# antonilo/unsupervised_detection

Hardware: NVIDIA H100
Metric: frame-pairs/sec adversarial train step 256x448 (higher is better)
Workload: dtype bf16

## Files before the change

include/cis_b200.h:

```cpp
#ifndef CIS_B200_H_
#define CIS_B200_H_
#include <stdint.h>
#include <stddef.h>

#ifdef __cplusplus
extern "C" {
#endif

typedef void* cis_stream_t;

enum { CIS_OK = 0, CIS_ERR_BAD_ARG = 1, CIS_ERR_UNSUPPORTED = 2, CIS_ERR_CUDA = 3 };
enum { CIS_ACT_NONE = 0, CIS_ACT_ELU = 1, CIS_ACT_LEAKY = 2 };
enum { CIS_MAX_TAPS = 49, CIS_MAX_SRC = 4 };

typedef struct {
  const void* ptr;
  int32_t pitch;
  int32_t c_off;
  int32_t chunks;
  int32_t n_mod;
} CisSrc;

typedef struct {
  int32_t N, H, W;
  int32_t OH, OW;
  int32_t sh, sw;
  int32_t ntaps;
  int16_t dh[CIS_MAX_TAPS];
  int16_t dw[CIS_MAX_TAPS];
  int32_t nsrc;
  CisSrc src[CIS_MAX_SRC];
  const void* wpack;
  int32_t K_pad;
  int32_t BN;
  int32_t n_tiles;
  const float* bias;
  int32_t act;
  float alpha;
  int32_t DH, DW;
  int32_t osh, osw, oa, ob;
  void* out;
  int32_t out_pitch, out_coff, out_ch;
  float* outf;
  int32_t outf_pitch, outf_coff, outf_ch;
  const void* add_pre;
  int32_t add_pre_pitch, add_pre_coff;
  const float* addf_pre;
  int32_t addf_pitch, addf_coff;
  const void* add_post;
  int32_t add_post_pitch, add_post_coff;
  int32_t mode;
  int32_t halo;
  int32_t dil;
  int32_t MT;
  int32_t hoy, hox;
  int32_t ey, ex;
  int32_t splits;
  float* sk_scratch;
  int32_t* sk_counters;
  int32_t nph;
  int32_t ph_tap[5];
  int32_t sk_cluster;
  int32_t nsub;
  struct {
    int32_t tap0, ntaps;
    int32_t hoy, hox;
    int32_t OH, OW, oa, ob;
    const void* wpack;
  } sub[4];
  int32_t nwg;
} CisConv;

typedef struct {
  int32_t N, H, W, OH, OW, sh, sw, ntaps;
  int16_t dh[CIS_MAX_TAPS];
  int16_t dw[CIS_MAX_TAPS];
  int32_t nsrc;
  CisSrc src[CIS_MAX_SRC];
  const void* g;
  int32_t g_pitch, g_coff, g_chunks;
  float* dwp;
  int32_t Cout;
  int32_t K_pad;
  int32_t splits;
  int32_t tma;
  int32_t nh;
  int32_t nwg;
} CisWgrad;

const char* cis_last_error(void);
int cis_version(void);
uint32_t cis_crc32c(uint32_t crc, const void* data, size_t n);
int cis_host_resize_bilinear_legacy(const float* src, int32_t H, int32_t W, int32_t C, float* dst, int32_t OH, int32_t OW);
int cis_host_bgr8_to_rgb_resized(const unsigned char* bgr, int32_t H, int32_t W, float* dst, int32_t OH, int32_t OW);

int cis_conv_igemm(const CisConv* d, cis_stream_t stream);
int cis_set_persist_mode(int mode);
int cis_conv_wgrad(const CisWgrad* d, cis_stream_t stream);

int cis_pack_weights(const float* w, const int32_t* kmap, int32_t K_pad, int32_t rows, int32_t cout, int32_t sn, const int32_t* nmap,
                     void* wp, cis_stream_t stream);
int cis_pack_weights_tiled(const float* w, const int32_t* kmap, int32_t cin8, int32_t ntaps, int32_t n_tiles, int32_t BN, int32_t cout,
                           int32_t sn, const int32_t* nmap, void* out, cis_stream_t stream);
int cis_unpack_wgrad(const float* dwp, const int32_t* kmap, int32_t K_pad, int32_t cout, int32_t nsplit, float* dw, const float* colpart,
                     int32_t nblocks, int32_t nch, float* db, int32_t layout, cis_stream_t stream);
int cis_bn_fold(const float* w, const float* bias, const float* gamma, const float* beta, int64_t nw, int32_t cout, float* w_eff,
                float* b_eff, cis_stream_t stream);
int cis_bn_chain(const float* w, const float* bias, const float* gamma, float* dw_eff_to_dw, const float* db_eff, int64_t nw,
                 int32_t cout, float* dbias, float* dgamma, float* dbeta, cis_stream_t stream);

enum { CIS_JOB_PACK = 0, CIS_JOB_PACK_TILED = 1, CIS_JOB_UNPACK = 2, CIS_JOB_BN_FOLD = 3, CIS_JOB_BN_CHAIN = 4 };
typedef struct {
  int32_t kind;
  int32_t i[8];
  int64_t n;
  const void* p[8];
} CisParamJob;
int cis_param_multi(const CisParamJob* jobs_dev, int32_t njobs, int32_t total_blocks, cis_stream_t stream);

int cis_dact_mul(void* g, int32_t g_pitch, int32_t g_coff, const void* y, int32_t y_pitch, int32_t y_coff, const void* res,
                 int32_t res_pitch, int32_t res_coff, int64_t npix, int32_t chunks, int32_t act, float alpha, cis_stream_t stream);
int cis_add_slice(void* dst, int32_t dst_pitch, int32_t dst_coff, const void* src, int32_t src_pitch, int32_t src_coff,
                  int64_t npix_dst, int32_t chunks, int32_t reps, int32_t accumulate, cis_stream_t stream);
int cis_colsum(const void* g, int32_t g_pitch, int32_t g_coff, int64_t npix, int32_t nch, float* part, int32_t nblocks, cis_stream_t stream);

int cis_zero(void* ptr, int64_t nbytes, cis_stream_t stream);

int cis_dact_colsum(void* g, int32_t g_pitch, int32_t g_coff, const void* y, int32_t y_pitch, int32_t y_coff, const void* res,
                    int32_t res_pitch, int32_t res_coff, int64_t npix, int32_t nch, int32_t act, float alpha, float* part, int32_t nblocks,
                    cis_stream_t stream);

int cis_resize_bilinear_bf16(const void* src, int32_t s_pitch, int32_t s_coff, int32_t N, int32_t H, int32_t W, void* dst,
                             int32_t d_pitch, int32_t d_coff, int32_t OH, int32_t OW, int32_t chunks, cis_stream_t stream);
int cis_resize_concat_bf16(const CisSrc* srcs, int32_t nsrc, int32_t N, int32_t H, int32_t W, void* dst, int32_t d_pitch, int32_t d_coff,
                           int32_t OH, int32_t OW, cis_stream_t stream);
int cis_resize_concat_bf16_bwd(const void* ddst, int32_t d_pitch, int32_t d_coff, int32_t N, int32_t OH, int32_t OW, const CisSrc* grads,
                               const int32_t* want, const int32_t* accumulate, int32_t nsrc, int32_t H, int32_t W, cis_stream_t stream);
int cis_resize_bilinear_bf16_bwd(const void* ddst, int32_t d_pitch, int32_t d_coff, int32_t N, int32_t OH, int32_t OW, void* dsrc,
                                 int32_t s_pitch, int32_t s_coff, int32_t H, int32_t W, int32_t chunks, int32_t accumulate,
                                 cis_stream_t stream);
int cis_resize_bilinear_f32(const float* src, int32_t N, int32_t H, int32_t W, int32_t C, float* dst, int32_t OH, int32_t OW,
                            float scale, cis_stream_t stream);
int cis_upsample_nn2x(const void* src, int32_t N, int32_t H, int32_t W, int32_t pitch, void* dst, cis_stream_t stream);
int cis_upsample_nn2x_bwd(const void* ddst, int32_t N, int32_t H, int32_t W, int32_t pitch, void* dsrc, int32_t accumulate,
                          cis_stream_t stream);
int cis_crop_resize_bilinear_f32(const float* src, int32_t Hs, int32_t Ws, int32_t C, int32_t y0, int32_t x0, int32_t ch, int32_t cw, float* dst,
                                 int32_t OH, int32_t OW, cis_stream_t stream);
int cis_crop_resize_flow_f32(const float* src, int32_t Hs, int32_t Ws, int32_t y0, int32_t x0, int32_t ch, int32_t cw, float* dst, int32_t OH,
                             int32_t OW, float s0, float s1, cis_stream_t stream);
int cis_resize_nn_f32(const float* src, int32_t N, int32_t H, int32_t W, int32_t C, float* dst, int32_t OH, int32_t OW,
                      cis_stream_t stream);
enum { CIS_RESIZE_BILINEAR = 0, CIS_RESIZE_NEAREST = 1 };
int cis_resize_f32(const float* src, int32_t N, int32_t H, int32_t W, int32_t C, float* dst, int32_t OH, int32_t OW, int32_t method,
                   int32_t align_corners, cis_stream_t stream);
int cis_resize_f32_bwd(const float* ddst, int32_t N, int32_t OH, int32_t OW, int32_t C, int32_t H, int32_t W, float* dsrc, int32_t method,
                       int32_t align_corners, cis_stream_t stream);

int cis_warp_costvol(const void* c1, int32_t c1_pitch, int32_t c1_coff, const void* c2, int32_t c2_pitch, int32_t c2_coff,
                     const float* flow, float flow_scale, int32_t B, int32_t h, int32_t w, int32_t C, void* out, int32_t out_pitch,
                     int32_t out_coff, cis_stream_t stream);
int cis_warp_costvol_r(const void* c1, int32_t c1_pitch, int32_t c1_coff, const void* c2, int32_t c2_pitch, int32_t c2_coff,
                       const float* flow, float flow_scale, int32_t B, int32_t h, int32_t w, int32_t C, void* out, int32_t out_pitch,
                       int32_t out_coff, int32_t search_range, cis_stream_t stream);
int cis_dense_image_warp(const void* img, int32_t pitch, int32_t coff, const float* flow, float flow_scale, int32_t B, int32_t h,
                         int32_t w, int32_t C, void* out, int32_t out_pitch, cis_stream_t stream);

int cis_pack_f32_to_bf16(const float* src, int64_t npix, int32_t C, float offset, void* dst, int32_t d_pitch, int32_t d_coff,
                         cis_stream_t stream);
int cis_flow_stats(const float* flow, int32_t B, int64_t hw, double* stats, cis_stream_t stream);
int cis_pack_generator_input(const float* image, const float* flow, const double* stats, int32_t B, int64_t hw, void* dst,
                             cis_stream_t stream);
int cis_flow_standardize(const float* flow, const double* stats, int32_t B, int64_t hw, float* out, cis_stream_t stream);
int cis_flow_standardize_bwd(const float* y, const float* dy, const double* stats, int32_t B, int64_t hw, double* scratch, float* dx,
                             cis_stream_t stream);
int cis_masked_epe(const float* pred, const float* gt, const float* mask, int32_t B, int64_t hw, double* scratch, double* out,
                   cis_stream_t stream);

int cis_mask_apply(const float* flow, const float* mask, int32_t B, int64_t hw, void* dst, cis_stream_t stream);
int cis_box_masks(float* mask, int32_t B, int32_t H, int32_t W, int32_t lo_h, int32_t hi_h, int32_t lo_w, int32_t hi_w, int64_t sample_offset,
                  const long long* step, uint64_t seed, cis_stream_t stream);
int cis_charbonnier_sum(const float* gt, const float* pred, const float* mask, int32_t B, int64_t hw, int32_t C, int32_t mask_c, float cbn,
                        double* sums, cis_stream_t stream);
int cis_cis_loss_fwd(const float* flow, const float* mask, const float* flow1, int32_t B, int32_t H, int32_t W, int32_t h1,
                     int32_t w1, float cbn, double* sums, float* pred_out , cis_stream_t stream);
int cis_cis_loss_reduce(const double* sums, int32_t B, int32_t global_batch, int64_t hw, float epsilon, float* scalars, float* coef,
                        cis_stream_t stream);
// ... 49 lines not shown
```

unsupervised_detection_b200/_lib.py:

```python
import ctypes as C
import os

_HERE = os.path.dirname(os.path.abspath(__file__))
LIB_PATH = os.path.join(_HERE, os.environ.get('CIS_LIB_NAME', 'libcis_b200.so'))

MAX_TAPS, MAX_SRC = 49, 4
ACT_NONE, ACT_ELU, ACT_LEAKY = 0, 1, 2
RESIZE_BILINEAR, RESIZE_NEAREST = 0, 1


class CisSrc(C.Structure):
    _fields_ = [('ptr', C.c_void_p), ('pitch', C.c_int32), ('c_off', C.c_int32), ('chunks', C.c_int32), ('n_mod', C.c_int32)]


class CisParamJob(C.Structure):
    _fields_ = [('kind', C.c_int32), ('i', C.c_int32 * 8), ('n', C.c_int64), ('p', C.c_void_p * 8)]


JOB_PACK, JOB_PACK_TILED, JOB_UNPACK, JOB_BN_FOLD, JOB_BN_CHAIN = range(5)


class CisSub(C.Structure):
    _fields_ = [('tap0', C.c_int32), ('ntaps', C.c_int32), ('hoy', C.c_int32), ('hox', C.c_int32), ('OH', C.c_int32), ('OW', C.c_int32),
                ('oa', C.c_int32), ('ob', C.c_int32), ('wpack', C.c_void_p)]


class CisConv(C.Structure):
    _fields_ = [('N', C.c_int32), ('H', C.c_int32), ('W', C.c_int32), ('OH', C.c_int32), ('OW', C.c_int32),
                ('sh', C.c_int32), ('sw', C.c_int32), ('ntaps', C.c_int32),
                ('dh', C.c_int16 * MAX_TAPS), ('dw', C.c_int16 * MAX_TAPS),
                ('nsrc', C.c_int32), ('src', CisSrc * MAX_SRC),
                ('wpack', C.c_void_p), ('K_pad', C.c_int32), ('BN', C.c_int32), ('n_tiles', C.c_int32),
                ('bias', C.c_void_p), ('act', C.c_int32), ('alpha', C.c_float),
                ('DH', C.c_int32), ('DW', C.c_int32), ('osh', C.c_int32), ('osw', C.c_int32), ('oa', C.c_int32), ('ob', C.c_int32),
                ('out', C.c_void_p), ('out_pitch', C.c_int32), ('out_coff', C.c_int32), ('out_ch', C.c_int32),
                ('outf', C.c_void_p), ('outf_pitch', C.c_int32), ('outf_coff', C.c_int32), ('outf_ch', C.c_int32),
                ('add_pre', C.c_void_p), ('add_pre_pitch', C.c_int32), ('add_pre_coff', C.c_int32),
                ('addf_pre', C.c_void_p), ('addf_pitch', C.c_int32), ('addf_coff', C.c_int32),
                ('add_post', C.c_void_p), ('add_post_pitch', C.c_int32), ('add_post_coff', C.c_int32),
                ('mode', C.c_int32),
                ('halo', C.c_int32), ('dil', C.c_int32), ('MT', C.c_int32), ('hoy', C.c_int32), ('hox', C.c_int32),
                ('ey', C.c_int32), ('ex', C.c_int32),
                ('splits', C.c_int32), ('sk_scratch', C.c_void_p), ('sk_counters', C.c_void_p),
                ('nph', C.c_int32), ('ph_tap', C.c_int32 * 5), ('sk_cluster', C.c_int32),
                ('nsub', C.c_int32), ('sub', CisSub * 4), ('nwg', C.c_int32)]


class CisWgrad(C.Structure):
    _fields_ = [('N', C.c_int32), ('H', C.c_int32), ('W', C.c_int32), ('OH', C.c_int32), ('OW', C.c_int32),
                ('sh', C.c_int32), ('sw', C.c_int32), ('ntaps', C.c_int32),
                ('dh', C.c_int16 * MAX_TAPS), ('dw', C.c_int16 * MAX_TAPS),
                ('nsrc', C.c_int32), ('src', CisSrc * MAX_SRC),
                ('g', C.c_void_p), ('g_pitch', C.c_int32), ('g_coff', C.c_int32), ('g_chunks', C.c_int32),
                ('dwp', C.c_void_p), ('Cout', C.c_int32), ('K_pad', C.c_int32), ('splits', C.c_int32), ('tma', C.c_int32),
                ('nh', C.c_int32), ('nwg', C.c_int32)]


_i32, _i64, _f32, _p, _u64 = C.c_int32, C.c_int64, C.c_float, C.c_void_p, C.c_uint64

_PROTOS = {
    'cis_conv_igemm': [C.POINTER(CisConv)],
    'cis_conv_wgrad': [C.POINTER(CisWgrad)],
    'cis_pack_weights': [_p, _p, _i32, _i32, _i32, _i32, _p, _p],
    'cis_pack_weights_tiled': [_p, _p, _i32, _i32, _i32, _i32, _i32, _i32, _p, _p],
    'cis_unpack_wgrad': [_p, _p, _i32, _i32, _i32, _p, _p, _i32, _i32, _p, _i32],
    'cis_bn_fold': [_p, _p, _p, _p, _i64, _i32, _p, _p],
    'cis_param_multi': [_p, _i32, _i32],
    'cis_bn_chain': [_p, _p, _p, _p, _p, _i64, _i32, _p, _p, _p],
    'cis_dact_mul': [_p, _i32, _i32, _p, _i32, _i32, _p, _i32, _i32, _i64, _i32, _i32, _f32],
    'cis_add_slice': [_p, _i32, _i32, _p, _i32, _i32, _i64, _i32, _i32, _i32],
    'cis_colsum': [_p, _i32, _i32, _i64, _i32, _p, _i32],
    'cis_zero': [_p, _i64],
    'cis_dact_colsum': [_p, _i32, _i32, _p, _i32, _i32, _p, _i32, _i32, _i64, _i32, _i32, _f32, _p, _i32],
    'cis_resize_bilinear_bf16': [_p, _i32, _i32, _i32, _i32, _i32, _p, _i32, _i32, _i32, _i32, _i32],
    'cis_resize_concat_bf16': [C.POINTER(CisSrc), _i32, _i32, _i32, _i32, _p, _i32, _i32, _i32, _i32],
    'cis_resize_concat_bf16_bwd': [_p, _i32, _i32, _i32, _i32, _i32, C.POINTER(CisSrc), C.POINTER(C.c_int32), C.POINTER(C.c_int32), _i32, _i32, _i32],
    'cis_resize_bilinear_bf16_bwd': [_p, _i32, _i32, _i32, _i32, _i32, _p, _i32, _i32, _i32, _i32, _i32, _i32],
    'cis_resize_bilinear_f32': [_p, _i32, _i32, _i32, _i32, _p, _i32, _i32, _f32],
    'cis_upsample_nn2x': [_p, _i32, _i32, _i32, _i32, _p],
    'cis_upsample_nn2x_bwd': [_p, _i32, _i32, _i32, _i32, _p, _i32],
    'cis_crop_resize_bilinear_f32': [_p, _i32, _i32, _i32, _i32, _i32, _i32, _i32, _p, _i32, _i32],
    'cis_crop_resize_flow_f32': [_p, _i32, _i32, _i32, _i32, _i32, _i32, _p, _i32, _i32, _f32, _f32],
    'cis_resize_nn_f32': [_p, _i32, _i32, _i32, _i32, _p, _i32, _i32],
    'cis_resize_f32': [_p, _i32, _i32, _i32, _i32, _p, _i32, _i32, _i32, _i32],
    'cis_resize_f32_bwd': [_p, _i32, _i32, _i32, _i32, _i32, _i32, _p, _i32, _i32],
    'cis_flow_standardize': [_p, _p, _i32, _i64, _p],
    'cis_flow_standardize_bwd': [_p, _p, _p, _i32, _i64, _p, _p],
    'cis_masked_epe': [_p, _p, _p, _i32, _i64, _p, _p],
    'cis_warp_costvol': [_p, _i32, _i32, _p, _i32, _i32, _p, _f32, _i32, _i32, _i32, _i32, _p, _i32, _i32],
    'cis_dense_image_warp': [_p, _i32, _i32, _p, _f32, _i32, _i32, _i32, _i32, _p, _i32],
    'cis_pack_f32_to_bf16': [_p, _i64, _i32, _f32, _p, _i32, _i32],
    'cis_flow_stats': [_p, _i32, _i64, _p],
    'cis_pack_generator_input': [_p, _p, _p, _i32, _i64, _p],
    'cis_mask_apply': [_p, _p, _i32, _i64, _p],
    'cis_box_masks': [_p, _i32, _i32, _i32, _i32, _i32, _i32, _i32, _i64, _p, _u64],
    'cis_charbonnier_sum': [_p, _p, _p, _i32, _i64, _i32, _i32, _f32, _p],
    'cis_cis_loss_fwd': [_p, _p, _p, _i32, _i32, _i32, _i32, _i32, _f32, _p, _p],
    'cis_cis_loss_reduce': [_p, _i32, _i32, _i64, _f32, _p, _p],
    'cis_cis_loss_bwd': [_p, _p, _p, _p, _p, _i32, _i32, _i32, _i32, _i32, _f32, _i32, _p, _p],
    'cis_resize_f32_bwd_to_bf16': [_p, _i32, _i32, _i32, _i32, _i32, _i32, _p, _i32],
    'cis_mask_bwd': [_p, _p, _p, _p, _i32, _i64, _p],
    'cis_abs_sum': [_p, _i64, _p],
    'cis_grad_avg_abs': [_p, _p, _i32, _p],
    'cis_clip_adam': [_p, _p, _p, _p, _i64, _f32, _f32, _f32, _f32, _f32, _f32, _p, _p, _i32, _u64],
    'cis_cast_f32_to_bf16': [_p, _i64, _p],
    'cis_cast_bf16_to_f32': [_p, _i64, _i32, _i32, _i32, _p],
    'cis_cast_bf16_to_f32_scaled': [_p, _i64, _i32, _i32, _i32, _f32, _p],
    'cis_charbonnier_bwd': [_p, _p, _p, _i32, _i64, _i32, _i32, _f32, _p, _p, _p, _p],
    'cis_dense_image_warp_bwd': [_p, _i32, _i32, _p, _f32, _i32, _i32, _i32, _i32, _p, _p, _p, _p],
    'cis_cost_volume_bwd': [_p, _i32, _i32, _p, _i32, _i32, _p, _i32, _i32, _i32, _i32, _p, _p, _p],
    'cis_resize_f32_bwd_to_bf16_scaled': [_p, _i32, _i32, _i32, _i32, _i32, _i32, _p, _i32, _f32],
    'cis_warp_costvol_bwd': [_p, _i32, _i32, _p, _i32, _i32, _p, _f32, _i32, _i32, _i32, _i32, _p, _i32, _i32, _p, _i32, _i32, _p, _i32, _i32,
                             _p, _i32, _i32, _i32, _p, _p, _p],
    'cis_parity_split_bf16': [_p, _i32, _i32, _i32, _i32, _i32, _i32, _p, _i32],
    'cis_warp_costvol_r': [_p, _i32, _i32, _p, _i32, _i32, _p, _f32, _i32, _i32, _i32, _i32, _p, _i32, _i32, _i32],
    'cis_cost_volume_bwd_r': [_p, _i32, _i32, _p, _i32, _i32, _p, _i32, _i32, _i32, _i32, _p, _p, _p, _i32],
    'cis_warp_costvol_bwd_r': [_p, _i32, _i32, _p, _i32, _i32, _p, _f32, _i32, _i32, _i32, _i32, _p, _i32, _i32, _p, _i32, _i32, _p, _i32, _i32,
                               _p, _i32, _i32, _i32, _p, _p, _p, _i32],
}
EXPORTS = sorted(list(_PROTOS) + ['cis_last_error', 'cis_version', 'cis_set_persist_mode', 'cis_crc32c', 'cis_host_resize_bilinear_legacy',
                                  'cis_host_bgr8_to_rgb_resized'])

_lib = None


def load():
    global _lib
    if _lib is None:
        if not os.path.exists(LIB_PATH):
            raise RuntimeError('libcis_b200.so not built: run `python -c "import __graft_entry__ as g; g.build()"` '
                               '(no CPU fallback exists for the product path)')
        lib = C.CDLL(LIB_PATH)
        lib.cis_last_error.restype = C.c_char_p
        lib.cis_version.restype = C.c_int
        lib.cis_set_persist_mode.argtypes = [C.c_int]
        lib.cis_set_persist_mode.restype = C.c_int
        lib.cis_crc32c.argtypes = [C.c_uint32, C.c_void_p, C.c_size_t]
        lib.cis_crc32c.restype = C.c_uint32
        lib.cis_host_resize_bilinear_legacy.argtypes = [C.c_void_p, C.c_int32, C.c_int32, C.c_int32, C.c_void_p, C.c_int32, C.c_int32]
        lib.cis_host_resize_bilinear_legacy.restype = C.c_int
        lib.cis_host_bgr8_to_rgb_resized.argtypes = [C.c_void_p, C.c_int32, C.c_int32, C.c_void_p, C.c_int32, C.c_int32]
        lib.cis_host_bgr8_to_rgb_resized.restype = C.c_int
        for name, args in _PROTOS.items():
            fn = getattr(lib, name)
            fn.argtypes = list(args) + [C.c_void_p]
            fn.restype = C.c_int
        _lib = lib
# ... 11 lines not shown
```

unsupervised_detection_b200/csrc/conv_igemm.cu:

```cuda
#include "ptx.cuh"
#include "../../include/cis_b200.h"
#include "common.cuh"
#include <cuda.h>
#include <stdlib.h>
#include <string.h>


namespace cis {

#ifdef CIS_TRACE
__device__ unsigned long long* g_trace = nullptr;
__device__ int g_trace_cap = 0;
#define CIS_TRACE_AT(slot)                                                                                         \
  do {                                                                                                             \
    if (g_trace && blockIdx.x == 0 && blockIdx.y == 0 && blockIdx.z == 0 && (slot) < g_trace_cap) g_trace[(slot)] = clock64(); \
  } while (0)
#else
#define CIS_TRACE_AT(slot) ((void)0)
#endif

static constexpr int kBM = 128;
static constexpr int kBK = 64;
static constexpr int kAStage = kBM * 128;
static constexpr int kThreads = 256;
// ... 408 lines not shown
      else if (i == 1) cp_async_wait<1>();
      else cp_async_wait<0>();
      fence_proxy_async();
      mbar_arrive(bar_full + 8 * ((nkb - 1 - i) % S));
    }

    mbar_wait(bar_accum, 0);
    if (tid == 0) CIS_TRACE_AT(2);
    const int qtr = warp & 3, half = warp >> 2;
    const int row = qtr * 32 + lane;
    const int g = blockIdx.x * kBM + row;
    const bool valid = g < M;
    size_t dpix = 0;
    if (valid) {
      const int ow = g % p.OW;
      const int t = g / p.OW;
      const int oh = t % p.OH;
      const int n = t / p.OH;
      dpix = (size_t)(n * p.DH + oh * p.osh + p.oa) * p.DW + ow * p.osw + p.ob;
    }
    const uint32_t t_row = tile_base + (uint32_t)row * 16;
    const int cbase = ny * BN;
    constexpr int kHalf = BN >= 32 ? BN / 2 : BN;
    const int c_lo = half * kHalf, c_hi = (BN >= 32 || half == 0) ? c_lo + kHalf : c_lo;
    if (nsplit > 1 && p.sk_cluster) {
    } else if (nsplit > 1) {
      const int tile_id = blockIdx.x * gridDim.y + ny;
      float* tile0 = p.sk_scratch + (size_t)tile_id * nsplit * kBM * BN;
      splitk_store_partial<BN>(tile0 + (size_t)blockIdx.z * kBM * BN, t_row, row, c_lo, c_hi);
    } else {
      epi_cols<BN>(p, t_row, cbase, dpix, valid, s_bias, c_lo, c_hi);
    }
  } else {
    const int wtid = tid - kMmaWarp * 32;
    float acc[BN];
    const uint32_t dhi = desc_hi(1024);
    constexpr uint32_t a_half = (8 * 1024) >> 4;
    for (int kb = 0; kb < nkb; ++kb) {
      const int s = kb % S;
      mbar_wait(bar_full + 8 * s, (uint32_t)((kb / S) & 1));
      if (wtid == 0) CIS_TRACE_AT(8 + 2 * kb);
      const uint32_t alo = desc_lo(a_base + s * kAStage, 16), blo = desc_lo(b_base + s * Cfg::kBStage, 16);
      wg_fence();
#pragma unroll
      for (int k = 0; k < kBK / 16; ++k) mma128<BN, 0, 0>(acc, alo + 2 * k, dhi, blo + 2 * k, dhi, a_half, (uint32_t)((kb | k) != 0));
      wg_commit();
      wg_wait<1>();
      if (wtid == 0 && kb > 0) mbar_arrive(bar_empty + 8 * ((kb - 1) % S));
      if (wtid == 0) CIS_TRACE_AT(9 + 2 * kb);
    }
    wg_wait<0>();
    acc_store<BN>(acc, tile_base, wtid);
    mbar_arrive(bar_accum);
  }
  if (nsplit > 1 && p.sk_cluster) {
    cluster_sync_all();
    if (warp < kMmaWarp) {
      const int cbase = ny * BN;
      cluster_reduce_rows<BN>(p, tile_base, nsplit, (int)cluster_ctarank(), tid, kGProducers, cbase, [&](int row, bool& valid) -> size_t {
        const int g = blockIdx.x * kBM + row;
        valid = g < M;
        if (!valid) return 0;
        const int ow = g % p.OW;
        const int t = g / p.OW;
        const int oh = t % p.OH;
        const int n = t / p.OH;
        return (size_t)(n * p.DH + oh * p.osh + p.oa) * p.DW + ow * p.osw + p.ob;
      });
    }
    cluster_sync_all();
  }
  if (tid == 0) CIS_TRACE_AT(3);
}


static constexpr int kHaloMaxBStages = 8;
struct HaloMaps {
  CUtensorMap m[CIS_MAX_SRC * 4];
};

template <int NK, int MT, int BN, int MTM>
__device__ __forceinline__ void halo_issue_stage(float (&acc)[MTM][BN], const uint32_t hlo, uint32_t blo, const uint32_t* s_aoff, const int gt,
                                                 const uint32_t ahi, const uint32_t bhi, const uint32_t a_mstep, const uint32_t a_half,
                                                 const bool first) {
  const uint32_t bstep = (uint32_t)(BN * 128) >> 4;
  uint32_t off0 = s_aoff[0], off1 = gt > 1 ? s_aoff[1] : 0u;
  int tt = 0;
#pragma unroll 1
  do {
    const uint32_t off2 = tt + 2 < gt ? s_aoff[tt + 2] : 0u;
    const uint32_t alo = hlo + off0;
    const uint32_t acc0 = (uint32_t)(!(first && tt == 0));
    wg_fence();
#pragma unroll
    for (int m = 0; m < MT; ++m) {
#pragma unroll
      for (int k = 0; k < NK; ++k) mma128<BN, 0, 0>(acc[m], alo + m * a_mstep + 2 * k, ahi, blo + 2 * k, bhi, a_half, k ? 1u : acc0);
    }
    wg_commit();
    off0 = off1;
    off1 = off2;
    blo += bstep;
  } while (++tt < gt);
}
template <int MT, int BN, int MTM>
__device__ __forceinline__ void halo_issue_nk(const int nk16, float (&acc)[MTM][BN], const uint32_t hlo, const uint32_t blo, const uint32_t* s_aoff,
                                              const int gt, const uint32_t ahi, const uint32_t bhi, const uint32_t a_mstep, const uint32_t a_half,
                                              const bool first) {
  if (nk16 == 4) halo_issue_stage<4, MT>(acc, hlo, blo, s_aoff, gt, ahi, bhi, a_mstep, a_half, first);
  else if (nk16 == 1) halo_issue_stage<1, MT>(acc, hlo, blo, s_aoff, gt, ahi, bhi, a_mstep, a_half, first);
  else if (nk16 == 2) halo_issue_stage<2, MT>(acc, hlo, blo, s_aoff, gt, ahi, bhi, a_mstep, a_half, first);
  else halo_issue_stage<3, MT>(acc, hlo, blo, s_aoff, gt, ahi, bhi, a_mstep, a_half, first);
}
template <int BN, int MTM>
__device__ __forceinline__ void halo_issue_any(const int nk16, float (&acc)[MTM][BN], const uint32_t hlo, const uint32_t blo, const uint32_t* s_aoff,
                                               const int gt, const int MT, const uint32_t ahi, const uint32_t bhi, const uint32_t a_mstep,
                                               const uint32_t a_half, const bool first) {
  static_assert(MTM >= 1 && MTM <= 4, "1..4 stacked tiles");
  if (MT == 1) halo_issue_nk<1>(nk16, acc, hlo, blo, s_aoff, gt, ahi, bhi, a_mstep, a_half, first);
  else if constexpr (MTM >= 2) {
    if (MT == 2) halo_issue_nk<2>(nk16, acc, hlo, blo, s_aoff, gt, ahi, bhi, a_mstep, a_half, first);
    else if constexpr (MTM >= 3) {
      if (MT == 3) halo_issue_nk<3>(nk16, acc, hlo, blo, s_aoff, gt, ahi, bhi, a_mstep, a_half, first);
      else if constexpr (MTM >= 4) halo_issue_nk<4>(nk16, acc, hlo, blo, s_aoff, gt, ahi, bhi, a_mstep, a_half, first);
    }
  }
  wg_wait<0>();
}

template <int BN, int NWG>
__global__ void __launch_bounds__(HaloCfg<BN, NWG>::kThreads, 1) conv_halo_kernel(const __grid_constant__ CisConv p, const int halo_stage_bytes, const int BS, const int NHS,
                                                        const __grid_constant__ HaloMaps maps, const int use_tma, const int G) {
  using Cfg = HaloCfg<BN, NWG>;
  constexpr int kBStage = BN * 128;
  constexpr int kHMmaWarp_ = Cfg::kMmaWarp, kHThreads_ = Cfg::kThreads;
  extern __shared__ uint8_t smem_raw[];
  __shared__ uint64_t bars[2 * 2 + 2 * kHaloMaxBStages + 1];
  __shared__ uint32_t s_aoff[CIS_MAX_TAPS];
  __shared__ SrcS s_src[CIS_MAX_SRC];

  const int tid = threadIdx.x, warp = tid >> 5, lane = tid & 31;
  const int MT = p.MT, MTC = NWG * MT, d = p.dil;
  const int nph = p.nph > 1 ? p.nph : 1;
  const int Wh = 8 + p.ex, Hh = 16 * MTC + p.ey, HP = Wh * Hh;
  const uint32_t stage_bytes = (uint32_t)G * kBStage;
  const uint32_t tile_base = (smem_u32(smem_raw) + 1023u) & ~1023u;
  const uint32_t h_base = tile_base;
  const uint32_t b_base = tile_base + NHS * halo_stage_bytes;
  int* pixtab = reinterpret_cast<int*>(smem_raw + (b_base + BS * stage_bytes - smem_u32(smem_raw)));
  const uint32_t bar_hfull = smem_u32(&bars[0]), bar_hempty = smem_u32(&bars[2]);
  const uint32_t bar_bfull = smem_u32(&bars[4]), bar_bempty = smem_u32(&bars[4 + kHaloMaxBStages]);
  const uint32_t bar_accum = smem_u32(&bars[4 + 2 * kHaloMaxBStages]);

  const bool grouped = p.nsub > 1;
  const int tap0 = grouped ? p.sub[blockIdx.z].tap0 : 0, ntaps = grouped ? p.sub[blockIdx.z].ntaps : p.ntaps;
  const int hoy = grouped ? p.sub[blockIdx.z].hoy : p.hoy, hox = grouped ? p.sub[blockIdx.z].hox : p.hox;
  const int OHs = grouped ? p.sub[blockIdx.z].OH : p.OH, OWs = grouped ? p.sub[blockIdx.z].OW : p.OW;
  const int oa = grouped ? p.sub[blockIdx.z].oa : p.oa, ob = grouped ? p.sub[blockIdx.z].ob : p.ob;
  const void* const wpack = grouped ? p.sub[blockIdx.z].wpack : p.wpack;
  const int Hp0 = (OHs + d - 1) / d, Wp0 = (OWs + d - 1) / d;
  const int tiles_x = (Wp0 + 7) / 8, tiles_y = (Hp0 + 16 * MTC - 1) / (16 * MTC);
  if (grouped && (int)blockIdx.x >= tiles_x * tiles_y * p.N) return;
  int bid = blockIdx.x;
  const int tx = bid % tiles_x; bid /= tiles_x;
  const int ty = bid % tiles_y; bid /= tiles_y;
  const int ph = bid % (d * d);
  const int n = bid / (d * d);
  const int pa = ph / d, pb = ph % d;
  const int ny = blockIdx.y;
  int m_chunks = 0;
  for (int i = 0; i < p.nsrc; ++i) m_chunks += p.src[i].chunks;
  const int nchunks_all = (m_chunks + 7) / 8;
  const int nsplit = (!grouped && p.splits > 1) ? p.splits : 1;
  const int cper = (nchunks_all + nsplit - 1) / nsplit;
  const int cc_lo = grouped ? 0 : blockIdx.z * cper;
  const int nchunks = min(cper, nchunks_all - cc_lo);
  __shared__ __align__(16) float s_bias[BN];
  pdl_launch_dependents();

  if (tid < ntaps) s_aoff[tid] = (uint32_t)((p.dh[tap0 + tid] * Wh + p.dw[tap0 + tid]) * 8);
  if (tid < p.nsrc) {
    s_src[tid].ptr = reinterpret_cast<const __nv_bfloat16*>(p.src[tid].ptr);
    s_src[tid].pitch = p.src[tid].pitch;
    s_src[tid].c_off = p.src[tid].c_off;
    s_src[tid].chunks = p.src[tid].chunks;
    s_src[tid].n_mod = p.src[tid].n_mod;
  }
  for (int q = tid; q < (use_tma ? 0 : HP); q += kHThreads_) {
    const int hy = q / Wh, hx = q - hy * Wh;
    const int gy = ty * 16 * MTC + hy + hoy, gx = tx * 8 + hx + hox;
    const int y = pa + d * gy, x = pb + d * gx;
    pixtab[q] = (gy >= 0 && gx >= 0 && y < p.H && x < p.W) ? (y * p.W + x) : -1;
  }
  if (tid == kHMmaWarp_ * 32) {
    for (int s = 0; s < 2; ++s) {
      mbar_init(bar_hfull + 8 * s, use_tma ? 1 : 96);
      mbar_init(bar_hempty + 8 * s, NWG);
    }
    for (int s = 0; s < BS; ++s) {
      mbar_init(bar_bfull + 8 * s, 1);
      mbar_init(bar_bempty + 8 * s, NWG);
    }
    mbar_init(bar_accum, 128 * NWG);
    fence_mbar_init();
  }
  if (use_tma && tid < p.nsrc) tma_prefetch_desc(&maps.m[tid]);
  pdl_wait();
  if (tid < BN) s_bias[tid] = p.bias ? p.bias[ny * BN + tid] : 0.f;
  __syncthreads();
  if (tid == 0) CIS_TRACE_AT(0);

  if (warp < kHMmaWarp_) {
   if (warp < 4) {
    if (use_tma) {
      if (tid == 0) {
        int hcount = 0;
        for (int vc = 0; vc < nchunks * nph; ++vc) {
          const int cc = vc / nph, ph = vc - cc * nph;
          if (nph > 1 && p.ph_tap[ph + 1] == p.ph_tap[ph]) continue;
          const int hs = hcount % NHS;
          mbar_wait(bar_hempty + 8 * hs, (uint32_t)(((hcount / NHS) & 1) ^ 1));
          ++hcount;
          int c = (cc_lo + cc) * 8, si = 0;
          while (si < p.nsrc - 1 && c >= s_src[si].chunks) {
            c -= s_src[si].chunks;
            ++si;
          }
          const int nmod = s_src[si].n_mod;
          mbar_expect_tx(bar_hfull + 8 * hs, (uint32_t)(HP * 128));
          tma_load_4d(h_base + hs * halo_stage_bytes, &maps.m[si * nph + ph], bar_hfull + 8 * hs, c * 8, pb + d * (tx * 8 + hox),
                      pa + d * (ty * 16 * MTC + hoy), nmod ? (n % nmod) : n);
        }
      }
      __syncwarp();
    } else if (warp != 2) {
      const int hid = warp == 3 ? tid - 32 : tid;
      const int j = hid & 7, pl = hid >> 3;
      for (int cc = 0; cc < nchunks; ++cc) {
        const int hs = cc % NHS;
        mbar_wait(bar_hempty + 8 * hs, (uint32_t)(((cc / NHS) & 1) ^ 1));
        const int rem = m_chunks - (cc_lo + cc) * 8;
        const int nk16 = rem >= 8 ? 4 : (rem + 1) / 2;
        const bool need = j < 2 * nk16;
        const bool cvalid = j < rem;
        int c = (cc_lo + cc) * 8 + j, si = 0;
        if (cvalid) {
          while (si < p.nsrc - 1 && c >= s_src[si].chunks) {
            c -= s_src[si].chunks;
            ++si;
          }
        } else {
          c = 0;
        }
        const int nmod = s_src[si].n_mod, pitch = s_src[si].pitch;
        const int ne = nmod ? (n % nmod) : n;
        const __nv_bfloat16* sp = s_src[si].ptr;
        const __nv_bfloat16* sb = sp + (size_t)ne * p.H * p.W * pitch + s_src[si].c_off + c * 8;
        if (need) {
          const uint32_t hdst = h_base + hs * halo_stage_bytes + (uint32_t)(j << 4);
          for (int q = pl; q < HP; q += 12) {
            const int off = pixtab[q];
            const bool ok = cvalid && off >= 0;
            cp_async16((hdst + q * 128) ^ (uint32_t)((q & 7) << 4), ok ? (const void*)(sb + (size_t)off * pitch) : (const void*)sp,
                       ok ? 16u : 0u);
          }
        }
        cp_async_commit();
        if (NHS == 1) {
          cp_async_wait<0>();
          fence_proxy_async();
          mbar_arrive(bar_hfull);
        } else if (cc >= 1) {
          cp_async_wait<1>();
          fence_proxy_async();
          mbar_arrive(bar_hfull + 8 * ((cc - 1) % NHS));
        }
      }
      if (NHS > 1) {
        cp_async_wait<0>();
        fence_proxy_async();
        mbar_arrive(bar_hfull + 8 * ((nchunks - 1) % NHS));
      }
    }
    if (tid == 64) {
      const uint8_t* wt = reinterpret_cast<const uint8_t*>(wpack) + ((size_t)ny * nchunks_all + cc_lo) * ntaps * kBStage;
      int bs = 0;
      uint32_t bph = 1;
      for (int vc = 0; vc < nchunks * nph; ++vc) {
        const int cc = vc / nph, ph = vc - cc * nph;
        const int tlo = nph > 1 ? p.ph_tap[ph] : 0, thi = nph > 1 ? p.ph_tap[ph + 1] : ntaps;
        for (int t0 = tlo; t0 < thi; t0 += G) {
          const uint32_t bytes = (uint32_t)min(G, thi - t0) * kBStage;
          mbar_wait(bar_bempty + 8 * bs, bph);
          mbar_expect_tx(bar_bfull + 8 * bs, bytes);
          bulk_g2s(b_base + bs * stage_bytes, wt + (size_t)(cc * ntaps + t0) * kBStage, bytes, bar_bfull + 8 * bs);
          if (++bs == BS) {
            bs = 0;
            bph ^= 1u;
          }
        }
      }
    }
    __syncwarp();
   }

  } else {
    const int wg = NWG > 1 ? (warp - kHMmaWarp_) >> 2 : 0;
    const int wtid = tid - (kHMmaWarp_ + 4 * wg) * 32;
    constexpr int MTM = Cfg::kMaxMT;
    float acc[MTM][BN];
    const uint32_t ahi = desc_hi((uint32_t)(Wh * 128)), bhi = desc_hi(1024);
    const uint32_t a_mstep = (uint32_t)(16 * Wh * 128) >> 4;
    const uint32_t a_half = (uint32_t)(8 * Wh * 128) >> 4;
    const uint32_t a_wg = (uint32_t)(wg * MT) * a_mstep;
    int bs = 0, hs = 0, it = 0;
    uint32_t bph = 0, hph = 0;
    bool any = false;
    for (int vc = 0; vc < nchunks * nph; ++vc) {
      const int cc = vc / nph, ph = vc - cc * nph;
      const int tlo = nph > 1 ? p.ph_tap[ph] : 0, thi = nph > 1 ? p.ph_tap[ph + 1] : ntaps;
      if (thi == tlo) continue;
      const int rem = m_chunks - (cc_lo + cc) * 8;
      const int nk16 = rem >= 8 ? 4 : (rem + 1) / 2;
      mbar_wait(bar_hfull + 8 * hs, hph);
      if (vc == 0 && wtid == 0 && wg == 0) CIS_TRACE_AT(1);
      const uint32_t hlo = desc_lo(h_base + hs * halo_stage_bytes, 16) + a_wg;
      for (int t0 = tlo; t0 < thi; t0 += G, ++it) {
        const int gt = min(G, thi - t0);
        mbar_wait(bar_bfull + 8 * bs, bph);
        if (wtid == 0 && wg == 0) CIS_TRACE_AT(8 + 2 * it);
        const uint32_t blo = desc_lo(b_base + bs * stage_bytes, 16);
        halo_issue_any<BN, MTM>(nk16, acc, hlo, blo, s_aoff + t0, gt, MT, ahi, bhi, a_mstep, a_half, !any);
        if (wtid == 0) {
          mbar_arrive(bar_bempty + 8 * bs);
          if (t0 + G >= thi) mbar_arrive(bar_hempty + 8 * hs);
          if (wg == 0) CIS_TRACE_AT(9 + 2 * it);
        }
        any = true;
        if (++bs == BS) {
          bs = 0;
          bph ^= 1u;
        }
      }
      if (++hs == NHS) {
        hs = 0;
        hph ^= 1u;
      }
    }
    if constexpr (NWG > 1) asm volatile("bar.sync 1, %0;" ::"n"(128 * NWG) : "memory");
#pragma unroll
    for (int m = 0; m < MTM; ++m)
      if (m < MT) acc_store<BN>(acc[m], tile_base + (uint32_t)((wg * MT + m) * BN) * kAccColBytes, wtid);
    mbar_arrive(bar_accum);
  }

  if (warp < Cfg::kEpiWarps) {
    mbar_wait(bar_accum, 0);
    if (tid == 0) CIS_TRACE_AT(2);
    constexpr int kParts = Cfg::kEpiParts, kCols = BN / kParts, kUnits = 4 * kParts;
    const int cbase = ny * BN;
    const int tile_id = blockIdx.x * gridDim.y + ny;
    if (!(nsplit > 1 && p.sk_cluster)) {
#pragma unroll 1
      for (int u = warp; u < MTC * kUnits; u += Cfg::kEpiWarps) {
        const int m = u / kUnits, r = (u & 3) * 32 + lane, c_lo = ((u >> 2) % kParts) * kCols, c_hi = c_lo + kCols;
        const uint32_t t_row = tile_base + (uint32_t)(m * BN) * kAccColBytes + (uint32_t)r * 16;
        if (nsplit > 1) {
          splitk_store_partial<BN>(p.sk_scratch + (((size_t)tile_id * MTC + m) * nsplit + blockIdx.z) * kBM * BN, t_row, r, c_lo, c_hi);
        } else {
          const int gy = ty * 16 * MTC + 16 * m + (r >> 3), gx = tx * 8 + (r & 7);
          const int oy = pa + d * gy, ox = pb + d * gx;
          const bool valid = oy < OHs && ox < OWs;
          const size_t dpix = valid ? ((size_t)(n * p.DH + oy * p.osh + oa) * p.DW + ox * p.osw + ob) : 0;
          epi_cols<BN>(p, t_row, cbase, dpix, valid, s_bias, c_lo, c_hi);
        }
      }
    }
  }
  if (nsplit > 1 && p.sk_cluster) {
    cluster_sync_all();
    if (warp < 4) {
      const int cbase = ny * BN;
      for (int m = 0; m < MTC; ++m)
        cluster_reduce_rows<BN>(p, tile_base + (uint32_t)m * (kBM * BN * 4), nsplit, (int)cluster_ctarank(), tid, 128, cbase,
                                [&](int row, bool& valid) -> size_t {
                                  const int gy = ty * 16 * MTC + 16 * m + (row >> 3), gx = tx * 8 + (row & 7);
                                  const int oy = pa + d * gy, ox = pb + d * gx;
                                  valid = oy < OHs && ox < OWs;
                                  return valid ? ((size_t)(n * p.DH + oy * p.osh + oa) * p.DW + ox * p.osw + ob) : 0;
                                });
    }
    cluster_sync_all();
  }
  if (tid == 0) CIS_TRACE_AT(3);
}

template <int BN>
__global__ void __launch_bounds__(256) splitk_finish_kernel(const __grid_constant__ CisConv p) {
  constexpr int G = BN / 16;
  constexpr int kBlock = (128 * G < 256) ? 128 * G : 256;
  constexpr int kSub = 128 * G / kBlock;
  pdl_launch_dependents();
  pdl_wait();
  const int tid = threadIdx.x;
  if (tid >= kBlock) return;
  const int m = blockIdx.z / kSub;
  const int item = (blockIdx.z % kSub) * kBlock + tid;
  const int r = item % 128, c0 = (item / 128) * 16;
  const int ny = blockIdx.y;
  const int nsplit = p.splits;
  const int tile_id = blockIdx.x * gridDim.y + ny;
  bool valid;
  size_t dpix = 0;
  const float* tile0;
  if (p.halo) {
    const int MT = p.MT * (p.nwg > 1 ? p.nwg : 1), d = p.dil;
    const int Hp0 = (p.OH + d - 1) / d, Wp0 = (p.OW + d - 1) / d;
    const int tiles_x = (Wp0 + 7) / 8, tiles_y = (Hp0 + 16 * MT - 1) / (16 * MT);
    int bid = blockIdx.x;
    const int tx = bid % tiles_x; bid /= tiles_x;
    const int ty = bid % tiles_y; bid /= tiles_y;
    const int ph = bid % (d * d);
    const int n = bid / (d * d);
    const int pa = ph / d, pb = ph % d;
    const int gy = ty * 16 * MT + 16 * m + (r >> 3), gx = tx * 8 + (r & 7);
    const int oy = pa + d * gy, ox = pb + d * gx;
    valid = oy < p.OH && ox < p.OW;
    if (valid) dpix = (size_t)(n * p.DH + oy * p.osh + p.oa) * p.DW + ox * p.osw + p.ob;
    tile0 = p.sk_scratch + ((size_t)tile_id * MT + m) * nsplit * kBM * BN;
  } else {
    const int M = p.N * p.OH * p.OW;
    const int g = blockIdx.x * kBM + r;
    valid = g < M;
    if (valid) {
      const int ow = g % p.OW;
      const int t = g / p.OW;
      const int oh = t % p.OH;
      const int n = t / p.OH;
      dpix = (size_t)(n * p.DH + oh * p.osh + p.oa) * p.DW + ow * p.osw + p.ob;
    }
    tile0 = p.sk_scratch + (size_t)tile_id * nsplit * kBM * BN;
  }
  if (!valid) return;
  float v[16];
  splitk_reduce16<BN>(tile0, nsplit, r, c0, v);
  epi_chunk(p, v, ny * BN + c0, dpix);
}
static constexpr int kPThreads = 448;
static constexpr int kPMaxAccCols = 64;

template <int BN>
__global__ void __launch_bounds__(kPThreads, 1) conv_halo_persist_kernel(const __grid_constant__ CisConv p, const int halo_stage_bytes,
                                                                       const int BS, const int NHS, const int AS, const int G,
                                                                       const __grid_constant__ HaloMaps maps, const int ws) {
  constexpr int kBStage = BN * 128;
  constexpr int kMaxHS = 4;
  extern __shared__ uint8_t smem_raw[];
  __shared__ uint64_t bars[2 * kMaxHS + 2 * kHaloMaxBStages + 4];
  __shared__ uint32_t s_aoff[CIS_MAX_TAPS];
  __shared__ __align__(16) float s_bias[BN];

  const int tid = threadIdx.x, warp = tid >> 5, lane = tid & 31;
  const int MT = p.MT;
  const int Wh = 8 + p.ex, Hh = 16 * MT + p.ey, HP = Wh * Hh;
  const uint32_t stage_bytes = (uint32_t)G * kBStage;
  const uint32_t tile_base = (smem_u32(smem_raw) + 1023u) & ~1023u;
  const uint32_t acc_bytes = (uint32_t)(MT * BN) * kAccColBytes;
  const uint32_t acc_base = tile_base, h_base = tile_base + AS * acc_bytes, b_base = h_base + NHS * halo_stage_bytes;
  const uint32_t bar_hfull = smem_u32(&bars[0]), bar_hempty = smem_u32(&bars[kMaxHS]);
  const uint32_t bar_bfull = smem_u32(&bars[2 * kMaxHS]), bar_bempty = smem_u32(&bars[2 * kMaxHS + kHaloMaxBStages]);
  const uint32_t bar_tfull = smem_u32(&bars[2 * kMaxHS + 2 * kHaloMaxBStages]), bar_tempty = smem_u32(&bars[2 * kMaxHS + 2 * kHaloMaxBStages + 2]);

  const int tiles_x = (p.OW + 7) / 8, tiles_y = (p.OH + 16 * MT - 1) / (16 * MT);
  const int total = tiles_x * tiles_y * p.N;
  int m_chunks = 0;
  for (int i = 0; i < p.nsrc; ++i) m_chunks += p.src[i].chunks;
  const int nchunks = (m_chunks + 7) / 8;

  pdl_launch_dependents();
  if (tid < p.ntaps) s_aoff[tid] = (uint32_t)((p.dh[tid] * Wh + p.dw[tid]) * 8);
  if (tid == 0) {
    for (int s = 0; s < NHS; ++s) {
      mbar_init(bar_hfull + 8 * s, 1);
      mbar_init(bar_hempty + 8 * s, 1);
    }
    for (int s = 0; s < BS; ++s) {
      mbar_init(bar_bfull + 8 * s, 1);
      mbar_init(bar_bempty + 8 * s, 1);
    }
    for (int s = 0; s < AS; ++s) {
      mbar_init(bar_tfull + 8 * s, 128);
      mbar_init(bar_tempty + 8 * s, 4);
    }
    fence_mbar_init();
  }
  if (tid < p.nsrc) tma_prefetch_desc(&maps.m[tid]);
  pdl_wait();
  if (tid < BN) s_bias[tid] = p.bias ? p.bias[tid] : 0.f;
  __syncthreads();
  if (tid == 0) {
    CIS_TRACE_AT(0);
    CIS_TRACE_AT(4);
  }

  if (warp == 12) {
    if (lane == 0) {
      int hs = 0;
      uint32_t hph = 1;
      for (int w = blockIdx.x; w < total; w += gridDim.x) {
        const int tx = w % tiles_x, r1 = w / tiles_x, ty = r1 % tiles_y, n = r1 / tiles_y;
        for (int cc = 0; cc < nchunks; ++cc) {
          mbar_wait(bar_hempty + 8 * hs, hph);
          int c = cc * 8, si = 0;
          while (si < p.nsrc - 1 && c >= p.src[si].chunks) {
            c -= p.src[si].chunks;
            ++si;
          }
          int nmod = p.src[0].n_mod;
          if (si == 1) nmod = p.src[1].n_mod;
          if (si == 2) nmod = p.src[2].n_mod;
          if (si == 3) nmod = p.src[3].n_mod;
          mbar_expect_tx(bar_hfull + 8 * hs, (uint32_t)(HP * 128));
          tma_load_4d(h_base + hs * halo_stage_bytes, &maps.m[si], bar_hfull + 8 * hs, c * 8, tx * 8 + p.hox, ty * 16 * MT + p.hoy,
                      nmod ? (n % nmod) : n);
          if (++hs == NHS) {
            hs = 0;
            hph ^= 1u;
          }
        }
      }
    }
  } else if (warp == 13) {
    if (lane == 0) {
      const uint8_t* wt = reinterpret_cast<const uint8_t*>(p.wpack);
      const int per_tile = nchunks * p.ntaps;
      if (ws) {
        if ((int)blockIdx.x < total) {
          mbar_expect_tx(bar_bfull, (uint32_t)(per_tile * kBStage));
          for (int it = 0; it < per_tile; it += 8) {
            const int nt = min(8, per_tile - it);
            bulk_g2s(b_base + it * kBStage, wt + (size_t)it * kBStage, (uint32_t)(nt * kBStage), bar_bfull);
          }
        }
      } else {
        int bs = 0;
        uint32_t bph = 1;
        for (int w = blockIdx.x; w < total; w += gridDim.x) {
          for (int cc = 0; cc < nchunks; ++cc) {
            for (int t0 = 0; t0 < p.ntaps; t0 += G) {
              const uint32_t bytes = (uint32_t)min(G, p.ntaps - t0) * kBStage;
              mbar_wait(bar_bempty + 8 * bs, bph);
              mbar_expect_tx(bar_bfull + 8 * bs, bytes);
              bulk_g2s(b_base + bs * stage_bytes, wt + (size_t)(cc * p.ntaps + t0) * kBStage, bytes, bar_bfull + 8 * bs);
              if (++bs == BS) {
                bs = 0;
                bph ^= 1u;
              }
            }
          }
        }
      }
    }
  } else if (warp < 4) {
    const int wtid = tid;
    constexpr int MTM = (kPMaxAccCols / BN) < 4 ? kPMaxAccCols / BN : 4;
    float acc[MTM][BN];
    const uint32_t ahi = desc_hi((uint32_t)(Wh * 128)), bhi = desc_hi(1024);
    const uint32_t a_mstep = (uint32_t)(16 * Wh * 128) >> 4;
    const uint32_t a_half = (uint32_t)(8 * Wh * 128) >> 4;
    int hs = 0, bs = 0, as = 0;
    uint32_t hph = 0, bph = 0, tph = 1;
    if (ws && (int)blockIdx.x < total) mbar_wait(bar_bfull, 0u);
    int wi = 0;
    for (int w = blockIdx.x; w < total; w += gridDim.x, ++wi) {
      if (wtid == 0) CIS_TRACE_AT(8 + 5 * wi);
      for (int cc = 0; cc < nchunks; ++cc) {
        const int rem = m_chunks - cc * 8;
        const int nk16 = rem >= 8 ? 4 : (rem + 1) / 2;
        mbar_wait(bar_hfull + 8 * hs, hph);
        if (cc == 0 && wtid == 0) CIS_TRACE_AT(10 + 5 * wi);
        const uint32_t hlo = desc_lo(h_base + hs * halo_stage_bytes, 16);
        const int gstep = ws ? p.ntaps : G;
        for (int t0 = 0; t0 < p.ntaps; t0 += gstep) {
          const int gt = min(gstep, p.ntaps - t0);
          if (!ws) mbar_wait(bar_bfull + 8 * bs, bph);
          const uint32_t blo = desc_lo(ws ? b_base + (uint32_t)(cc * p.ntaps) * kBStage : b_base + bs * stage_bytes, 16);
          halo_issue_any<BN, MTM>(nk16, acc, hlo, blo, s_aoff + t0, gt, MT, ahi, bhi, a_mstep, a_half, (cc | t0) == 0);
          if (wtid == 0) {
            if (!ws) mbar_arrive(bar_bempty + 8 * bs);
            if (t0 + gstep >= p.ntaps) mbar_arrive(bar_hempty + 8 * hs);
          }
          if (!ws && ++bs == BS) {
            bs = 0;
            bph ^= 1u;
          }
        }
        if (++hs == NHS) {
          hs = 0;
          hph ^= 1u;
        }
      }
      mbar_wait(bar_tempty + 8 * as, tph);
      if (wtid == 0) CIS_TRACE_AT(9 + 5 * wi);
#pragma unroll
      for (int m = 0; m < MTM; ++m)
        if (m < MT) acc_store<BN>(acc[m], acc_base + as * acc_bytes + (uint32_t)(m * BN) * kAccColBytes, wtid);
      mbar_arrive(bar_tfull + 8 * as);
      if (wtid == 0) CIS_TRACE_AT(11 + 5 * wi);
      if (++as == AS) {
        as = 0;
        tph ^= 1u;
      }
    }
  } else if (warp >= 4) {
    const int grp = (warp - 4) >> 2, q = warp & 3;
    const int r = q * 32 + lane;
    if (grp < AS) {
      uint32_t tph = 0;
      int wi = 0;
      for (int w = blockIdx.x; w < total; w += gridDim.x, ++wi) {
        if (wi % AS != grp) continue;
        const int tx = w % tiles_x, r1 = w / tiles_x, ty = r1 % tiles_y, n = r1 / tiles_y;
        mbar_wait(bar_tfull + 8 * grp, tph);
        tph ^= 1u;
        for (int m = 0; m < MT; ++m) {
          const int oy = ty * 16 * MT + 16 * m + (r >> 3), ox = tx * 8 + (r & 7);
          const bool valid = oy < p.OH && ox < p.OW;
          const size_t dpix = valid ? ((size_t)(n * p.DH + oy * p.osh + p.oa) * p.DW + ox * p.osw + p.ob) : 0;
          epi_row<BN>(p, acc_base + grp * acc_bytes + (uint32_t)r * 16 + (uint32_t)(m * BN) * kAccColBytes, 0, dpix, valid, s_bias);
        }
        __syncwarp();
        if (lane == 0) mbar_arrive(bar_tempty + 8 * grp);
        if (q == 0 && lane == 0) CIS_TRACE_AT(12 + 5 * wi);
      }
    }
  }
}

static constexpr int kWStages = 3;
static constexpr int kWTile = 64 * 128;
static constexpr int kWStage = 4 * kWTile;
static constexpr int kWSmem = kWStages * kWStage + 1024;

struct WgradMaps {
  CUtensorMap g;
  CUtensorMap x[CIS_MAX_SRC];
};

__global__ void __launch_bounds__(kGThreads) conv_wgrad_kernel(const __grid_constant__ CisWgrad p, const __grid_constant__ WgradMaps maps) {
  constexpr int S = kWStages;
  extern __shared__ uint8_t smem_raw[];
  __shared__ uint64_t bars[2 * S + 1];
  __shared__ int s_dh[CIS_MAX_TAPS], s_dw[CIS_MAX_TAPS];
  const uint32_t tile_base = (smem_u32(smem_raw) + 1023u) & ~1023u;
  const uint32_t bar_full = smem_u32(&bars[0]);
  const uint32_t bar_empty = smem_u32(&bars[S]);
  const uint32_t bar_accum = smem_u32(&bars[2 * S]);
  const int tid = threadIdx.x, warp = tid >> 5, lane = tid & 31;
  const int nprod = (int)blockDim.x - 128, mma_warp = nprod >> 5;
  pdl_launch_dependents();
  if (tid < p.ntaps) {
    s_dh[tid] = p.dh[tid];
    s_dw[tid] = p.dw[tid];
  }
  const int M = p.N * p.OH * p.OW;
  int m_chunks = 0;
  for (int i = 0; i < p.nsrc; ++i) m_chunks += p.src[i].chunks;
  const int k_chunks = p.ntaps * m_chunks;
  const int tiles_x = (p.OW + 7) / 8, tiles_y = (p.OH + 7) / 8;
  const int nkb_total = p.tma ? p.N * tiles_x * tiles_y : (M + 63) / 64;
  const int per = (nkb_total + p.splits - 1) / p.splits;
  const int kb0 = blockIdx.y * per;
  const int kb1 = min(kb0 + per, nkb_total);
  const int nkb = kb1 - kb0;
  if (nkb <= 0) return;

  if (tid == mma_warp * 32) {
    for (int s = 0; s < S; ++s) {
      mbar_init(bar_full + 8 * s, p.tma ? 1 : nprod);
      mbar_init(bar_empty + 8 * s, 1);
    }
    mbar_init(bar_accum, 128);
    fence_mbar_init();
  }
  pdl_wait();
  __syncthreads();

  if (warp < mma_warp) {
    if (p.tma) {
      if (tid == 0) {
        const int nch64 = (m_chunks + 7) / 8;
        int gsrc[2], gc0[2], gdh[2], gdw[2], gnm[2];
        bool gok[2];
#pragma unroll
        for (int u = 0; u < 2; ++u) {
          const int grp = blockIdx.x * 2 + u;
          gok[u] = grp < p.ntaps * nch64;
          const int t = gok[u] ? grp / nch64 : 0;
          int c = gok[u] ? (grp - t * nch64) * 8 : 0, si = 0;
          while (si < p.nsrc - 1 && c >= p.src[si].chunks) {
            c -= p.src[si].chunks;
            ++si;
          }
          gsrc[u] = si;
          gc0[u] = c * 8;
          gdh[u] = s_dh[t];
          gdw[u] = s_dw[t];
          int nm = p.src[0].n_mod;
          if (si == 1) nm = p.src[1].n_mod;
          if (si == 2) nm = p.src[2].n_mod;
          if (si == 3) nm = p.src[3].n_mod;
// ... 349 lines not shown
  constexpr int kBlock = (128 * G < 256) ? 128 * G : 256;
  constexpr int kSub = 128 * G / kBlock;
  const int mt = d->halo ? d->MT * (d->nwg > 1 ? d->nwg : 1) : 1;
  return launch_pdl(splitk_finish_kernel<BN>, dim3(main_grid.x, main_grid.y, mt * kSub), dim3(kBlock), 0, st, *d);
}

template <int BN>
static int launch_fwd(const CisConv* d, cudaStream_t st) {
  using Cfg = FwdCfg<BN>;
  static bool attr_set = false;
  if (!attr_set) {
    cudaError_t e = cudaFuncSetAttribute(conv_igemm_kernel<BN>, cudaFuncAttributeMaxDynamicSharedMemorySize, Cfg::kSmem);
    if (e != cudaSuccess) return cis_set_cuda_error(e, "cudaFuncSetAttribute(conv_igemm)");
    attr_set = true;
  }
  const int M = d->N * d->OH * d->OW;
  int splits = d->splits > 1 ? d->splits : 1;
  if (splits > 1) {
    const int nkb = d->K_pad / kBK, per = (nkb + splits - 1) / splits;
    if ((!d->sk_scratch && !d->sk_cluster) || d->sk_counters || (splits - 1) * per >= nkb || (d->sk_cluster && splits > 8))
      return cis_set_error(CIS_ERR_BAD_ARG, "cis_conv_igemm: bad split-K setup");
  }
  dim3 grid((M + kBM - 1) / kBM, d->n_tiles, splits);
  cudaError_t le = (splits > 1 && d->sk_cluster)
                       ? launch_pdl_zcluster(conv_igemm_kernel<BN>, grid, dim3(kGThreads), Cfg::kSmem, st, splits, *d)
                       : launch_pdl(conv_igemm_kernel<BN>, grid, dim3(kGThreads), Cfg::kSmem, st, *d);
  if (le != cudaSuccess) return cis_set_cuda_error(le, "launch(conv_igemm)");
  if (splits > 1 && !d->sk_cluster) {
    le = launch_splitk_finish<BN>(d, grid, st);
    if (le != cudaSuccess) return cis_set_cuda_error(le, "launch(splitk_finish)");
  }
  return cis_check_launch("conv_igemm");
}


typedef CUresult (*EncodeTiledFn)(CUtensorMap*, CUtensorMapDataType, cuuint32_t, void*, const cuuint64_t*, const cuuint64_t*, const cuuint32_t*,
                                  const cuuint32_t*, CUtensorMapInterleave, CUtensorMapSwizzle, CUtensorMapL2promotion, CUtensorMapFloatOOBfill);
static EncodeTiledFn get_encode_tiled() {
  static EncodeTiledFn fn = nullptr;
  static bool tried = false;
  if (!tried) {
    tried = true;
    void* p = nullptr;
    cudaDriverEntryPointQueryResult q;
    if (cudaGetDriverEntryPoint("cuTensorMapEncodeTiled", &p, cudaEnableDefault, &q) == cudaSuccess && q == cudaDriverEntryPointSuccess)
      fn = (EncodeTiledFn)p;
  }
  return fn;
}
static bool encode_src_map(CUtensorMap* m, const CisSrc& s, int N, int H, int W, int bw, int bh, int step = 1, int py = 0, int px = 0,
                           int estride = 1, int bc = 64, CUtensorMapSwizzle swz = CU_TENSOR_MAP_SWIZZLE_128B) {
  EncodeTiledFn enc = get_encode_tiled();
  if (!enc) return false;
  const int nb = s.n_mod > 0 ? s.n_mod : N;
  const int Hq = (H - py + step - 1) / step, Wq = (W - px + step - 1) / step;
  if (Hq < 1 || Wq < 1) return false;
  cuuint64_t dims[4] = {(cuuint64_t)s.chunks * 8, (cuuint64_t)Wq, (cuuint64_t)Hq, (cuuint64_t)nb};
  cuuint64_t strides[3] = {(cuuint64_t)step * s.pitch * 2, (cuuint64_t)step * W * s.pitch * 2, (cuuint64_t)H * W * s.pitch * 2};
  cuuint32_t box[4] = {(cuuint32_t)bc, (cuuint32_t)(bw * estride), (cuuint32_t)(bh * estride), 1};
  cuuint32_t es[4] = {1, (cuuint32_t)estride, (cuuint32_t)estride, 1};
  void* base = (void*)((const char*)s.ptr + ((size_t)(py * W + px) * s.pitch + (size_t)s.c_off) * 2);
  return enc(m, CU_TENSOR_MAP_DATA_TYPE_BFLOAT16, 4, base, dims, strides, box, es, CU_TENSOR_MAP_INTERLEAVE_NONE, swz,
             CU_TENSOR_MAP_L2_PROMOTION_L2_128B, CU_TENSOR_MAP_FLOAT_OOB_FILL_NONE) == CUDA_SUCCESS;
}

#ifdef CIS_TRACE
extern "C" int cis_trace_set(unsigned long long* buf, int cap) {
  cudaError_t e = cudaMemcpyToSymbol(cis::g_trace, &buf, sizeof(buf));
  if (e == cudaSuccess) e = cudaMemcpyToSymbol(cis::g_trace_cap, &cap, sizeof(cap));
  return e == cudaSuccess ? CIS_OK : cis_set_cuda_error(e, "cis_trace_set");
}
#endif

static int g_persist_mode = -1;
extern "C" int cis_set_persist_mode(int mode) {
  g_persist_mode = mode;
  return CIS_OK;
}

template <int BN, int NWG>
static int launch_halo(const CisConv* d, cudaStream_t st) {
  const int MTC = d->MT * NWG;
  const int Wh = 8 + d->ex, Hh = 16 * MTC + d->ey, HP = Wh * Hh;
  const int halo_stage = (HP * 128 + 1023) & ~1023;
  int chunks = 0;
  for (int i = 0; i < d->nsrc; ++i) chunks += d->src[i].chunks;
  const int nchunks = (chunks + 7) / 8;
  const int nsub = d->nsub > 1 ? d->nsub : 1;
  const int nsp = (nsub == 1 && d->splits > 1) ? d->splits : 1;
  const int cper = (nchunks + nsp - 1) / nsp;
  const int nhs = cper > 1 ? 2 : 1;
  const int dd = d->dil;
  int tiles = 0, ntaps_max = d->ntaps;
  if (nsub > 1) {
    if (nsub > 4 || dd != 1 || d->splits > 1 || d->nph > 1) return cis_set_error(CIS_ERR_BAD_ARG, "cis_conv_igemm(halo): bad grouped launch");
    ntaps_max = 0;
    int tsum = 0;
    for (int i = 0; i < nsub; ++i) {
      const int t = ((d->sub[i].OW + 7) / 8) * ((d->sub[i].OH + 16 * MTC - 1) / (16 * MTC));
      if (t > tiles) tiles = t;
      if (d->sub[i].ntaps > ntaps_max) ntaps_max = d->sub[i].ntaps;
      if (d->sub[i].ntaps < 1 || d->sub[i].tap0 != tsum || !d->sub[i].wpack) return cis_set_error(CIS_ERR_BAD_ARG, "cis_conv_igemm(halo): bad sub-problem");
      tsum += d->sub[i].ntaps;
    }
    if (tsum != d->ntaps) return cis_set_error(CIS_ERR_BAD_ARG, "cis_conv_igemm(halo): sub-problem taps must add up to ntaps");
  } else {
    const int Hp0 = (d->OH + dd - 1) / dd, Wp0 = (d->OW + dd - 1) / dd;
    tiles = ((Wp0 + 7) / 8) * ((Hp0 + 16 * MTC - 1) / (16 * MTC));
  }
  const long ncta_all = (long)tiles * dd * dd * d->N * d->n_tiles * nsp * nsub;
  static const int g_env = getenv("CIS_HALO_G") ? atoi(getenv("CIS_HALO_G")) : 0;
  static const int stage_kb = getenv("CIS_HALO_STAGE_KB") ? atoi(getenv("CIS_HALO_STAGE_KB")) : 48;
  const int kB = BN * 128;
  int G = g_env > 0 ? g_env : (stage_kb * 1024) / kB;
  if (G < 1) G = 1;
  if (G > ntaps_max) G = ntaps_max;
  const int fixed = nhs * halo_stage + HP * 4 + 1024;
  static const int lim_small_kb = getenv("CIS_HALO_SMALL_KB") ? atoi(getenv("CIS_HALO_SMALL_KB")) : 226;
  static const int lim_kb_wide = getenv("CIS_HALO_LIMIT_KB") ? atoi(getenv("CIS_HALO_LIMIT_KB")) : 113;
  static const int lim_kb_thin = getenv("CIS_HALO_LIMIT_THIN_KB") ? atoi(getenv("CIS_HALO_LIMIT_THIN_KB")) : 113;
  const int lim_kb = BN <= 32 ? lim_kb_thin : lim_kb_wide;
  const int nsm = cis_num_sms();
  int limit = (ncta_all > nsm && fixed + 2 * kB <= lim_kb * 1024) ? lim_kb * 1024 : 226 * 1024;
  if (ncta_all <= nsm && fixed + 2 * kB <= lim_small_kb * 1024) limit = lim_small_kb * 1024;
  while (G > 1 && fixed + 2 * G * kB > limit) --G;
  const int groups = cper * ((nsub > 1 ? 1 : (ntaps_max + G - 1) / G));
  int BS = (limit - fixed) / (G * kB);
  if (BS > (ncta_all > nsm ? 4 : kHaloMaxBStages)) BS = ncta_all > nsm ? 4 : kHaloMaxBStages;
  if (BS > groups) BS = groups;
  if (BS < 1) return cis_set_error(CIS_ERR_UNSUPPORTED, "cis_conv_igemm(halo): tile does not fit shared memory");
  int smem = fixed + BS * G * kB;
  if (smem < MTC * kBM * BN * 4 + 1024) smem = MTC * kBM * BN * 4 + 1024;
  if (smem > 226 * 1024) return cis_set_error(CIS_ERR_UNSUPPORTED, "cis_conv_igemm(halo): accumulator tiles do not fit shared memory");
  static int attr_smem = 0;
  if (smem > attr_smem) {
    cudaError_t e = cudaFuncSetAttribute(conv_halo_kernel<BN, NWG>, cudaFuncAttributeMaxDynamicSharedMemorySize, smem);
    if (e != cudaSuccess) return cis_set_cuda_error(e, "cudaFuncSetAttribute(conv_halo)");
    attr_smem = smem;
  }

  int splits = d->splits > 1 ? d->splits : 1;
  if (splits > 1) {
    const int per = (nchunks + splits - 1) / splits;
    if ((!d->sk_scratch && !d->sk_cluster) || d->sk_counters || (splits - 1) * per >= nchunks || (d->sk_cluster && splits > 8))
      return cis_set_error(CIS_ERR_BAD_ARG, "cis_conv_igemm(halo): bad split-K setup");
  }
  dim3 grid(tiles * dd * dd * d->N, d->n_tiles, nsub > 1 ? nsub : splits);
  HaloMaps maps;
  const int nph = d->nph > 1 ? d->nph : 1;
  static const int dil_tma = getenv("CIS_DIL_TMA") ? atoi(getenv("CIS_DIL_TMA")) : 1;
  int use_tma = ((d->dil == 1 || dil_tma) && Wh * d->dil <= 256 && Hh * d->dil <= 256) ? 1 : 0;
  for (int i = 0; use_tma && i < d->nsrc - 1; ++i)
    if (d->src[i].chunks % 8) use_tma = 0;
  for (int i = 0; use_tma && i < d->nsrc; ++i) {
    if (((uintptr_t)d->src[i].ptr + (size_t)d->src[i].c_off * 2) % 16) use_tma = 0;
    for (int ph = 0; use_tma && ph < nph; ++ph)
      if (!encode_src_map(&maps.m[i * nph + ph], d->src[i], d->N, d->H, d->W, Wh, Hh, nph > 1 ? 2 : 1, ph >> 1, ph & 1, d->dil)) use_tma = 0;
  }
  if (!use_tma) memset(&maps, 0, sizeof(maps));
  if (nph > 1 && !use_tma) return cis_set_error(CIS_ERR_UNSUPPORTED, "cis_conv_igemm(halo): stride-2 phases need the TMA halo path");
  const int persist_mode = g_persist_mode >= 0 ? g_persist_mode : (getenv("CIS_PERSIST_MODE") ? atoi(getenv("CIS_PERSIST_MODE")) : 1);
  static const int p_min_tiles = getenv("CIS_PERSIST_MIN_TILES") ? atoi(getenv("CIS_PERSIST_MIN_TILES")) : 296;
  static const int p_ws_kb = getenv("CIS_PERSIST_WS_KB") ? atoi(getenv("CIS_PERSIST_WS_KB")) : 112;
  if constexpr (BN <= kPMaxAccCols && NWG == 1) {
   if (persist_mode > 0 && use_tma && d->n_tiles == 1 && splits == 1 && nph == 1 && nsub == 1 && dd == 1 && d->MT * BN <= kPMaxAccCols) {
    const int total = tiles * d->N;
    const int per_tile = nchunks * d->ntaps;
    const int acc_stage = d->MT * BN * (int)kAccColBytes;
    const int AS = 2;
    const int fixed_p = AS * acc_stage + 1024;
    const int ws_bytes = per_tile * kB;
    int p_nhs = nchunks >= 3 ? 4 : 3;
    while (p_nhs > 2 && p_nhs * halo_stage + fixed_p + (ws_bytes <= p_ws_kb * 1024 ? ws_bytes : 2 * G * kB) > 226 * 1024) --p_nhs;
    const bool ws_fits = ws_bytes <= p_ws_kb * 1024 && p_nhs * halo_stage + fixed_p + ws_bytes <= 226 * 1024;
    const bool take = persist_mode == 2 || (persist_mode == 3 && ws_fits) || (persist_mode == 1 && ws_fits && total >= p_min_tiles);
    int p_bs = 0, p_smem = 0;
    if (ws_fits) {
      p_bs = 1;
      p_smem = p_nhs * halo_stage + fixed_p + ws_bytes;
    } else {
      p_bs = (226 * 1024 - p_nhs * halo_stage - fixed_p) / (G * kB);
      if (p_bs > 4) p_bs = 4;
      p_smem = p_nhs * halo_stage + fixed_p + p_bs * G * kB;
    }
    if (take && p_bs >= (ws_fits ? 1 : 2)) {
      static int attr_p = 0;
      if (p_smem > attr_p) {
        cudaError_t e = cudaFuncSetAttribute(conv_halo_persist_kernel<BN>, cudaFuncAttributeMaxDynamicSharedMemorySize, p_smem);
        if (e != cudaSuccess) return cis_set_cuda_error(e, "cudaFuncSetAttribute(conv_halo_persist)");
        attr_p = p_smem;
      }
      int cps = 0;
      cudaError_t e = cudaOccupancyMaxActiveBlocksPerMultiprocessor(&cps, conv_halo_persist_kernel<BN>, kPThreads, p_smem);
      if (e != cudaSuccess) return cis_set_cuda_error(e, "cudaOccupancyMaxActiveBlocksPerMultiprocessor(conv_halo_persist)");
      if (cps < 1) cps = 1;
      int g = total < nsm * cps ? total : nsm * cps;
      cudaError_t le = launch_pdl(conv_halo_persist_kernel<BN>, dim3(g), dim3(kPThreads), p_smem, st, *d, halo_stage, p_bs, p_nhs, AS, G, maps,
                                  ws_fits ? 1 : 0);
      if (le != cudaSuccess) return cis_set_cuda_error(le, "launch(conv_halo_persist)");
      return cis_check_launch("conv_halo_persist");
    }
   }
  }
  cudaError_t le = (splits > 1 && d->sk_cluster)
                       ? launch_pdl_zcluster(conv_halo_kernel<BN, NWG>, grid, dim3(HaloCfg<BN, NWG>::kThreads), smem, st, splits, *d, halo_stage, BS, nhs, maps,
                                             use_tma, G)
                       : launch_pdl(conv_halo_kernel<BN, NWG>, grid, dim3(HaloCfg<BN, NWG>::kThreads), smem, st, *d, halo_stage, BS, nhs, maps, use_tma, G);
  if (le != cudaSuccess) return cis_set_cuda_error(le, "launch(conv_halo)");
  if (splits > 1 && !d->sk_cluster) {
    le = launch_splitk_finish<BN>(d, grid, st);
    if (le != cudaSuccess) return cis_set_cuda_error(le, "launch(splitk_finish)");
  }
  return cis_check_launch("conv_halo");
}

extern "C" int cis_conv_igemm(const CisConv* d, cis_stream_t stream) {
  if (!d || d->ntaps < 1 || d->ntaps > CIS_MAX_TAPS || d->nsrc < 1 || d->nsrc > CIS_MAX_SRC || d->K_pad % 64 != 0 || d->K_pad <= 0 ||
      d->n_tiles < 1 || !d->wpack)
    return cis_set_error(CIS_ERR_BAD_ARG, "cis_conv_igemm: bad descriptor");
  int chunks = 0;
  for (int i = 0; i < d->nsrc; ++i) {
    if ((d->src[i].pitch | d->src[i].c_off) & 7) return cis_set_error(CIS_ERR_BAD_ARG, "cis_conv_igemm: source pitch/c_off must be multiples of 8");
    chunks += d->src[i].chunks;
  }
  if (d->ntaps * chunks * 8 > d->K_pad) return cis_set_error(CIS_ERR_BAD_ARG, "cis_conv_igemm: K_pad smaller than taps*channels");
  if (d->mode == 1 && !d->outf) return cis_set_error(CIS_ERR_BAD_ARG, "cis_conv_igemm: mode 1 needs outf");
  if ((d->add_pre || d->add_post) && (((d->add_pre_pitch | d->add_pre_coff | d->add_post_pitch | d->add_post_coff | d->out_ch) & 7) != 0))
    return cis_set_error(CIS_ERR_BAD_ARG, "cis_conv_igemm: residual slices must be 8-channel aligned");
  cudaStream_t st = (cudaStream_t)stream;
  if (d->halo) {
    if (d->MT < 1 || d->MT > 4 || d->MT * d->BN > kMaxAccCols || d->nwg < 0 || d->nwg > 2 || (d->nwg == 2 && d->BN < 64) || d->dil < 1 ||
        d->sh != 1 || d->sw != 1 || d->ey < 0 || d->ex < 0 ||
        (d->dil > 1 && (d->OH != d->H || d->OW != d->W)) || (d->nph > 1 && (d->nph != 4 || d->dil != 1 || d->ph_tap[0] != 0 || d->ph_tap[4] != d->ntaps)))
      return cis_set_error(CIS_ERR_BAD_ARG, "cis_conv_igemm(halo): bad tile parameters");
    switch (d->BN) {
      case 16: return launch_halo<16, 1>(d, st);
      case 32: return launch_halo<32, 1>(d, st);
      case 64: return d->nwg == 2 ? launch_halo<64, 2>(d, st) : launch_halo<64, 1>(d, st);
      case 128: return d->nwg == 2 ? launch_halo<128, 2>(d, st) : launch_halo<128, 1>(d, st);
      default: return cis_set_error(CIS_ERR_UNSUPPORTED, "cis_conv_igemm: BN must be 16/32/64/128");
    }
  }
  switch (d->BN) {
    case 16: return launch_fwd<16>(d, st);
    case 32: return launch_fwd<32>(d, st);
    case 64: return launch_fwd<64>(d, st);
    case 128: return launch_fwd<128>(d, st);
    default: return cis_set_error(CIS_ERR_UNSUPPORTED, "cis_conv_igemm: BN must be 16/32/64/128");
  }
}

template <int NH, int NWG>
static int launch_wgrad_halo_t(const CisWgrad* d, cudaStream_t st, int nch64, int Wh, int Hh, int hoy, int hox, int halo_bytes) {
  using Cfg = WgradHaloCfg<NH>;
  const bool wg_halves = NWG == 2 && d->Cout > 64;
  const int stage = halo_bytes + (wg_halves ? 2 : 1) * (int)Cfg::kGTile;
  const int npairs = (d->ntaps + 1) / 2, nhalf = d->Cout > 64 ? 2 : 1;
  const int gz = wg_halves ? (npairs + Cfg::kPairs - 1) / Cfg::kPairs : nhalf * ((npairs + NWG * Cfg::kPairs - 1) / (NWG * Cfg::kPairs));
  int S = (200 * 1024) / stage;
  if (S > kWHMaxStages) S = kWHMaxStages;
  if (S < 2) return cis_set_error(CIS_ERR_UNSUPPORTED, "cis_conv_wgrad(halo): halo does not fit shared memory");
  int smem = S * stage + 1024;
  const int acc_smem = NWG * kMaxAccCols * (int)kAccColBytes + 1024;
  if (smem < acc_smem) smem = acc_smem;
  static int attr_smem = 0;
  if (smem > attr_smem) {
    cudaError_t e = cudaFuncSetAttribute(conv_wgrad_halo_kernel<NH, NWG>, cudaFuncAttributeMaxDynamicSharedMemorySize, smem);
    if (e != cudaSuccess) return cis_set_cuda_error(e, "cudaFuncSetAttribute(conv_wgrad_halo)");
// ... 85 lines not shown
```

unsupervised_detection_b200/csrc/misc_kernels.cu:

```cuda
#include "ptx.cuh"
#include "../../include/cis_b200.h"
#include "common.cuh"
#include <math.h>

namespace cis {

typedef __nv_bfloat16 bf16;

__device__ __forceinline__ void unpack8(const uint4& u, float* f) {
  f[0] = bf16lo(u.x); f[1] = bf16hi(u.x); f[2] = bf16lo(u.y); f[3] = bf16hi(u.y);
  f[4] = bf16lo(u.z); f[5] = bf16hi(u.z); f[6] = bf16lo(u.w); f[7] = bf16hi(u.w);
}
__device__ __forceinline__ uint4 pack8(const float* f) {
  return make_uint4(pack_bf16(f[0], f[1]), pack_bf16(f[2], f[3]), pack_bf16(f[4], f[5]), pack_bf16(f[6], f[7]));
}
__device__ __forceinline__ float warp_sum(float v) {
#pragma unroll
  for (int o = 16; o > 0; o >>= 1) v += __shfl_xor_sync(0xffffffffu, v, o);
  return v;
}
__device__ __forceinline__ double warp_sum_d(double v) {
#pragma unroll
  for (int o = 16; o > 0; o >>= 1) v += __shfl_xor_sync(0xffffffffu, v, o);
  return v;
}

__device__ __forceinline__ void pack_weights_body(size_t i, const float* __restrict__ w, const int* __restrict__ kmap, int K_pad, int rows, int cout,
                                                  int sn, const int* __restrict__ nmap, bf16* __restrict__ wp) {
  if (i >= (size_t)rows * K_pad) return;
  const int n = (int)(i / K_pad), k = (int)(i % K_pad);
  const int km = kmap[k];
  const int ne = nmap ? nmap[n] : (n < cout ? n : -1);
  const float v = (km >= 0 && ne >= 0) ? w[(size_t)km + (size_t)ne * sn] : 0.f;
  wp[i] = __float2bfloat16(v);
}
__device__ __forceinline__ void pack_weights_tiled_body(size_t i, const float* __restrict__ w, const int* __restrict__ kmap, int cin8, int ntaps,
                                                        int n_tiles, int BN, int cout, int sn, const int* __restrict__ nmap,
                                                        bf16* __restrict__ out) {
  const int nchunks = (cin8 + 63) / 64;
  const size_t total = (size_t)n_tiles * nchunks * ntaps * BN * 64;
  if (i >= total) return;
  const int pos = (int)(i % 64);
  size_t r = i / 64;
  const int n = (int)(r % BN); r /= BN;
  const int t = (int)(r % ntaps); r /= ntaps;
  const int cc = (int)(r % nchunks);
  const int ny = (int)(r / nchunks);
  const int kk = (((pos >> 3) ^ (n & 7)) << 3) | (pos & 7);
  const int c = cc * 64 + kk;
  float v = 0.f;
  if (c < cin8) {
    const int km = kmap[t * cin8 + c];
    const int ng = ny * BN + n;
    const int ne = nmap ? nmap[ng] : (ng < cout ? ng : -1);
    if (km >= 0 && ne >= 0) v = w[(size_t)km + (size_t)ne * sn];
  }
  out[i] = __float2bfloat16(v);
}
__device__ __forceinline__ void pack_weights_tiled_tile(int blk, const float* __restrict__ w, const int* __restrict__ kmap, int cin8, int ntaps,
                                                        int n_tiles, int BN, int cout, const int* __restrict__ nmap, bf16* __restrict__ out,
                                                        float* tile) {
  const int nchunks = (cin8 + 63) / 64;
  const int t = blk % ntaps;
  const int r = blk / ntaps;
  const int cc = r % nchunks, ny = r / nchunks;
  const int ld = BN + 1;
  for (int idx = threadIdx.x; idx < BN * 64; idx += blockDim.x) {
    const int n = idx % BN, kk = idx / BN;
    const int c = cc * 64 + kk;
    float v = 0.f;
    if (c < cin8) {
      const int km = kmap[t * cin8 + c];
      const int ng = ny * BN + n;
      const int ne = nmap ? nmap[ng] : (ng < cout ? ng : -1);
      if (km >= 0 && ne >= 0) v = w[(size_t)km + ne];
    }
    tile[kk * ld + n] = v;
  }
  __syncthreads();
  bf16* o = out + (size_t)blk * BN * 64;
  for (int idx = threadIdx.x; idx < BN * 64; idx += blockDim.x) {
    const int pos = idx & 63, n = idx >> 6;
    const int kk = (((pos >> 3) ^ (n & 7)) << 3) | (pos & 7);
    o[idx] = __float2bfloat16(tile[kk * ld + n]);
  }
}
__device__ __forceinline__ void unpack_wgrad_body(size_t i, const float* __restrict__ dwp, const int* __restrict__ kmap, int K_pad, int cout,
                                                  int nsplit, float* __restrict__ dw, const float* __restrict__ colpart, int nblocks, int nch,
                                                  float* __restrict__ db, int layout) {
  const size_t nw = (size_t)cout * K_pad;
  if (i < nw) {
    const size_t sn = (layout >> 8) ? (size_t)(layout >> 8) : 1;
    int n, k;
    if ((layout & 0xff) == 0) {
      n = (int)(i / K_pad);
      k = (int)(i % K_pad);
    } else {
      const size_t g4 = i / ((size_t)cout * 4);
      const int rem = (int)(i - g4 * cout * 4);
      n = rem >> 2;
      k = (int)g4 * 4 + (rem & 3);
    }
    const int km = kmap[k];
    if (km < 0) return;
    float a[8] = {0.f, 0.f, 0.f, 0.f, 0.f, 0.f, 0.f, 0.f};
    const float* q = dwp + i;
    int s = 0;
    for (; s + 8 <= nsplit; s += 8) {
      float t[8];
#pragma unroll
      for (int u = 0; u < 8; ++u) t[u] = __ldcg(q + (size_t)(s + u) * nw);
#pragma unroll
      for (int u = 0; u < 8; ++u) a[u] += t[u];
    }
    for (; s < nsplit; ++s) a[0] += __ldcg(q + (size_t)s * nw);
    dw[(size_t)km + n * sn] = ((a[0] + a[1]) + (a[2] + a[3])) + ((a[4] + a[5]) + (a[6] + a[7]));
  } else if (colpart != nullptr && i - nw < (size_t)nch) {
    const int c = (int)(i - nw);
    float a = 0.f;
    for (int b = 0; b < nblocks; ++b) a += __ldcg(colpart + (size_t)b * nch + c);
    db[c] = a;
  }
}
#define BN_RSQRT 0.99950037468777323f
__device__ __forceinline__ void bn_fold_body(size_t i, const float* __restrict__ w, const float* __restrict__ bias, const float* __restrict__ gamma,
                                             const float* __restrict__ beta, size_t nw, int cout, float* __restrict__ w_eff,
                                             float* __restrict__ b_eff) {
  if (i < nw) w_eff[i] = w[i] * gamma[i % cout] * BN_RSQRT;
  if (i < (size_t)cout) b_eff[i] = bias[i] * gamma[i] * BN_RSQRT + beta[i];
}
static constexpr int kBnChainCo = 8;
__device__ __forceinline__ void bn_chain_body(int blk, const float* __restrict__ w, const float* __restrict__ bias, const float* __restrict__ gamma,
                                              float* __restrict__ dwe, const float* __restrict__ dbe, size_t nw, int cout,
                                              float* __restrict__ dbias, float* __restrict__ dgamma, float* __restrict__ dbeta, float* red) {
  const int rows = (int)(nw / cout);
  const int cl = threadIdx.x & 7, rl = threadIdx.x >> 3;
  const int co = blk * kBnChainCo + cl;
  const bool ok = co < cout;
  float acc = 0.f;
  if (ok)
    for (int r = rl; r < rows; r += 32) acc += dwe[(size_t)r * cout + co] * w[(size_t)r * cout + co];
  red[rl * 8 + cl] = acc;
  __syncthreads();
  float g = 0.f;
  if (ok) {
    g = gamma[co] * BN_RSQRT;
    if (rl == 0) {
      float v = 0.f;
      for (int q = 0; q < 32; ++q) v += red[q * 8 + cl];
      dgamma[co] = BN_RSQRT * (v + dbe[co] * bias[co]);
      dbias[co] = dbe[co] * g;
      dbeta[co] = dbe[co];
    }
    for (int r = rl; r < rows; r += 32) dwe[(size_t)r * cout + co] *= g;
  }
}
__global__ void pack_weights_kernel(const float* __restrict__ w, const int* __restrict__ kmap, int K_pad, int rows, int cout, int sn,
                                    const int* __restrict__ nmap, bf16* __restrict__ wp) {
  pdl_launch_dependents();
  pdl_wait();
  pack_weights_body((size_t)blockIdx.x * blockDim.x + threadIdx.x, w, kmap, K_pad, rows, cout, sn, nmap, wp);
}
__global__ void pack_weights_tiled_kernel(const float* __restrict__ w, const int* __restrict__ kmap, int cin8, int ntaps, int n_tiles, int BN,
                                          int cout, int sn, const int* __restrict__ nmap, bf16* __restrict__ out) {
  pdl_launch_dependents();
  pdl_wait();
  __shared__ float tile[64 * 129];
  if (sn == 1) pack_weights_tiled_tile(blockIdx.x, w, kmap, cin8, ntaps, n_tiles, BN, cout, nmap, out, tile);
  else pack_weights_tiled_body((size_t)blockIdx.x * blockDim.x + threadIdx.x, w, kmap, cin8, ntaps, n_tiles, BN, cout, sn, nmap, out);
}
__global__ void unpack_wgrad_kernel(const float* __restrict__ dwp, const int* __restrict__ kmap, int K_pad, int cout, int nsplit,
                                    float* __restrict__ dw, const float* __restrict__ colpart, int nblocks, int nch, float* __restrict__ db,
                                    int layout) {
  pdl_launch_dependents();
  pdl_wait();
  unpack_wgrad_body((size_t)blockIdx.x * blockDim.x + threadIdx.x, dwp, kmap, K_pad, cout, nsplit, dw, colpart, nblocks, nch, db, layout);
}
__global__ void bn_fold_kernel(const float* __restrict__ w, const float* __restrict__ bias, const float* __restrict__ gamma,
                               const float* __restrict__ beta, size_t nw, int cout, float* __restrict__ w_eff, float* __restrict__ b_eff) {
  pdl_launch_dependents();
  pdl_wait();
  bn_fold_body((size_t)blockIdx.x * blockDim.x + threadIdx.x, w, bias, gamma, beta, nw, cout, w_eff, b_eff);
}
__global__ void bn_chain_kernel(const float* __restrict__ w, const float* __restrict__ bias, const float* __restrict__ gamma,
                                float* __restrict__ dwe, const float* __restrict__ dbe, size_t nw, int cout, float* __restrict__ dbias,
                                float* __restrict__ dgamma, float* __restrict__ dbeta) {
  pdl_launch_dependents();
  pdl_wait();
  __shared__ float red[256];
  bn_chain_body(blockIdx.x, w, bias, gamma, dwe, dbe, nw, cout, dbias, dgamma, dbeta, red);
}
__global__ void param_multi_kernel(const CisParamJob* __restrict__ jobs, int njobs) {
  pdl_launch_dependents();
  pdl_wait();
  int lo = 0, hi = njobs - 1;
  while (lo < hi) {
    const int mid = (lo + hi + 1) >> 1;
    if (jobs[mid].i[7] <= (int)blockIdx.x) lo = mid; else hi = mid - 1;
  }
  const CisParamJob j = jobs[lo];
  const int blk = (int)blockIdx.x - j.i[7];
  const size_t i = (size_t)blk * blockDim.x + threadIdx.x;
  __shared__ float red[256];
  __shared__ float tile[64 * 129];
  switch (j.kind) {
    case CIS_JOB_PACK:
      pack_weights_body(i, (const float*)j.p[0], (const int*)j.p[1], j.i[0], j.i[1], j.i[2], j.i[3], (const int*)j.p[2], (bf16*)j.p[3]);
      break;
    case CIS_JOB_PACK_TILED:
      if (j.i[5] == 1)
        pack_weights_tiled_tile(blk, (const float*)j.p[0], (const int*)j.p[1], j.i[0], j.i[1], j.i[2], j.i[3], j.i[4], (const int*)j.p[2],
                                (bf16*)j.p[3], tile);
      else
        pack_weights_tiled_body(i, (const float*)j.p[0], (const int*)j.p[1], j.i[0], j.i[1], j.i[2], j.i[3], j.i[4], j.i[5], (const int*)j.p[2],
                                (bf16*)j.p[3]);
      break;
    case CIS_JOB_UNPACK:
      unpack_wgrad_body(i, (const float*)j.p[0], (const int*)j.p[1], j.i[0], j.i[1], j.i[2], (float*)j.p[2], (const float*)j.p[3], j.i[3], j.i[4],
                        (float*)j.p[4], j.i[5]);
      break;
    case CIS_JOB_BN_FOLD:
      bn_fold_body(i, (const float*)j.p[0], (const float*)j.p[1], (const float*)j.p[2], (const float*)j.p[3], (size_t)j.n, j.i[0], (float*)j.p[4],
                   (float*)j.p[5]);
      break;
    case CIS_JOB_BN_CHAIN:
      bn_chain_body(blk, (const float*)j.p[0], (const float*)j.p[1], (const float*)j.p[2], (float*)j.p[3], (const float*)j.p[4], (size_t)j.n,
                    j.i[0], (float*)j.p[5], (float*)j.p[6], (float*)j.p[7], red);
      break;
  }
}

__global__ void dact_mul_kernel(bf16* g, int gp, int gc, const bf16* __restrict__ y, int yp, int yc, const bf16* __restrict__ res, int rp,
                                int rc, size_t npix, int chunks, int act, float alpha) {
  pdl_launch_dependents();
  pdl_wait();
  const size_t i = (size_t)blockIdx.x * blockDim.x + threadIdx.x;
  if (i >= npix * chunks) return;
  const size_t pix = i / chunks;
  const int c = (int)(i % chunks) * 8;
  uint4* gpp = reinterpret_cast<uint4*>(g + pix * gp + gc + c);
  float gv[8], yv[8], rv[8];
  unpack8(*gpp, gv);
  unpack8(*reinterpret_cast<const uint4*>(y + pix * yp + yc + c), yv);
  if (res) {
    unpack8(*reinterpret_cast<const uint4*>(res + pix * rp + rc + c), rv);
#pragma unroll
    for (int e = 0; e < 8; ++e) yv[e] -= rv[e];
  }
#pragma unroll
  for (int e = 0; e < 8; ++e) {
    const float u = yv[e];
    const float d = (act == CIS_ACT_ELU) ? (u > 0.f ? 1.f : u + 1.f) : (u > 0.f ? 1.f : alpha);
    gv[e] *= d;
  }
  *gpp = pack8(gv);
}
__global__ void add_slice_kernel(bf16* dst, int dp, int dc, const bf16* __restrict__ src, int sp, int sc, size_t npix, int chunks, int reps,
                                 int accumulate) {
  pdl_launch_dependents();
  pdl_wait();
  const size_t i = (size_t)blockIdx.x * blockDim.x + threadIdx.x;
  if (i >= npix * chunks) return;
  const size_t pix = i / chunks;
  const int c = (int)(i % chunks) * 8;
  float a[8] = {0, 0, 0, 0, 0, 0, 0, 0}, t[8];
  uint4* d = reinterpret_cast<uint4*>(dst + pix * dp + dc + c);
  if (accumulate) unpack8(*d, a);
  for (int j = 0; j < reps; ++j) {
    unpack8(*reinterpret_cast<const uint4*>(src + (pix + (size_t)j * npix) * sp + sc + c), t);
#pragma unroll
    for (int e = 0; e < 8; ++e) a[e] += t[e];
  }
  *d = pack8(a);
}
__global__ void colsum_kernel(const bf16* __restrict__ g, int gp, int gc, size_t npix, int nch, int chunks, float* __restrict__ part) {
  pdl_launch_dependents();
  pdl_wait();
  extern __shared__ float sm[];
  const int P = blockDim.x / chunks;
  const int ck = threadIdx.x % chunks, pl = threadIdx.x / chunks;
  float a[8] = {0, 0, 0, 0, 0, 0, 0, 0}, t[8];
  if (pl < P) {
    for (size_t p = (size_t)blockIdx.x * P + pl; p < npix; p += (size_t)gridDim.x * P) {
      unpack8(*reinterpret_cast<const uint4*>(g + p * gp + gc + ck * 8), t);
#pragma unroll
      for (int e = 0; e < 8; ++e) a[e] += t[e];
    }
#pragma unroll
    for (int e = 0; e < 8; ++e) sm[pl * chunks * 8 + ck * 8 + e] = a[e];
  }
  __syncthreads();
  for (int c = threadIdx.x; c < nch; c += blockDim.x) {
    float s = 0.f;
// ... 1334 lines not shown
  if (!attr) {
    cudaError_t e = cudaFuncSetAttribute(warp_costvol_kernel<R>, cudaFuncAttributeMaxDynamicSharedMemorySize, cv_smem(R));
    if (e != cudaSuccess) return cis_set_cuda_error(e, "cudaFuncSetAttribute(warp_costvol)");
    attr = true;
  }
  dim3 grid((w + kCvTW - 1) / kCvTW, (h + kCvTH - 1) / kCvTH, B);
  CIS_LAUNCH(warp_costvol_kernel<R>, grid, 256, cv_smem(R), ST, (cbf)c1, c1p, c1o, (cbf)c2, c2p, c2o, flow, fs, B, h, w, C, (mbf)out, op, oo);
  return cis_check_launch("warp_costvol");
}
template <int R>
static int cost_volume_bwd(const void* c1, int32_t c1p, int32_t c1o, const void* warp, int32_t wp, int32_t wo, const float* dout, int32_t B,
                           int32_t h, int32_t w, int32_t C, float* gscratch, float* dc1, float* dwarp, cis_stream_t stream) {
  if (h < 2 || w < 2) return cis_set_error(CIS_ERR_BAD_ARG, "cis_cost_volume_bwd: needs h,w >= 2 (core_warp.py:188)");
  if (!gscratch || !dc1 || !dwarp) return cis_set_error(CIS_ERR_BAD_ARG, "cis_cost_volume_bwd: NULL output or scratch");
  static bool attr = false;
  if (!attr) {
    cudaError_t e = cudaFuncSetAttribute(costvol_bwd_gate_kernel<R, float>, cudaFuncAttributeMaxDynamicSharedMemorySize, cv_smem(R));
    if (e == cudaSuccess) e = cudaFuncSetAttribute(costvol_bwd_kernel<R, F32Out, F32Out>, cudaFuncAttributeMaxDynamicSharedMemorySize, cv_bwd_smem(R));
    if (e != cudaSuccess) return cis_set_cuda_error(e, "cudaFuncSetAttribute(costvol_bwd)");
    attr = true;
  }
  dim3 grid((w + kCvTW - 1) / kCvTW, (h + kCvTH - 1) / kCvTH, B);
  CIS_LAUNCH((costvol_bwd_gate_kernel<R, float>), grid, 256, cv_smem(R), ST, (cbf)c1, c1p, c1o, (cbf)warp, wp, wo, (const float*)nullptr, 1.f, dout,
             cv_ndisp(R), 0, B, h, w, C, gscratch);
  CIS_LAUNCH((costvol_bwd_kernel<R, F32Out, F32Out>), grid, 256, cv_bwd_smem(R), ST, (cbf)c1, c1p, c1o, (cbf)warp, wp, wo, (const float*)nullptr,
             1.f, (const float*)gscratch, B, h, w, C, F32Out{dc1, C, 0}, F32Out{dwarp, C, 0});
  return cis_check_launch("cost_volume_bwd");
}
template <int R>
static int warp_costvol_bwd(const void* c1, int32_t c1p, int32_t c1o, const void* c2, int32_t c2p, int32_t c2o, const float* flow, float fs,
                            int32_t B, int32_t h, int32_t w, int32_t C, const void* dcorr, int32_t dcp, int32_t dco, void* dc1, int32_t dc1p,
                            int32_t dc1o, void* dc2, int32_t dc2p, int32_t dc2o, void* dflow, int32_t dfp, int32_t dfo, int32_t accumulate,
                            float* gscratch, float* wscratch, double* dscratch, cis_stream_t stream) {
  if (h < 2 || w < 2) return cis_set_error(CIS_ERR_BAD_ARG, "cis_warp_costvol_bwd: needs h,w >= 2 (core_warp.py:188)");
  if (!dcorr || !dc1 || !dc2 || !gscratch) return cis_set_error(CIS_ERR_BAD_ARG, "cis_warp_costvol_bwd: NULL gradient or scratch");
  if (flow && (!dflow || !wscratch || !dscratch)) return cis_set_error(CIS_ERR_BAD_ARG, "cis_warp_costvol_bwd: the warp needs dflow and scratch");
  if ((c1p | c1o | c2p | c2o) & 7) return cis_set_error(CIS_ERR_BAD_ARG, "cis_warp_costvol_bwd: feature slices must be 8-channel aligned");
  static bool attr = false;
  if (!attr) {
    cudaError_t e = cudaFuncSetAttribute(costvol_bwd_gate_kernel<R, bf16>, cudaFuncAttributeMaxDynamicSharedMemorySize, cv_smem(R));
    if (e == cudaSuccess)
      e = cudaFuncSetAttribute(costvol_bwd_kernel<R, Bf16Out, F32Out>, cudaFuncAttributeMaxDynamicSharedMemorySize, cv_bwd_smem(R));
    if (e == cudaSuccess)
      e = cudaFuncSetAttribute(costvol_bwd_kernel<R, Bf16Out, Bf16Out>, cudaFuncAttributeMaxDynamicSharedMemorySize, cv_bwd_smem(R));
    if (e != cudaSuccess) return cis_set_cuda_error(e, "cudaFuncSetAttribute(warp_costvol_bwd)");
    attr = true;
  }
  const Bf16Out o1{(mbf)dc1, dc1p, dc1o, accumulate & 1}, o2{(mbf)dc2, dc2p, dc2o, (accumulate >> 1) & 1};
  dim3 grid((w + kCvTW - 1) / kCvTW, (h + kCvTH - 1) / kCvTH, B);
  CIS_LAUNCH((costvol_bwd_gate_kernel<R, bf16>), grid, 256, cv_smem(R), ST, (cbf)c1, c1p, c1o, (cbf)c2, c2p, c2o, flow, fs, (cbf)dcorr, dcp, dco, B,
             h, w, C, gscratch);
  if (!flow) {
    CIS_LAUNCH((costvol_bwd_kernel<R, Bf16Out, Bf16Out>), grid, 256, cv_bwd_smem(R), ST, (cbf)c1, c1p, c1o, (cbf)c2, c2p, c2o, flow, fs,
               (const float*)gscratch, B, h, w, C, o1, o2);
    return cis_check_launch("warp_costvol_bwd");
  }
  CIS_LAUNCH((costvol_bwd_kernel<R, Bf16Out, F32Out>), grid, 256, cv_bwd_smem(R), ST, (cbf)c1, c1p, c1o, (cbf)c2, c2p, c2o, flow, fs,
             (const float*)gscratch, B, h, w, C, o1, F32Out{wscratch, C, 0});
  const size_t npix = (size_t)B * h * w;
  cudaError_t e = cudaMemsetAsync(dscratch, 0, npix * C * sizeof(double), ST);
  if (e != cudaSuccess) return cis_set_cuda_error(e, "cudaMemsetAsync");
  CIS_LAUNCH(dense_image_warp_bwd_kernel<Bf16Out>, nblk(npix), 256, 0, ST, (cbf)c2, c2p, c2o, flow, fs, B, h, w, C, (const float*)wscratch, dscratch,
             Bf16Out{(mbf)dflow, dfp, dfo, (accumulate >> 2) & 1});
  CIS_LAUNCH(round_f64_kernel<Bf16Out>, nblk(npix * C), 256, 0, ST, (const double*)dscratch, npix, C, o2);
  return cis_check_launch("warp_costvol_bwd");
}
#define CIS_CV_DISPATCH(fn, what, ...)                                                                                  \
  switch (search_range) {                                                                                              \
    case 1: return fn<1>(__VA_ARGS__);                                                                                 \
    case 2: return fn<2>(__VA_ARGS__);                                                                                 \
    case 3: return fn<3>(__VA_ARGS__);                                                                                 \
    case 4: return fn<4>(__VA_ARGS__);                                                                                 \
    default: return cis_set_error(CIS_ERR_BAD_ARG, what ": search_range must be 1, 2, 3 or 4");                       \
  }

extern "C" {

int cis_pack_weights(const float* w, const int32_t* kmap, int32_t K_pad, int32_t rows, int32_t cout, int32_t sn, const int32_t* nmap, void* wp,
                     cis_stream_t stream) {
  CIS_LAUNCH(pack_weights_kernel, nblk((size_t)rows * K_pad), 256, 0, ST, w, kmap, K_pad, rows, cout, sn, nmap, (mbf)wp);
  return cis_check_launch("pack_weights");
}
int cis_pack_weights_tiled(const float* w, const int32_t* kmap, int32_t cin8, int32_t ntaps, int32_t n_tiles, int32_t BN, int32_t cout, int32_t sn,
                           const int32_t* nmap, void* out, cis_stream_t stream) {
  const size_t total = (size_t)n_tiles * ((cin8 + 63) / 64) * ntaps * BN * 64;
  const unsigned blocks = sn == 1 ? (unsigned)(n_tiles * ((cin8 + 63) / 64) * ntaps) : nblk(total);
  if (BN > 128) return cis_set_error(CIS_ERR_UNSUPPORTED, "cis_pack_weights_tiled: BN > 128");
  CIS_LAUNCH(pack_weights_tiled_kernel, blocks, 256, 0, ST, w, kmap, cin8, ntaps, n_tiles, BN, cout, sn, nmap, (mbf)out);
  return cis_check_launch("pack_weights_tiled");
}
int cis_unpack_wgrad(const float* dwp, const int32_t* kmap, int32_t K_pad, int32_t cout, int32_t nsplit, float* dw, const float* colpart,
                     int32_t nblocks, int32_t nch, float* db, int32_t layout, cis_stream_t stream) {
  if (nsplit < 1 || (colpart && (nblocks < 1 || !db)) || ((layout & 0xff) != 0 && (layout & 0xff) != 1) || layout < 0 || K_pad % 4)
    return cis_set_error(CIS_ERR_BAD_ARG, "cis_unpack_wgrad: bad split / column-sum / layout arguments");
  CIS_LAUNCH(unpack_wgrad_kernel, nblk((size_t)cout * K_pad + (colpart ? nch : 0)), 256, 0, ST, dwp, kmap, K_pad, cout, nsplit, dw, colpart, nblocks,
             nch, db, layout);
  return cis_check_launch("unpack_wgrad");
}
int cis_param_multi(const CisParamJob* jobs_dev, int32_t njobs, int32_t total_blocks, cis_stream_t stream) {
  if (!jobs_dev || njobs < 1 || total_blocks < 1) return cis_set_error(CIS_ERR_BAD_ARG, "cis_param_multi: bad job table");
  CIS_LAUNCH(param_multi_kernel, (unsigned)total_blocks, 256, 0, ST, jobs_dev, njobs);
  return cis_check_launch("param_multi");
}
int cis_bn_fold(const float* w, const float* bias, const float* gamma, const float* beta, int64_t nw, int32_t cout, float* w_eff, float* b_eff,
                cis_stream_t stream) {
  CIS_LAUNCH(bn_fold_kernel, nblk((size_t)nw), 256, 0, ST, w, bias, gamma, beta, (size_t)nw, cout, w_eff, b_eff);
  return cis_check_launch("bn_fold");
}
int cis_bn_chain(const float* w, const float* bias, const float* gamma, float* dwe, const float* dbe, int64_t nw, int32_t cout, float* dbias,
                 float* dgamma, float* dbeta, cis_stream_t stream) {
  CIS_LAUNCH(bn_chain_kernel, (unsigned)((cout + kBnChainCo - 1) / kBnChainCo), 256, 0, ST, w, bias, gamma, dwe, dbe, (size_t)nw, cout, dbias, dgamma, dbeta);
  return cis_check_launch("bn_chain");
}
int cis_dact_mul(void* g, int32_t gp, int32_t gc, const void* y, int32_t yp, int32_t yc, const void* res, int32_t rp, int32_t rc, int64_t npix,
                 int32_t chunks, int32_t act, float alpha, cis_stream_t stream) {
  if (act == CIS_ACT_NONE) return CIS_OK;
  CIS_LAUNCH(dact_mul_kernel, nblk((size_t)npix * chunks), 256, 0, ST, (mbf)g, gp, gc, (cbf)y, yp, yc, (cbf)res, rp, rc, (size_t)npix, chunks, act, alpha);
  return cis_check_launch("dact_mul");
}
int cis_add_slice(void* dst, int32_t dp, int32_t dc, const void* src, int32_t sp, int32_t sc, int64_t npix, int32_t chunks, int32_t reps,
                  int32_t accumulate, cis_stream_t stream) {
  CIS_LAUNCH(add_slice_kernel, nblk((size_t)npix * chunks), 256, 0, ST, (mbf)dst, dp, dc, (cbf)src, sp, sc, (size_t)npix, chunks, reps, accumulate);
  return cis_check_launch("add_slice");
}
int cis_colsum(const void* g, int32_t gp, int32_t gc, int64_t npix, int32_t nch, float* part, int32_t nblocks, cis_stream_t stream) {
  const int chunks = (nch + 7) / 8;
  if (chunks > 32) return cis_set_error(CIS_ERR_UNSUPPORTED, "cis_colsum: more than 256 channels");
  if (nblocks < 1 || nblocks > 592) return cis_set_error(CIS_ERR_BAD_ARG, "cis_colsum: nblocks must be in [1, 592]");
  const int P = 256 / chunks;
  CIS_LAUNCH(colsum_kernel, (unsigned)nblocks, 256, P * chunks * 8 * sizeof(float), ST, (cbf)g, gp, gc, (size_t)npix, nch, chunks, part);
  return cis_check_launch("colsum");
}
int cis_zero(void* ptr, int64_t nbytes, cis_stream_t stream) {
  if (!ptr || nbytes < 0) return cis_set_error(CIS_ERR_BAD_ARG, "cis_zero: bad buffer");
  cudaError_t e = cudaMemsetAsync(ptr, 0, (size_t)nbytes, ST);
  if (e != cudaSuccess) return cis_set_cuda_error(e, "cudaMemsetAsync");
  return CIS_OK;
}
int cis_dact_colsum(void* g, int32_t gp, int32_t gc, const void* y, int32_t yp, int32_t yc, const void* res, int32_t rp, int32_t rc, int64_t npix,
                    int32_t nch, int32_t act, float alpha, float* part, int32_t nblocks, cis_stream_t stream) {
  const int chunks = (nch + 7) / 8;
  if (act == CIS_ACT_NONE) return cis_colsum(g, gp, gc, npix, nch, part, nblocks, stream);
  if (chunks > 32) return cis_set_error(CIS_ERR_UNSUPPORTED, "cis_dact_colsum: more than 256 channels");
  if (nblocks < 1 || nblocks > 592) return cis_set_error(CIS_ERR_BAD_ARG, "cis_dact_colsum: nblocks must be in [1, 592]");
  const int P = 256 / chunks;
  CIS_LAUNCH(dact_colsum_kernel, (unsigned)nblocks, 256, P * chunks * 8 * sizeof(float), ST, (mbf)g, gp, gc, (cbf)y, yp, yc, (cbf)res, rp, rc,
             (size_t)npix, nch, chunks, act, alpha, part);
  return cis_check_launch("dact_colsum");
}
int cis_resize_bilinear_bf16(const void* src, int32_t sp, int32_t sc, int32_t N, int32_t H, int32_t W, void* dst, int32_t dp, int32_t dc, int32_t OH,
                             int32_t OW, int32_t chunks, cis_stream_t stream) {
  CIS_LAUNCH(resize_bilinear_bf16_kernel, nblk((size_t)N * OH * OW * chunks), 256, 0, ST, (cbf)src, sp, sc, N, H, W, (mbf)dst, dp, dc, OH, OW, chunks);
  return cis_check_launch("resize_bilinear_bf16");
}
int cis_resize_bilinear_bf16_bwd(const void* dd, int32_t dp, int32_t dc, int32_t N, int32_t OH, int32_t OW, void* ds, int32_t sp, int32_t sc, int32_t H,
                                 int32_t W, int32_t chunks, int32_t accumulate, cis_stream_t stream) {
  CIS_LAUNCH(resize_bilinear_bf16_bwd_kernel, nblk((size_t)N * H * W * chunks), 256, 0, ST, (cbf)dd, dp, dc, N, OH, OW, (mbf)ds, sp, sc, H, W, chunks,
                                                                                     accumulate);
  return cis_check_launch("resize_bilinear_bf16_bwd");
}
int cis_resize_concat_bf16(const CisSrc* srcs, int32_t nsrc, int32_t N, int32_t H, int32_t W, void* dst, int32_t dp, int32_t dc, int32_t OH, int32_t OW,
                           cis_stream_t stream) {
  if (!srcs || nsrc < 1 || nsrc > CIS_MAX_SRC) return cis_set_error(CIS_ERR_BAD_ARG, "cis_resize_concat_bf16: 1..4 sources");
  RcArgs a;
  a.nsrc = nsrc;
  int total = 0;
  for (int i = 0; i < nsrc; ++i) {
    a.s[i] = srcs[i];
    if ((srcs[i].pitch | srcs[i].c_off) & 7) return cis_set_error(CIS_ERR_BAD_ARG, "cis_resize_concat_bf16: slices must be 8-channel aligned");
    total += srcs[i].chunks;
  }
// ... 292 lines not shown
```

unsupervised_detection_b200/csrc/ptx.cuh:

```cuda
#pragma once
#include <cuda_runtime.h>
#include <cuda_bf16.h>
#include <stdint.h>

namespace cis {

__device__ __forceinline__ uint32_t smem_u32(const void* p) {
  return static_cast<uint32_t>(__cvta_generic_to_shared(p));
}

__device__ __forceinline__ void mbar_init(uint32_t bar, uint32_t count) {
  asm volatile("mbarrier.init.shared::cta.b64 [%0], %1;" ::"r"(bar), "r"(count) : "memory");
}
__device__ __forceinline__ void fence_mbar_init() {
  asm volatile("fence.mbarrier_init.release.cluster;" ::: "memory");
}
__device__ __forceinline__ void mbar_arrive(uint32_t bar) {
  asm volatile("{\n\t.reg .b64 st;\n\tmbarrier.arrive.shared::cta.b64 st, [%0];\n\t}" ::"r"(bar) : "memory");
}
__device__ __forceinline__ void mbar_expect_tx(uint32_t bar, uint32_t bytes) {
  asm volatile("{\n\t.reg .b64 st;\n\tmbarrier.arrive.expect_tx.shared::cta.b64 st, [%0], %1;\n\t}" ::"r"(bar), "r"(bytes)
               : "memory");
}
__device__ __forceinline__ bool mbar_try_wait(uint32_t bar, uint32_t parity) {
// ... 33 lines not shown
}
__device__ __forceinline__ void tma_load_4d(uint32_t dst, const void* tmap, uint32_t bar, int c0, int c1, int c2, int c3) {
  asm volatile(
      "cp.async.bulk.tensor.4d.shared::cluster.global.mbarrier::complete_tx::bytes [%0], [%1, {%3, %4, %5, %6}], [%2];" ::"r"(dst),
      "l"(tmap), "r"(bar), "r"(c0), "r"(c1), "r"(c2), "r"(c3)
      : "memory");
}
__device__ __forceinline__ void bulk_g2s(uint32_t dst, const void* src, uint32_t bytes, uint32_t bar) {
  asm volatile("cp.async.bulk.shared::cluster.global.mbarrier::complete_tx::bytes [%0], [%1], %2, [%3];" ::"r"(dst), "l"(src), "r"(bytes),
               "r"(bar)
               : "memory");
}
__device__ __forceinline__ uint32_t cluster_ctarank() {
  uint32_t r;
  asm volatile("mov.u32 %0, %%cluster_ctarank;" : "=r"(r));
  return r;
}
__device__ __forceinline__ void cluster_sync_all() {
  asm volatile("barrier.cluster.arrive.release.aligned;\n\tbarrier.cluster.wait.acquire.aligned;" ::: "memory");
}
__device__ __forceinline__ uint32_t dsmem_addr(uint32_t saddr, uint32_t rank) {
  uint32_t r;
  asm volatile("mapa.shared::cluster.u32 %0, %1, %2;" : "=r"(r) : "r"(saddr), "r"(rank));
  return r;
}
__device__ __forceinline__ float4 dsmem_ld4(uint32_t caddr) {
  float4 v;
  asm volatile("ld.shared::cluster.v4.f32 {%0, %1, %2, %3}, [%4];" : "=f"(v.x), "=f"(v.y), "=f"(v.z), "=f"(v.w) : "r"(caddr) : "memory");
  return v;
}
__device__ __forceinline__ void tma_prefetch_desc(const void* tmap) {
  asm volatile("prefetch.tensormap [%0];" ::"l"(tmap) : "memory");
}

__device__ __forceinline__ void pdl_launch_dependents() { asm volatile("griddepcontrol.launch_dependents;" ::: "memory"); }
__device__ __forceinline__ void pdl_wait() { asm volatile("griddepcontrol.wait;" ::: "memory"); }

__device__ __forceinline__ void wg_fence() { asm volatile("wgmma.fence.sync.aligned;" ::: "memory"); }
__device__ __forceinline__ void wg_commit() { asm volatile("wgmma.commit_group.sync.aligned;" ::: "memory"); }
template <int N>
__device__ __forceinline__ void wg_wait() {
  asm volatile("wgmma.wait_group.sync.aligned %0;" ::"n"(N) : "memory");
}

template <int N, int TA, int TB> struct Wgmma;
template <int TA, int TB> struct Wgmma<16, TA, TB> {
  static __device__ __forceinline__ void mma(float (&d)[8], uint64_t da, uint64_t db, uint32_t scale_d) {
    asm volatile(
        "{\n\t.reg .pred p;\n\tsetp.ne.b32 p, %10, 0;\n\t"
        "wgmma.mma_async.sync.aligned.m64n16k16.f32.bf16.bf16 {%0,%1,%2,%3,%4,%5,%6,%7}, %8, %9, p, 1, 1, %11, %12;\n\t}"
        : "+f"(d[0]), "+f"(d[1]), "+f"(d[2]), "+f"(d[3]), "+f"(d[4]), "+f"(d[5]), "+f"(d[6]), "+f"(d[7])
        : "l"(da), "l"(db), "r"(scale_d), "n"(TA), "n"(TB));
  }
};
template <int TA, int TB> struct Wgmma<32, TA, TB> {
  static __device__ __forceinline__ void mma(float (&d)[16], uint64_t da, uint64_t db, uint32_t scale_d) {
    asm volatile(
        "{\n\t.reg .pred p;\n\tsetp.ne.b32 p, %18, 0;\n\t"
        "wgmma.mma_async.sync.aligned.m64n32k16.f32.bf16.bf16 {%0,%1,%2,%3,%4,%5,%6,%7,%8,%9,%10,%11,%12,%13,%14,%15}, %16, %17, p, 1, 1, %19, %20;\n\t}"
        : "+f"(d[0]), "+f"(d[1]), "+f"(d[2]), "+f"(d[3]), "+f"(d[4]), "+f"(d[5]), "+f"(d[6]), "+f"(d[7]), "+f"(d[8]), "+f"(d[9]), "+f"(d[10]), "+f"(d[11]), "+f"(d[12]), "+f"(d[13]), "+f"(d[14]), "+f"(d[15])
        : "l"(da), "l"(db), "r"(scale_d), "n"(TA), "n"(TB));
  }
};
template <int TA, int TB> struct Wgmma<64, TA, TB> {
  static __device__ __forceinline__ void mma(float (&d)[32], uint64_t da, uint64_t db, uint32_t scale_d) {
    asm volatile(
        "{\n\t.reg .pred p;\n\tsetp.ne.b32 p, %34, 0;\n\t"
        "wgmma.mma_async.sync.aligned.m64n64k16.f32.bf16.bf16 {%0,%1,%2,%3,%4,%5,%6,%7,%8,%9,%10,%11,%12,%13,%14,%15,%16,%17,%18,%19,%20,%21,%22,%23,%24,%25,%26,%27,%28,%29,%30,%31}, %32, %33, p, 1, 1, %35, %36;\n\t}"
        : "+f"(d[0]), "+f"(d[1]), "+f"(d[2]), "+f"(d[3]), "+f"(d[4]), "+f"(d[5]), "+f"(d[6]), "+f"(d[7]), "+f"(d[8]), "+f"(d[9]), "+f"(d[10]), "+f"(d[11]), "+f"(d[12]), "+f"(d[13]), "+f"(d[14]), "+f"(d[15]), "+f"(d[16]), "+f"(d[17]), "+f"(d[18]), "+f"(d[19]), "+f"(d[20]), "+f"(d[21]), "+f"(d[22]), "+f"(d[23]), "+f"(d[24]), "+f"(d[25]), "+f"(d[26]), "+f"(d[27]), "+f"(d[28]), "+f"(d[29]), "+f"(d[30]), "+f"(d[31])
        : "l"(da), "l"(db), "r"(scale_d), "n"(TA), "n"(TB));
  }
};
template <int TA, int TB> struct Wgmma<128, TA, TB> {
  static __device__ __forceinline__ void mma(float (&d)[64], uint64_t da, uint64_t db, uint32_t scale_d) {
    asm volatile(
        "{\n\t.reg .pred p;\n\tsetp.ne.b32 p, %66, 0;\n\t"
        "wgmma.mma_async.sync.aligned.m64n128k16.f32.bf16.bf16 {%0,%1,%2,%3,%4,%5,%6,%7,%8,%9,%10,%11,%12,%13,%14,%15,%16,%17,%18,%19,%20,%21,%22,%23,%24,%25,%26,%27,%28,%29,%30,%31,%32,%33,%34,%35,%36,%37,%38,%39,%40,%41,%42,%43,%44,%45,%46,%47,%48,%49,%50,%51,%52,%53,%54,%55,%56,%57,%58,%59,%60,%61,%62,%63}, %64, %65, p, 1, 1, %67, %68;\n\t}"
        : "+f"(d[0]), "+f"(d[1]), "+f"(d[2]), "+f"(d[3]), "+f"(d[4]), "+f"(d[5]), "+f"(d[6]), "+f"(d[7]), "+f"(d[8]), "+f"(d[9]), "+f"(d[10]), "+f"(d[11]), "+f"(d[12]), "+f"(d[13]), "+f"(d[14]), "+f"(d[15]), "+f"(d[16]), "+f"(d[17]), "+f"(d[18]), "+f"(d[19]), "+f"(d[20]), "+f"(d[21]), "+f"(d[22]), "+f"(d[23]), "+f"(d[24]), "+f"(d[25]), "+f"(d[26]), "+f"(d[27]), "+f"(d[28]), "+f"(d[29]), "+f"(d[30]), "+f"(d[31]), "+f"(d[32]), "+f"(d[33]), "+f"(d[34]), "+f"(d[35]), "+f"(d[36]), "+f"(d[37]), "+f"(d[38]), "+f"(d[39]), "+f"(d[40]), "+f"(d[41]), "+f"(d[42]), "+f"(d[43]), "+f"(d[44]), "+f"(d[45]), "+f"(d[46]), "+f"(d[47]), "+f"(d[48]), "+f"(d[49]), "+f"(d[50]), "+f"(d[51]), "+f"(d[52]), "+f"(d[53]), "+f"(d[54]), "+f"(d[55]), "+f"(d[56]), "+f"(d[57]), "+f"(d[58]), "+f"(d[59]), "+f"(d[60]), "+f"(d[61]), "+f"(d[62]), "+f"(d[63])
        : "l"(da), "l"(db), "r"(scale_d), "n"(TA), "n"(TB));
  }
};

__device__ __forceinline__ uint32_t desc_hi(uint32_t sbo_bytes) { return ((sbo_bytes >> 4) & 0x3FFF) | (1u << 30); }
__device__ __forceinline__ uint32_t desc_lo(uint32_t saddr, uint32_t lbo_bytes) {
  return ((saddr & 0x3FFFF) >> 4) | (((lbo_bytes >> 4) & 0x3FFF) << 16);
}

template <int N, int TA, int TB>
__device__ __forceinline__ void mma128(float (&acc)[N], uint32_t alo, uint32_t ahi, uint32_t blo, uint32_t bhi, uint32_t a_half,
                                       uint32_t scale_d) {
  const uint64_t db = ((uint64_t)bhi << 32) | blo;
  Wgmma<N, TA, TB>::mma(*reinterpret_cast<float(*)[N / 2]>(&acc[0]), ((uint64_t)ahi << 32) | alo, db, scale_d);
  Wgmma<N, TA, TB>::mma(*reinterpret_cast<float(*)[N / 2]>(&acc[N / 2]), ((uint64_t)ahi << 32) | (alo + a_half), db, scale_d);
}

static constexpr uint32_t kAccColBytes = 512;
template <int N>
__device__ __forceinline__ void acc_store(const float (&acc)[N], uint32_t base, int wtid) {
  const int w = wtid >> 5, lane = wtid & 31;
  const int c2 = 2 * (lane & 3);
#pragma unroll
  for (int h = 0; h < 2; ++h) {
    const int row = 64 * h + 16 * w + (lane >> 2);
#pragma unroll
    for (int i = 0; i < N / 8; ++i) {
      const int col = 8 * i + c2;
      const uint32_t a = base + (uint32_t)((col >> 2) * 2048 + row * 16 + (col & 3) * 4);
      asm volatile("st.shared.v2.f32 [%0], {%1, %2};" ::"r"(a), "f"(acc[h * (N / 2) + 4 * i]), "f"(acc[h * (N / 2) + 4 * i + 1]) : "memory");
      asm volatile("st.shared.v2.f32 [%0], {%1, %2};" ::"r"(a + 8 * 16), "f"(acc[h * (N / 2) + 4 * i + 2]), "f"(acc[h * (N / 2) + 4 * i + 3])
                   : "memory");
    }
  }
}
__device__ __forceinline__ void acc_ld16(uint32_t addr, float* v) {
#pragma unroll
  for (int h = 0; h < 4; ++h)
    asm volatile("ld.shared.v4.f32 {%0, %1, %2, %3}, [%4];"
                 : "=f"(v[4 * h]), "=f"(v[4 * h + 1]), "=f"(v[4 * h + 2]), "=f"(v[4 * h + 3])
                 : "r"(addr + (uint32_t)h * 2048)
                 : "memory");
}

__device__ __forceinline__ float bf16lo(uint32_t u) { return __uint_as_float(u << 16); }
__device__ __forceinline__ float bf16hi(uint32_t u) { return __uint_as_float(u & 0xFFFF0000u); }
__device__ __forceinline__ uint32_t pack_bf16(float a, float b) {
  __nv_bfloat162 t = __floats2bfloat162_rn(a, b);
  return *reinterpret_cast<uint32_t*>(&t);
}

}
```

unsupervised_detection_b200/engine.py:

```python
import ctypes as C
import dataclasses
import os

import numpy as np
import torch

from . import _lib
from ._lib import CisConv, CisWgrad, CisSrc, ACT_NONE, ACT_ELU, ACT_LEAKY


def ru(x, m):
    return (x + m - 1) // m * m


def same_pad(n_in, k, s=1, d=1):
    out = -(-n_in // s)
    total = max((out - 1) * s + (k - 1) * d + 1 - n_in, 0)
    return total // 2, total - total // 2


SIDE_STREAM = True
_SIDE = {}
MULTI_PARAM_OPS = os.environ.get('CIS_MULTI_PARAM', '1') == '1'
DACT_COLSUM = os.environ.get('CIS_DACT_COLSUM', '1') == '1'
# ... 7 lines not shown
        _SIDE[k] = torch.cuda.Stream(device=device)
    return _SIDE[k]


class Plan(object):

    def __init__(self, name=''):
        self.name = name
        self.ops = []
        self.keep = []

    def add(self, fname, *args, flops=0.0, lane=0):
        fn = getattr(_lib.load(), fname)
        self.ops.append((fn, args, fname, flops, lane))

    def add_py(self, fn, label='py'):
        self.ops.append((None, fn, label, 0.0, 0))

    def zero(self, t):
        self.keep.append(t)
        self.add('cis_zero', t.data_ptr(), t.numel() * t.element_size())

    def join(self):
        self.ops.append((None, None, 'join', 0.0, 0))

    def run(self, stream=None, lane_key=0):
        if stream is not None or not SIDE_STREAM or not any(op[4] for op in self.ops):
            st = stream if stream is not None else torch.cuda.current_stream().cuda_stream
            for fn, args, name, _, _ in self.ops:
                if fn is None:
                    if args is not None:
                        args()
                else:
                    rc = fn(*args, st)
                    if rc != 0:
                        _lib.check(rc, name)
            return
        main = torch.cuda.current_stream()
        side = _side_stream(main.device, lane_key)
        st0, st1 = main.cuda_stream, side.cuda_stream
        main_ahead, side_used = True, False
        for fn, args, name, _, lane in self.ops:
            if fn is None:
                if name == 'join':
                    if side_used:
                        ev = torch.cuda.Event()
                        ev.record(side)
                        main.wait_event(ev)
                        side_used = False
                elif args is not None:
                    args()
                    main_ahead = True
                continue
            if lane == 1:
                if main_ahead:
                    ev = torch.cuda.Event()
                    ev.record(main)
                    side.wait_event(ev)
                    main_ahead = False
                rc = fn(*args, st1)
                side_used = True
            else:
                rc = fn(*args, st0)
                main_ahead = True
            if rc != 0:
                _lib.check(rc, name)
        if side_used:
            ev = torch.cuda.Event()
            ev.record(side)
            main.wait_event(ev)

    def batch_param_ops(self, device):
        from ._lib import CisParamJob, JOB_PACK, JOB_PACK_TILED, JOB_UNPACK, JOB_BN_FOLD, JOB_BN_CHAIN
        if not MULTI_PARAM_OPS or not self.ops:
            return self
        jobs = {k: [] for k in range(5)}
        for fn, a, name, _, _ in self.ops:
            j = CisParamJob()
            if name == 'cis_pack_weights':
                w, kmap, K_pad, rows, cout, sn, nmap, wp = a
                j.kind, blocks = JOB_PACK, -(-(rows * K_pad) // 256)
                ptrs, ints = [w, kmap, nmap, wp], [K_pad, rows, cout, sn]
            elif name == 'cis_pack_weights_tiled':
                w, kmap, cin8, ntaps, n_tiles, BN, cout, sn, nmap, out = a
                j.kind, blocks = JOB_PACK_TILED, -(-(n_tiles * (-(-cin8 // 64)) * ntaps * BN * 64) // 256)
                if sn == 1:
                    blocks = n_tiles * (-(-cin8 // 64)) * ntaps
                ptrs, ints = [w, kmap, nmap, out], [cin8, ntaps, n_tiles, BN, cout, sn]
            elif name == 'cis_unpack_wgrad':
                dwp, kmap, K_pad, cout, nsplit, dw, colpart, nblocks, nch, db, layout = a
                j.kind, blocks = JOB_UNPACK, -(-(cout * K_pad + nch) // 256)
                ptrs, ints = [dwp, kmap, dw, colpart, db], [K_pad, cout, nsplit, nblocks, nch, layout]
            elif name == 'cis_bn_fold':
                w, bias, gamma, beta, nw, cout, w_eff, b_eff = a
                j.kind, blocks, j.n = JOB_BN_FOLD, -(-max(nw, cout) // 256), nw
                ptrs, ints = [w, bias, gamma, beta, w_eff, b_eff], [cout]
            elif name == 'cis_bn_chain':
                w, bias, gamma, dwe, dbe, nw, cout, dbias, dgamma, dbeta = a
                j.kind, blocks, j.n = JOB_BN_CHAIN, -(-cout // 8), nw
                ptrs, ints = [w, bias, gamma, dwe, dbe, dbias, dgamma, dbeta], [cout]
            else:
                return self
            for q, v in enumerate(ptrs):
                j.p[q] = v
            for q, v in enumerate(ints):
                j.i[q] = v
            jobs[j.kind].append((j, blocks))
        out = Plan(self.name + '.multi')
        out.keep = self.keep
        for kind in (JOB_BN_FOLD, JOB_PACK_TILED, JOB_PACK, JOB_UNPACK, JOB_BN_CHAIN):
            if not jobs[kind]:
                continue
            arr = (CisParamJob * len(jobs[kind]))()
            first = 0
            for q, (j, blocks) in enumerate(jobs[kind]):
                j.i[7] = first
                arr[q] = j
                first += blocks
            tab = torch.frombuffer(bytearray(bytes(arr)), dtype=torch.uint8).to(device)
            out.keep.append(tab)
            out.add('cis_param_multi', tab.data_ptr(), len(jobs[kind]), first)
        return out

    def count(self):
        n = 0
        for fn, args, name, _, _ in self.ops:
            if fn is None or name == 'cis_zero':
                continue
            n += 1
            if name == 'cis_conv_igemm':
                d = args[0]._obj
                if d.splits > 1 and not d.sk_cluster:
                    n += 1
        return n

    def extend(self, other):
        self.ops += other.ops
        self.keep += other.keep


class Act(object):

    def __init__(self, N, H, W, C, device, buf=None, c_off=0, chanmap=None, n_mod=0, dep=frozenset(), name=''):
        if chanmap is not None and not C:
            C = max(chanmap) + 1
        self.N, self.H, self.W, self.C = N, H, W, C
        self.C8 = ru(C, 8) if chanmap is None else len(chanmap)
        if buf is None:
            buf = torch.zeros(N, H, W, self.C8, dtype=torch.bfloat16, device=device)
        self.buf = buf
        self.pitch = buf.shape[-1]
        self.c_off = c_off
        self.chanmap = list(chanmap) if chanmap is not None else list(range(C)) + [-1] * (self.C8 - C)
        self.n_mod = n_mod
        self.dep = frozenset(dep)
        self.name = name
        self.grad = None
        self.grad_written = {}
        self.device = device
        self.gen_rows = None
        self.grad_buf = None
        self._owner = None

    @property
    def ptr(self):
        return self.buf.data_ptr()

    def src(self):
        return CisSrc(self.ptr, self.pitch, self.c_off, self.C8 // 8, self.n_mod)

    def rows(self, mode):
# ... 166 lines not shown
def setup_splitk(d, device, keep):
    if not SPLITK:
        return
    m_chunks = sum(d.src[i].chunks for i in range(d.nsrc))
    if d.halo:
        Hp0, Wp0 = -(-d.OH // d.dil), -(-d.OW // d.dil)
        mt = d.MT * max(d.nwg, 1)
        tiles = (-(-Wp0 // 8)) * (-(-Hp0 // (16 * mt))) * d.dil * d.dil * d.N
        ncta, units, min_units = tiles * d.n_tiles, -(-m_chunks // 8), 1
    else:
        ncta, units, min_units, mt = (-(-(d.N * d.OH * d.OW) // 128)) * d.n_tiles, d.K_pad // 64, 4, 1
    steps = units * (d.ntaps if d.halo else 1)
    if ncta > SPLITK_NCTA or steps < SPLITK_MIN_UNITS:
        return
    splits = min(units // min_units, -(-2 * NUM_SMS // ncta), SPLITK_MAX, 8 if SPLITK_CLUSTER else 1 << 30)
    if splits < 2:
        return
    per = -(-units // splits)
    splits = -(-units // per)
    if splits < 2:
        return
    if SPLITK_CLUSTER and splits <= 8 and mt * 128 * d.BN * 4 + 1024 <= 226 * 1024:
        d.splits, d.sk_scratch, d.sk_counters, d.sk_cluster = splits, None, None, 1
        return
    sc = torch.empty(ncta * mt * splits * 128 * d.BN, dtype=torch.float32, device=device)
    keep.append(sc)
    d.splits, d.sk_scratch, d.sk_counters = splits, sc.data_ptr(), None


def setup_halo(d, taps, dil, n_tiles):
    if not HALO_ENABLED or d.sh != 1 or d.sw != 1:
        return False
    if any(a % dil or b % dil for a, b in taps):
        return False
    if dil > 1 and (d.OH != d.H or d.OW != d.W):
        return False
    th = [(a // dil, b // dil) for a, b in taps]
    hoy, hox = min(a for a, _ in th), min(b for _, b in th)
    rel = [(a - hoy, b - hox) for a, b in th]
    ey, ex = max(a for a, _ in rel), max(b for _, b in rel)
    Hp0, Wp0 = -(-d.OH // dil), -(-d.OW // dil)
    tiles_x = -(-Wp0 // 8)
    best = None
    ntaps = len(taps)
    m_chunks = sum(d.src[i].chunks for i in range(d.nsrc))
    if HALO_SKIP_THIN and m_chunks * 8 <= HALO_SKIP_THIN and ntaps >= 16:
        return False
    nchunks = -(-m_chunks // 8)
    nhs = 2 if nchunks > 1 else 1
    force = int(os.environ.get('CIS_FORCE_MT128', '0')) if d.BN == 128 else 0
    for MT in (1, 2, 3, 4):
        if MT * d.BN > MAX_ACC_COLS or (force and MT != force):
            continue
        HP = (8 + ex) * (16 * MT + ey)
        fixed = nhs * ru(HP * 128, 1024) + HP * 4 + 1024
        smem = fixed + min(3, ntaps * nchunks) * d.BN * 128 + 1024
        if smem > 227 * 1024:
            continue
        tiles_y = -(-Hp0 // (16 * MT))
        util = (Hp0 * Wp0) / float(tiles_y * 16 * MT * tiles_x * 8)
        if util < (HALO_MIN_UTIL if dil == 1 else 0.5):
            continue
        ncta = d.N * dil * dil * tiles_x * tiles_y * n_tiles
        cps = max(1, min((225 * 1024) // smem, 6))
        t_mma = MT * 2.0 * d.BN * ntaps * nchunks
        t_mem = (d.BN * 128 * ntaps / 40.0 + HP * 128 / 16.0) * nchunks
        t_cta = max(t_mma, t_mem) + (4000.0 + 1500.0 * MT) / cps
        cost = -(-ncta // (NUM_SMS * cps)) * cps * t_cta / min(cps, max(1.0, ncta / float(NUM_SMS)))
        if PLAN_MODEL == 2:
            per_sm = -(-ncta // NUM_SMS)
            cost = per_sm * max(t_mma, t_mem) + (4000.0 + 1500.0 * MT) * (-(-per_sm // cps))
        if PLAN_MODEL == 3:
            cost = float(MT)
        if PLAN_MODEL == 4:
            n1 = d.N * dil * dil * tiles_x * (-(-Hp0 // 16)) * n_tiles
            if not (2.0 * d.BN * ntaps * nchunks < 6000.0 and n1 > 4 * NUM_SMS):
                cost = float(MT)
        if best is None or cost < best[0] - 1e-9:
            best = (cost, MT, util)
    if best is None:
        return False
    d.halo, d.dil, d.MT, d.hoy, d.hox, d.ey, d.ex = 1, dil, best[1], hoy, hox, ey, ex
    d.nwg = halo_nwg(d, best[1], Hp0, Wp0, dil, n_tiles, ntaps, nchunks, ey, ex)
    _fill_taps(d, rel)
    return True


S2_HALO = os.environ.get('CIS_S2_HALO', '0') == '1'


def setup_halo_s2(d, taps, n_tiles):
    if not (HALO_ENABLED and S2_HALO) or d.sh != 2 or d.sw != 2:
        return None
    if any(d.src[i].chunks % 8 for i in range(d.nsrc - 1)):
        return None
    ph = [((u % 2) * 2 + (v % 2), u // 2, v // 2) for u, v in taps]
    order = sorted(range(len(taps)), key=lambda i: (ph[i][0], i))
    hoy, hox = min(a for _, a, _ in ph), min(b for _, _, b in ph)
    rel = [(ph[i][1] - hoy, ph[i][2] - hox) for i in order]
    ey, ex = max(a for a, _ in rel), max(b for _, b in rel)
    m_chunks = sum(d.src[i].chunks for i in range(d.nsrc))
    nchunks = -(-m_chunks // 8)
    tiles_x = -(-d.OW // 8)
    best = None
    for MT in (1, 2, 3, 4):
        if MT * d.BN > MAX_ACC_COLS:
            continue
        HP = (8 + ex) * (16 * MT + ey)
        smem = 2 * ru(HP * 128, 1024) + HP * 4 + 2048 + 2 * d.BN * 128
        if smem > 227 * 1024:
            continue
        tiles_y = -(-d.OH // (16 * MT))
        util = (d.OH * d.OW) / float(tiles_y * 16 * MT * tiles_x * 8)
        if util < HALO_MIN_UTIL:
            continue
        ncta = d.N * tiles_x * tiles_y * n_tiles
        cps = max(1, min((225 * 1024) // smem, 4))
        t_mma = MT * 2.0 * d.BN * len(taps) * nchunks
        t_mem = (d.BN * 128 * len(taps) / 40.0 + 4 * HP * 128 / 40.0) * nchunks
        t_cta = max(t_mma, t_mem) + (4000.0 + 1500.0 * MT) / cps
        cost = -(-ncta // (NUM_SMS * cps)) * cps * t_cta / min(cps, max(1.0, ncta / float(NUM_SMS)))
        if best is None or cost < best[0] - 1e-9:
            best = (cost, MT)
    if best is None:
        return None
    d.halo, d.dil, d.MT, d.hoy, d.hox, d.ey, d.ex = 1, 1, best[1], hoy, hox, ey, ex
    d.nwg = halo_nwg(d, best[1], d.OH, d.OW, 1, n_tiles, len(taps), nchunks, ey, ex)
    d.sh = d.sw = 1
    _fill_taps(d, rel)
    d.nph = 4
    bounds = [0]
    for q in range(4):
        bounds.append(bounds[-1] + sum(1 for i in order if ph[i][0] == q))
    for q in range(5):
        d.ph_tap[q] = bounds[q]
    return order


GROUP_PARITY = os.environ.get('CIS_GROUP_PARITY', '1') == '1'
GROUP_PARITY_MAX_TILES = int(os.environ.get('CIS_GROUP_PARITY_MAX_TILES', '1000000'))


def merge_parity_launches(descs):
    if not GROUP_PARITY or not (2 <= len(descs) <= 4):
        return None
    d0 = descs[0]
    same = ('N', 'H', 'W', 'BN', 'n_tiles', 'nsrc', 'act', 'DH', 'DW', 'osh', 'osw', 'out', 'out_pitch', 'out_coff', 'out_ch', 'outf', 'outf_pitch',
            'outf_coff', 'outf_ch', 'add_pre', 'add_pre_pitch', 'add_pre_coff', 'add_post', 'addf_pre', 'mode', 'bias')
    for d in descs:
        if not d.halo or d.dil != 1 or d.splits > 1 or d.nph > 1 or any(getattr(d, f) != getattr(d0, f) for f in same):
            return None
        if any(bytes(d.src[i]) != bytes(d0.src[i]) for i in range(d0.nsrc)):
            return None
    if sum(d.ntaps for d in descs) > _lib.MAX_TAPS:
        return None
    if max(d.N * (-(-d.OH // 16)) * (-(-d.OW // 8)) for d in descs) > GROUP_PARITY_MAX_TILES:
        return None
    g = CisConv.from_buffer_copy(bytes(d0))
    g.MT, g.ey, g.ex = min(d.MT for d in descs), max(d.ey for d in descs), max(d.ex for d in descs)
    g.nwg = min(max(d.nwg, 1) for d in descs)
    g.OH, g.OW = max(d.OH for d in descs), max(d.OW for d in descs)
    t = 0
    for i, d in enumerate(descs):
        for k in range(d.ntaps):
            g.dh[t + k], g.dw[t + k] = d.dh[k], d.dw[k]
        sb = g.sub[i]
        sb.tap0, sb.ntaps, sb.hoy, sb.hox, sb.OH, sb.OW, sb.oa, sb.ob, sb.wpack = t, d.ntaps, d.hoy, d.hox, d.OH, d.OW, d.oa, d.ob, d.wpack
        t += d.ntaps
    m_chunks = sum(g.src[i].chunks for i in range(g.nsrc))
    g.ntaps, g.nsub, g.splits, g.K_pad = t, len(descs), 0, ru(t * m_chunks * 8, 64)
    return g


class ParamStore(object):

    def __init__(self, device):
        self.device = device
        self.entries = []
        self.index = {}
        self.size = 0
        self.flat = None

    def declare(self, name, shape, padded=None):
        n = int(np.prod(shape))
        pn = ru(padded or n, 4)
        self.index[name] = len(self.entries)
        self.entries.append((name, tuple(shape), n, self.size, pn))
        self.size += pn

    def finalize(self, trainable):
        self.flat = torch.zeros(self.size, dtype=torch.float32, device=self.device)
        if trainable:
            self.grad = torch.zeros_like(self.flat)
            self.m = torch.zeros_like(self.flat)
            self.v = torch.zeros_like(self.flat)
            seg = [0]
            for _, _, n, off, _ in self.entries:
                seg.append(off + n)
            self.seg_pairs = [(off, off + n) for _, _, n, off, _ in self.entries]

    def off(self, name):
        return self.entries[self.index[name]][3]

    def ptr(self, name, which='flat'):
        return getattr(self, which).data_ptr() + 4 * self.off(name)

    def view(self, name, which='flat'):
        _, shape, n, off, _ = self.entries[self.index[name]]
        return getattr(self, which)[off:off + n].view(shape)

    def load(self, params):
        for name, shape, n, off, _ in self.entries:
            if name not in params:
                raise KeyError('missing parameter ' + name)
            t = params[name].detach().to(torch.float32).reshape(-1)
            if t.numel() != n:
                raise ValueError('shape mismatch for %s: %d vs %d' % (name, t.numel(), n))
            self.flat[off:off + n].copy_(t)

    def export(self, which='flat'):
        return {name: getattr(self, which)[off:off + n].view(shape).clone() for name, shape, n, off, _ in self.entries}

    def real_count(self):
        return sum(e[2] for e in self.entries)


@dataclasses.dataclass(eq=False)
class Pack:
    a: int = 0
    b: int = 0
    taps: list = dataclasses.field(default_factory=list)
    kmap: torch.Tensor = None
    K_pad: int = 0
    rows: int = 0
    BN: int = 0
    n_tiles: int = 0
    nmap: torch.Tensor = None
    w: torch.Tensor = None
    wt: torch.Tensor = None
    wt_kmap: torch.Tensor = None
    rows_used: bool = None
    wg_splits: dict = dataclasses.field(default_factory=dict)
    dwp: torch.Tensor = None

    def __getitem__(self, field):
        return getattr(self, field)


def _ptr(t):
    return t.data_ptr() if t is not None else None


def _parity_taps(k, s, d, pt, pl, a, b):
    rows = [r for r in range(k) if (a + pt - r * d) % s == 0]
    cols = [c for c in range(k) if (b + pl - c * d) % s == 0]
    return [r * k + c for r in rows for c in cols], [((a + pt - r * d) // s, (b + pl - c * d) // s) for r in rows for c in cols]


class ConvLayer(object):

    def __init__(self, store, name, k, cin, cout, stride=1, dil=1, act=ACT_NONE, alpha=0.2, tag='', bn=False,
                 wname='kernel', bname='bias', transposed=False, bn_cap=None):
        self.store, self.name, self.k, self.cin, self.cout = store, name, k, cin, cout
        self.stride, self.dil, self.act, self.alpha, self.tag, self.bn = stride, dil, act, alpha, tag, bn
        self.transposed = transposed
        self.bn_cap = bn_cap
        self.BN, self.n_tiles = pick_bn(cout, bn_cap)
        self.npad = self.BN * self.n_tiles
        self.wkey, self.bkey = '%s/%s' % (name, wname), '%s/%s' % (name, bname)
        if transposed:
            store.declare(self.wkey, (k, k, cout, cin))
        else:
            store.declare(self.wkey, (k, k, cin, cout))
        store.declare(self.bkey, (cout,), padded=self.npad)
        if bn:
            store.declare('%s/gamma' % name, (cout,))
            store.declare('%s/beta' % name, (cout,))
        self.device = store.device
        self.in_chanmap = None
        self.fwd_kmap, self.K_pad = None, 0
        self.fwd_pack = None
        self.tr_packs = None
        self.dgrad_packs = None
        self.tr_dgrad = None
        self.dgrad_used = False
        self.w_eff = self.b_eff = self.db_eff = None
        self.ncalls = 0
        self.colpart, self.col_blocks = None, {}
        self.tr_planes = None
        self.dcat = None
        self.wg_tma = self.wg_halo = False
        self.wg_kmap, self.wg_K_pad = None, 0
        self.dwp, self.wg_splits = None, {}
        self.dwp_hi, self.wg_splits_hi = {}, {}
        self.wgrad_modes = set()

    def _kmap(self, taps_idx, chanmap, per_tap_stride, chan_stride):
        m = len(chanmap)
        K = len(taps_idx) * m
        Kp = ru(max(K, (len(taps_idx) - 1) * m + ru(m, 64)), 64)
        km = np.full(Kp, -1, dtype=np.int32)
        cm = np.asarray(chanmap, dtype=np.int64)
        for ti, t in enumerate(taps_idx):
            v = np.where(cm >= 0, t * per_tap_stride + cm * chan_stride, -1)
            km[ti * m:(ti + 1) * m] = v
        return torch.from_numpy(km).to(self.device), Kp

    def _rows(self, rows, K_pad):
        return torch.zeros(rows, K_pad, dtype=torch.bfloat16, device=self.device)

    def setup_fwd(self, chanmap):
        assert max(chanmap) == self.cin - 1, (self.name, max(chanmap), self.cin)
        self.in_chanmap = list(chanmap)
        kk = self.k * self.k
        if self.transposed:
            raise RuntimeError('use setup_transposed')
        self.fwd_kmap, self.K_pad = self._kmap(range(kk), chanmap, self.cin * self.cout, self.cout)
        self.fwd_pack = Pack(taps=list(range(kk)), kmap=self.fwd_kmap, K_pad=self.K_pad, rows=self.npad, BN=self.BN, n_tiles=self.n_tiles,
                             w=self._rows(self.npad, self.K_pad))
        if self.bn:
            self.w_eff = torch.zeros(kk * self.cin * self.cout, dtype=torch.float32, device=self.device)
            self.b_eff = torch.zeros(self.npad, dtype=torch.float32, device=self.device)
            self.db_eff = torch.zeros(self.npad, dtype=torch.float32, device=self.device)

    def _alloc_tiles(self, ntaps, cin8, BN, n_tiles):
        nchunks = -(-cin8 // 64)
        return torch.zeros(n_tiles * nchunks * ntaps * BN * 64, dtype=torch.bfloat16, device=self.device)

    def place(self, d, pk, taps, dil, kch, order=None):
        if order is None and not setup_halo(d, taps, dil, pk.n_tiles):
            pk.rows_used = True
            return
        if pk.wt is None:
            pk.wt = self._alloc_tiles(len(taps), kch, pk.BN, pk.n_tiles)
            if order is not None:
                pk.taps = list(order)
                pk.wt_kmap, _ = self._kmap(pk.taps, self.in_chanmap, self.cin * self.cout, self.cout)
        assert order is None or pk.taps == list(order), self.name
        d.wpack = pk.wt.data_ptr()
        if pk.rows_used is None:
            pk.rows_used = False

    def w_src_ptr(self):
        return self.w_eff.data_ptr() if self.bn else self.store.ptr(self.wkey)

    def bias_ptr(self):
        return self.b_eff.data_ptr() if self.bn else self.store.ptr(self.bkey)

    def plan_pack(self, plan, dgrad=False):
        s = self.store
        if self.bn:
            plan.add('cis_bn_fold', s.ptr(self.wkey), s.ptr(self.bkey), s.ptr(self.name + '/gamma'), s.ptr(self.name + '/beta'),
                     self.k * self.k * self.cin * self.cout, self.cout, self.w_eff.data_ptr(), self.b_eff.data_ptr())
        cin8 = len(self.in_chanmap or ())
        packs = [(pk, cin8, self.cout, self.cin) for pk in self.tr_packs or ()]
        packs += [(pk, cin8, self.cout, 1) for pk in (self.fwd_pack,) if pk is not None]
        if dgrad:
            packs += [(pk, cin8, cin8, 1) for pk in (self.tr_dgrad,) if pk is not None]
            packs += [(pk, ru(self.cout, 8), cin8, self.cout) for pk in self.dgrad_packs or ()]
        for pk, kch, nch, sn in packs:
            if pk.wt is not None:
                plan.add('cis_pack_weights_tiled', self.w_src_ptr(), (pk.kmap if pk.wt_kmap is None else pk.wt_kmap).data_ptr(), kch,
                         len(pk.taps), pk.n_tiles, pk.BN, nch, sn, _ptr(pk.nmap), pk.wt.data_ptr())
            if pk.rows_used is not False:
                plan.add('cis_pack_weights', self.w_src_ptr(), pk.kmap.data_ptr(), pk.K_pad, pk.rows, nch, sn, _ptr(pk.nmap), pk.w.data_ptr())

    def plan_finalize(self, bp, mode):
        s = self.store
        if self.transposed:
            for q, pk in enumerate(p for p in self.tr_packs or () if mode in p.wg_splits):
                bp.add('cis_unpack_wgrad', pk.dwp.data_ptr(), pk.kmap.data_ptr(), pk.K_pad, self.cout, pk.wg_splits[mode],
                       s.ptr(self.wkey, 'grad'), self.colpart.data_ptr() if q == 0 else None, self.col_blocks[mode] if q == 0 else 0,
                       self.cout if q == 0 else 0, s.ptr(self.bkey, 'grad') if q == 0 else None, 1 | (self.cin << 8))
            return
        if mode not in self.wg_splits:
            return
        bp.add('cis_unpack_wgrad', self.dwp.data_ptr(), self.wg_kmap.data_ptr(), self.wg_K_pad, min(128, self.cout), self.wg_splits[mode],
               s.ptr(self.wkey, 'grad'), self.colpart.data_ptr(), self.col_blocks[mode], self.cout,
               (self.db_eff.data_ptr() if self.bn else s.ptr(self.bkey, 'grad')), 0 if self.wg_halo else 1)
        for g0, buf in sorted(self.dwp_hi.items()):
            if (mode, g0) in self.wg_splits_hi:
                bp.add('cis_unpack_wgrad', buf.data_ptr(), self.wg_kmap.data_ptr(), self.wg_K_pad, min(128, self.cout - g0),
                       self.wg_splits_hi[(mode, g0)], s.ptr(self.wkey, 'grad') + 4 * g0, None, 0, 0, None, 0 if self.wg_halo else 1)
        if self.bn:
            bp.add('cis_bn_chain', s.ptr(self.wkey), s.ptr(self.bkey), s.ptr(self.name + '/gamma'), s.ptr(self.wkey, 'grad'),
                   self.db_eff.data_ptr(), self.k * self.k * self.cin * self.cout, self.cout, s.ptr(self.bkey, 'grad'),
                   s.ptr(self.name + '/gamma', 'grad'), s.ptr(self.name + '/beta', 'grad'))

    def fwd_taps(self, H, W):
        pt, _ = same_pad(H, self.k, self.stride, self.dil)
        pl, _ = same_pad(W, self.k, self.stride, self.dil)
        return [(r * self.dil - pt, c * self.dil - pl) for r in range(self.k) for c in range(self.k)], pt, pl

    def setup_wgrad(self, taps, srcs):
        if self.wg_kmap is not None:
            return
        cin8 = len(self.in_chanmap)
        aligned = all(s.C8 % 64 == 0 for s in srcs[:-1])
        self.wg_tma = bool(WGRAD_TMA and self.stride == 1 and cin8 >= 32 and aligned)
        self.wg_halo = bool(WGRAD_HALO and cin8 >= WGRAD_HALO_MIN_CH and wgrad_halo_fits(taps, self.cout, self.stride) and aligned)
        if not (self.wg_tma or self.wg_halo):
            self.wg_K_pad, self.wg_kmap = self.K_pad, self.fwd_kmap
            return
        nch64 = -(-cin8 // 64)
        self.wg_K_pad = ru(self.k * self.k * nch64 * 64, 128)
        km = np.full(self.wg_K_pad, -1, dtype=np.int32)
        fk = self.fwd_kmap.cpu().numpy()
        for t in range(self.k * self.k):
            for pos in range(cin8):
                km[(t * nch64 + pos // 64) * 64 + pos % 64] = fk[t * cin8 + pos]
        self.wg_kmap = torch.from_numpy(km).to(self.device)

    def setup_dgrad(self, H, W):
        if self.dgrad_packs is not None:
            return
        _, pt, pl = self.fwd_taps(H, W)
        k, s, d = self.k, self.stride, self.dil
        g_chan = list(range(self.cout)) + [-1] * (ru(self.cout, 8) - self.cout)
        cin8 = len(self.in_chanmap)
        bn_, nt = pick_bn(cin8, self.bn_cap)
        rows = bn_ * nt
        nmap = torch.tensor(list(self.in_chanmap) + [-1] * (rows - cin8), dtype=torch.int32, device=self.device)
        packs = []
        for a in range(s):
            for b in range(s):
                tl, offs = _parity_taps(k, s, d, pt, pl, a, b)
                if not tl:
                    packs.append(Pack(a=a, b=b, rows_used=False))
                    continue
                kmap, Kp = self._kmap(tl, g_chan, self.cin * self.cout, 1)
                packs.append(Pack(a=a, b=b, taps=offs, kmap=kmap, K_pad=Kp, rows=rows, BN=bn_, n_tiles=nt, nmap=nmap, w=self._rows(rows, Kp)))
        self.dgrad_packs = packs

    def setup_transposed(self, chanmap):
        assert self.transposed and self.k == 4
        self.in_chanmap = list(chanmap)
        packs = []
        for a in range(2):
            for b in range(2):
                tl, offs = _parity_taps(4, 2, 1, 1, 1, a, b)
                kmap, Kp = self._kmap(tl, chanmap, self.cout * self.cin, 1)
                packs.append(Pack(a=a, b=b, taps=offs, kmap=kmap, K_pad=Kp, rows=self.npad, BN=self.BN, n_tiles=self.n_tiles,
                                  w=self._rows(self.npad, Kp)))
        self.tr_packs = packs

    def setup_transposed_dgrad(self, g_pos):
# ... 367 lines not shown
```

Before: 619.4.

## Add thin non-swizzled halo layout for convs with 8 or 16 input channels

Adds a 'thin' mode for halo implicit-GEMM convolutions whose input has only one or two 8-channel chunks. The halo is loaded as 16-byte-per-pixel planes with a non-swizzled descriptor instead of 128-byte padded pixels. For 8 channels, pairs of taps are packed into a single K=16 MMA step, which roughly halves the step count and shrinks the weight stages. The goal is to stop wasting TMA bandwidth, shared memory and MMA work on zero-padded channels in the first layers. It also adds per-subproblem tile decoding to the persistent kernel and a thin weight packing path; the risk is correctness in the new descriptor and tap-pairing logic.

```diff
diff --git a/include/cis_b200.h b/include/cis_b200.h
--- a/include/cis_b200.h
+++ b/include/cis_b200.h
@@ -69,6 +69,7 @@
     const void* wpack;
   } sub[4];
   int32_t nwg;
+  int32_t thin;
 } CisConv;
 
 typedef struct {
@@ -101,7 +102,7 @@
 int cis_pack_weights(const float* w, const int32_t* kmap, int32_t K_pad, int32_t rows, int32_t cout, int32_t sn, const int32_t* nmap,
                      void* wp, cis_stream_t stream);
 int cis_pack_weights_tiled(const float* w, const int32_t* kmap, int32_t cin8, int32_t ntaps, int32_t n_tiles, int32_t BN, int32_t cout,
-                           int32_t sn, const int32_t* nmap, void* out, cis_stream_t stream);
+                           int32_t sn, const int32_t* nmap, void* out, int32_t thin, cis_stream_t stream);
 int cis_unpack_wgrad(const float* dwp, const int32_t* kmap, int32_t K_pad, int32_t cout, int32_t nsplit, float* dw, const float* colpart,
                      int32_t nblocks, int32_t nch, float* db, int32_t layout, cis_stream_t stream);
 int cis_bn_fold(const float* w, const float* bias, const float* gamma, const float* beta, int64_t nw, int32_t cout, float* w_eff,
diff --git a/unsupervised_detection_b200/_lib.py b/unsupervised_detection_b200/_lib.py
--- a/unsupervised_detection_b200/_lib.py
+++ b/unsupervised_detection_b200/_lib.py
@@ -43,7 +43,7 @@
                 ('ey', C.c_int32), ('ex', C.c_int32),
                 ('splits', C.c_int32), ('sk_scratch', C.c_void_p), ('sk_counters', C.c_void_p),
                 ('nph', C.c_int32), ('ph_tap', C.c_int32 * 5), ('sk_cluster', C.c_int32),
-                ('nsub', C.c_int32), ('sub', CisSub * 4), ('nwg', C.c_int32)]
+                ('nsub', C.c_int32), ('sub', CisSub * 4), ('nwg', C.c_int32), ('thin', C.c_int32)]
 
 
 class CisWgrad(C.Structure):
@@ -62,7 +62,7 @@
     'cis_conv_igemm': [C.POINTER(CisConv)],
     'cis_conv_wgrad': [C.POINTER(CisWgrad)],
     'cis_pack_weights': [_p, _p, _i32, _i32, _i32, _i32, _p, _p],
-    'cis_pack_weights_tiled': [_p, _p, _i32, _i32, _i32, _i32, _i32, _i32, _p, _p],
+    'cis_pack_weights_tiled': [_p, _p, _i32, _i32, _i32, _i32, _i32, _i32, _p, _p, _i32],
     'cis_unpack_wgrad': [_p, _p, _i32, _i32, _i32, _p, _p, _i32, _i32, _p, _i32],
     'cis_bn_fold': [_p, _p, _p, _p, _i64, _i32, _p, _p],
     'cis_param_multi': [_p, _i32, _i32],
diff --git a/unsupervised_detection_b200/csrc/conv_igemm.cu b/unsupervised_detection_b200/csrc/conv_igemm.cu
--- a/unsupervised_detection_b200/csrc/conv_igemm.cu
+++ b/unsupervised_detection_b200/csrc/conv_igemm.cu
@@ -514,8 +514,7 @@
 template <int NK, int MT, int BN, int MTM>
 __device__ __forceinline__ void halo_issue_stage(float (&acc)[MTM][BN], const uint32_t hlo, uint32_t blo, const uint32_t* s_aoff, const int gt,
                                                  const uint32_t ahi, const uint32_t bhi, const uint32_t a_mstep, const uint32_t a_half,
-                                                 const bool first) {
-  const uint32_t bstep = (uint32_t)(BN * 128) >> 4;
+                                                 const uint32_t bstep, const bool first) {
   uint32_t off0 = s_aoff[0], off1 = gt > 1 ? s_aoff[1] : 0u;
   int tt = 0;
 #pragma unroll 1
@@ -538,26 +537,37 @@
 template <int MT, int BN, int MTM>
 __device__ __forceinline__ void halo_issue_nk(const int nk16, float (&acc)[MTM][BN], const uint32_t hlo, const uint32_t blo, const uint32_t* s_aoff,
                                               const int gt, const uint32_t ahi, const uint32_t bhi, const uint32_t a_mstep, const uint32_t a_half,
-                                              const bool first) {
-  if (nk16 == 4) halo_issue_stage<4, MT>(acc, hlo, blo, s_aoff, gt, ahi, bhi, a_mstep, a_half, first);
-  else if (nk16 == 1) halo_issue_stage<1, MT>(acc, hlo, blo, s_aoff, gt, ahi, bhi, a_mstep, a_half, first);
-  else if (nk16 == 2) halo_issue_stage<2, MT>(acc, hlo, blo, s_aoff, gt, ahi, bhi, a_mstep, a_half, first);
-  else halo_issue_stage<3, MT>(acc, hlo, blo, s_aoff, gt, ahi, bhi, a_mstep, a_half, first);
+                                              const uint32_t bstep, const bool first) {
+  if (nk16 == 4) halo_issue_stage<4, MT>(acc, hlo, blo, s_aoff, gt, ahi, bhi, a_mstep, a_half, bstep, first);
+  else if (nk16 == 1) halo_issue_stage<1, MT>(acc, hlo, blo, s_aoff, gt, ahi, bhi, a_mstep, a_half, bstep, first);
+  else if (nk16 == 2) halo_issue_stage<2, MT>(acc, hlo, blo, s_aoff, gt, ahi, bhi, a_mstep, a_half, bstep, first);
+  else halo_issue_stage<3, MT>(acc, hlo, blo, s_aoff, gt, ahi, bhi, a_mstep, a_half, bstep, first);
 }
 template <int BN, int MTM>
 __device__ __forceinline__ void halo_issue_any(const int nk16, float (&acc)[MTM][BN], const uint32_t hlo, const uint32_t blo, const uint32_t* s_aoff,
                                                const int gt, const int MT, const uint32_t ahi, const uint32_t bhi, const uint32_t a_mstep,
-                                               const uint32_t a_half, const bool first) {
+                                               const uint32_t a_half, const uint32_t bstep, const bool first) {
   static_assert(MTM >= 1 && MTM <= 4, "1..4 stacked tiles");
-  if (MT == 1) halo_issue_nk<1>(nk16, acc, hlo, blo, s_aoff, gt, ahi, bhi, a_mstep, a_half, first);
+  if (MT == 1) halo_issue_nk<1>(nk16, acc, hlo, blo, s_aoff, gt, ahi, bhi, a_mstep, a_half, bstep, first);
   else if constexpr (MTM >= 2) {
-    if (MT == 2) halo_issue_nk<2>(nk16, acc, hlo, blo, s_aoff, gt, ahi, bhi, a_mstep, a_half, first);
+    if (MT == 2) halo_issue_nk<2>(nk16, acc, hlo, blo, s_aoff, gt, ahi, bhi, a_mstep, a_half, bstep, first);
     else if constexpr (MTM >= 3) {
-      if (MT == 3) halo_issue_nk<3>(nk16, acc, hlo, blo, s_aoff, gt, ahi, bhi, a_mstep, a_half, first);
-      else if constexpr (MTM >= 4) halo_issue_nk<4>(nk16, acc, hlo, blo, s_aoff, gt, ahi, bhi, a_mstep, a_half, first);
+      if (MT == 3) halo_issue_nk<3>(nk16, acc, hlo, blo, s_aoff, gt, ahi, bhi, a_mstep, a_half, bstep, first);
+      else if constexpr (MTM >= 4) halo_issue_nk<4>(nk16, acc, hlo, blo, s_aoff, gt, ahi, bhi, a_mstep, a_half, bstep, first);
     }
   }
   wg_wait<0>();
+}
+
+__host__ __device__ __forceinline__ int thin_plane_bytes(int HP) { return (HP * 16 + 127) & ~127; }
+__host__ __device__ __forceinline__ int halo_nsteps(int thin, int ntaps) { return thin == 8 ? (ntaps + 1) / 2 : ntaps; }
+__device__ __forceinline__ uint32_t halo_step_off(const CisConv& p, const int t0, const int nt, const int s, const int Wh, const uint32_t plane16) {
+  if (!p.thin) return (uint32_t)((p.dh[t0 + s] * Wh + p.dw[t0 + s]) * 8);
+  const int ta = p.thin == 8 ? 2 * s : s;
+  const uint32_t o0 = (uint32_t)(p.dh[t0 + ta] * Wh + p.dw[t0 + ta]);
+  if (p.thin == 16) return o0 | (plane16 << 16);
+  const uint32_t o1 = ta + 1 < nt ? (uint32_t)(p.dh[t0 + ta + 1] * Wh + p.dw[t0 + ta + 1]) : o0;
+  return o0 | ((o1 - o0) << 16);
 }
 
 template <int BN, int NWG>
@@ -575,7 +585,9 @@
   const int MT = p.MT, MTC = NWG * MT, d = p.dil;
   const int nph = p.nph > 1 ? p.nph : 1;
   const int Wh = 8 + p.ex, Hh = 16 * MTC + p.ey, HP = Wh * Hh;
-  const uint32_t stage_bytes = (uint32_t)G * kBStage;
+  const int thin = p.thin;
+  const uint32_t wstep = thin ? BN * 32 : kBStage;
+  const uint32_t stage_bytes = (uint32_t)G * wstep;
   const uint32_t tile_base = (smem_u32(smem_raw) + 1023u) & ~1023u;
   const uint32_t h_base = tile_base;
   const uint32_t b_base = tile_base + NHS * halo_stage_bytes;
@@ -586,6 +598,7 @@
 
   const bool grouped = p.nsub > 1;
   const int tap0 = grouped ? p.sub[blockIdx.z].tap0 : 0, ntaps = grouped ? p.sub[blockIdx.z].ntaps : p.ntaps;
+  const int nst = halo_nsteps(thin, ntaps);
   const int hoy = grouped ? p.sub[blockIdx.z].hoy : p.hoy, hox = grouped ? p.sub[blockIdx.z].hox : p.hox;
   const int OHs = grouped ? p.sub[blockIdx.z].OH : p.OH, OWs = grouped ? p.sub[blockIdx.z].OW : p.OW;
   const int oa = grouped ? p.sub[blockIdx.z].oa : p.oa, ob = grouped ? p.sub[blockIdx.z].ob : p.ob;
@@ -610,7 +623,7 @@
   __shared__ __align__(16) float s_bias[BN];
   pdl_launch_dependents();
 
-  if (tid < ntaps) s_aoff[tid] = (uint32_t)((p.dh[tap0 + tid] * Wh + p.dw[tap0 + tid]) * 8);
+  if (tid < nst) s_aoff[tid] = halo_step_off(p, tap0, ntaps, tid, Wh, (uint32_t)thin_plane_bytes(HP) >> 4);
   if (tid < p.nsrc) {
     s_src[tid].ptr = reinterpret_cast<const __nv_bfloat16*>(p.src[tid].ptr);
     s_src[tid].pitch = p.src[tid].pitch;
@@ -659,6 +672,21 @@
             ++si;
           }
           const int nmod = s_src[si].n_mod;
+          if (thin) {
+            const int npl = thin / 8, pb16 = thin_plane_bytes(HP);
+            mbar_expect_tx(bar_hfull + 8 * hs, (uint32_t)(npl * HP * 16));
+            for (int q = 0; q < npl; ++q) {
+              int cq = q, sq = 0;
+              while (sq < p.nsrc - 1 && cq >= s_src[sq].chunks) {
+                cq -= s_src[sq].chunks;
+                ++sq;
+              }
+              const int nm = s_src[sq].n_mod;
+              tma_load_4d(h_base + hs * halo_stage_bytes + q * pb16, &maps.m[sq], bar_hfull + 8 * hs, cq * 8, tx * 8 + hox, ty * 16 * MTC + hoy,
+                          nm ? (n % nm) : n);
+            }
+            continue;
+          }
           mbar_expect_tx(bar_hfull + 8 * hs, (uint32_t)(HP * 128));
           tma_load_4d(h_base + hs * halo_stage_bytes, &maps.m[si * nph + ph], bar_hfull + 8 * hs, c * 8, pb + d * (tx * 8 + hox),
                       pa + d * (ty * 16 * MTC + hoy), nmod ? (n % nmod) : n);
@@ -715,17 +743,17 @@
       }
     }
     if (tid == 64) {
-      const uint8_t* wt = reinterpret_cast<const uint8_t*>(wpack) + ((size_t)ny * nchunks_all + cc_lo) * ntaps * kBStage;
+      const uint8_t* wt = reinterpret_cast<const uint8_t*>(wpack) + ((size_t)ny * nchunks_all + cc_lo) * nst * wstep;
       int bs = 0;
       uint32_t bph = 1;
       for (int vc = 0; vc < nchunks * nph; ++vc) {
         const int cc = vc / nph, ph = vc - cc * nph;
-        const int tlo = nph > 1 ? p.ph_tap[ph] : 0, thi = nph > 1 ? p.ph_tap[ph + 1] : ntaps;
+        const int tlo = nph > 1 ? p.ph_tap[ph] : 0, thi = nph > 1 ? p.ph_tap[ph + 1] : nst;
         for (int t0 = tlo; t0 < thi; t0 += G) {
-          const uint32_t bytes = (uint32_t)min(G, thi - t0) * kBStage;
+          const uint32_t bytes = (uint32_t)min(G, thi - t0) * wstep;
           mbar_wait(bar_bempty + 8 * bs, bph);
           mbar_expect_tx(bar_bfull + 8 * bs, bytes);
-          bulk_g2s(b_base + bs * stage_bytes, wt + (size_t)(cc * ntaps + t0) * kBStage, bytes, bar_bfull + 8 * bs);
+          bulk_g2s(b_base + bs * stage_bytes, wt + (size_t)(cc * nst + t0) * wstep, bytes, bar_bfull + 8 * bs);
           if (++bs == BS) {
             bs = 0;
             bph ^= 1u;
@@ -741,28 +769,29 @@
     const int wtid = tid - (kHMmaWarp_ + 4 * wg) * 32;
     constexpr int MTM = Cfg::kMaxMT;
     float acc[MTM][BN];
-    const uint32_t ahi = desc_hi((uint32_t)(Wh * 128)), bhi = desc_hi(1024);
-    const uint32_t a_mstep = (uint32_t)(16 * Wh * 128) >> 4;
-    const uint32_t a_half = (uint32_t)(8 * Wh * 128) >> 4;
+    const uint32_t pix = thin ? 16u : 128u;
+    const uint32_t ahi = thin ? desc_hi_ns((uint32_t)Wh * pix) : desc_hi((uint32_t)Wh * pix), bhi = thin ? desc_hi_ns(256) : desc_hi(1024);
+    const uint32_t a_mstep = (16u * Wh * pix) >> 4;
+    const uint32_t a_half = (8u * Wh * pix) >> 4;
     const uint32_t a_wg = (uint32_t)(wg * MT) * a_mstep;
     int bs = 0, hs = 0, it = 0;
     uint32_t bph = 0, hph = 0;
     bool any = false;
     for (int vc = 0; vc < nchunks * nph; ++vc) {
       const int cc = vc / nph, ph = vc - cc * nph;
-      const int tlo = nph > 1 ? p.ph_tap[ph] : 0, thi = nph > 1 ? p.ph_tap[ph + 1] : ntaps;
+      const int tlo = nph > 1 ? p.ph_tap[ph] : 0, thi = nph > 1 ? p.ph_tap[ph + 1] : nst;
       if (thi == tlo) continue;
       const int rem = m_chunks - (cc_lo + cc) * 8;
       const int nk16 = rem >= 8 ? 4 : (rem + 1) / 2;
       mbar_wait(bar_hfull + 8 * hs, hph);
       if (vc == 0 && wtid == 0 && wg == 0) CIS_TRACE_AT(1);
-      const uint32_t hlo = desc_lo(h_base + hs * halo_stage_bytes, 16) + a_wg;
+      const uint32_t hlo = desc_lo(h_base + hs * halo_stage_bytes, thin ? 0 : 16) + a_wg;
       for (int t0 = tlo; t0 < thi; t0 += G, ++it) {
         const int gt = min(G, thi - t0);
         mbar_wait(bar_bfull + 8 * bs, bph);
         if (wtid == 0 && wg == 0) CIS_TRACE_AT(8 + 2 * it);
-        const uint32_t blo = desc_lo(b_base + bs * stage_bytes, 16);
-        halo_issue_any<BN, MTM>(nk16, acc, hlo, blo, s_aoff + t0, gt, MT, ahi, bhi, a_mstep, a_half, !any);
+        const uint32_t blo = desc_lo(b_base + bs * stage_bytes, thin ? 128 : 16);
+        halo_issue_any<BN, MTM>(nk16, acc, hlo, blo, s_aoff + t0, gt, MT, ahi, bhi, a_mstep, a_half, wstep >> 4, !any);
         if (wtid == 0) {
           mbar_arrive(bar_bempty + 8 * bs);
           if (t0 + G >= thi) mbar_arrive(bar_hempty + 8 * hs);
@@ -895,7 +924,11 @@
   const int tid = threadIdx.x, warp = tid >> 5, lane = tid & 31;
   const int MT = p.MT;
   const int Wh = 8 + p.ex, Hh = 16 * MT + p.ey, HP = Wh * Hh;
-  const uint32_t stage_bytes = (uint32_t)G * kBStage;
+  const int thin = p.thin;
+  const bool grouped = p.nsub > 1;
+  const int nsb = grouped ? p.nsub : 1;
+  const uint32_t wstep = thin ? BN * 32 : kBStage;
+  const uint32_t stage_bytes = (uint32_t)G * wstep;
   const uint32_t tile_base = (smem_u32(smem_raw) + 1023u) & ~1023u;
   const uint32_t acc_bytes = (uint32_t)(MT * BN) * kAccColBytes;
   const uint32_t acc_base = tile_base, h_base = tile_base + AS * acc_bytes, b_base = h_base + NHS * halo_stage_bytes;
@@ -903,14 +936,30 @@
   const uint32_t bar_bfull = smem_u32(&bars[2 * kMaxHS]), bar_bempty = smem_u32(&bars[2 * kMaxHS + kHaloMaxBStages]);
   const uint32_t bar_tfull = smem_u32(&bars[2 * kMaxHS + 2 * kHaloMaxBStages]), bar_tempty = smem_u32(&bars[2 * kMaxHS + 2 * kHaloMaxBStages + 2]);
 
-  const int tiles_x = (p.OW + 7) / 8, tiles_y = (p.OH + 16 * MT - 1) / (16 * MT);
-  const int total = tiles_x * tiles_y * p.N;
+  __shared__ int s_tcum[5], s_sbase[5];
   int m_chunks = 0;
   for (int i = 0; i < p.nsrc; ++i) m_chunks += p.src[i].chunks;
   const int nchunks = (m_chunks + 7) / 8;
 
   pdl_launch_dependents();
-  if (tid < p.ntaps) s_aoff[tid] = (uint32_t)((p.dh[tid] * Wh + p.dw[tid]) * 8);
+  {
+    int tc = 0, sb = 0;
+    for (int z = 0; z < nsb; ++z) {
+      const int nt = grouped ? p.sub[z].ntaps : p.ntaps, t0 = grouped ? p.sub[z].tap0 : 0, ns = halo_nsteps(thin, nt);
+      const int oh = grouped ? p.sub[z].OH : p.OH, ow = grouped ? p.sub[z].OW : p.OW;
+      if (tid >= sb && tid < sb + ns) s_aoff[tid] = halo_step_off(p, t0, nt, tid - sb, Wh, (uint32_t)thin_plane_bytes(HP) >> 4);
+      if (tid == 0) {
+        s_tcum[z] = tc;
+        s_sbase[z] = sb;
+      }
+      tc += ((ow + 7) / 8) * ((oh + 16 * MT - 1) / (16 * MT)) * p.N;
+      sb += ns;
+    }
+    if (tid == 0) {
+      s_tcum[nsb] = tc;
+      s_sbase[nsb] = sb;
+    }
+  }
   if (tid == 0) {
     for (int s = 0; s < NHS; ++s) {
       mbar_init(bar_hfull + 8 * s, 1);
@@ -930,6 +979,16 @@
   pdl_wait();
   if (tid < BN) s_bias[tid] = p.bias ? p.bias[tid] : 0.f;
   __syncthreads();
+  const int total = s_tcum[nsb];
+  auto decode = [&](const int w, int& z, int& tx, int& ty, int& n) {
+    z = 0;
+    while (z + 1 < nsb && w >= s_tcum[z + 1]) ++z;
+    const int tiles_x = ((grouped ? p.sub[z].OW : p.OW) + 7) / 8, tiles_y = ((grouped ? p.sub[z].OH : p.OH) + 16 * MT - 1) / (16 * MT);
+    const int l = w - s_tcum[z];
+    tx = l % tiles_x;
+    ty = (l / tiles_x) % tiles_y;
+    n = l / (tiles_x * tiles_y);
+  };
   if (tid == 0) {
     CIS_TRACE_AT(0);
     CIS_TRACE_AT(4);
@@ -940,7 +999,9 @@
       int hs = 0;
       uint32_t hph = 1;
       for (int w = blockIdx.x; w < total; w += gridDim.x) {
-        const int tx = w % tiles_x, r1 = w / tiles_x, ty = r1 % tiles_y, n = r1 / tiles_y;
+        int z, tx, ty, n;
+        decode(w, z, tx, ty, n);
+        const int hox = grouped ? p.sub[z].hox : p.hox, hoy = grouped ? p.sub[z].hoy : p.hoy;
         for (int cc = 0; cc < nchunks; ++cc) {
           mbar_wait(bar_hempty + 8 * hs, hph);
           int c = cc * 8, si = 0;
@@ -952,9 +1013,24 @@
           if (si == 1) nmod = p.src[1].n_mod;
           if (si == 2) nmod = p.src[2].n_mod;
           if (si == 3) nmod = p.src[3].n_mod;
-          mbar_expect_tx(bar_hfull + 8 * hs, (uint32_t)(HP * 128));
-          tma_load_4d(h_base + hs * halo_stage_bytes, &maps.m[si], bar_hfull + 8 * hs, c * 8, tx * 8 + p.hox, ty * 16 * MT + p.hoy,
-                      nmod ? (n % nmod) : n);
+          if (thin) {
+            const int npl = thin / 8, pb16 = thin_plane_bytes(HP);
+            mbar_expect_tx(bar_hfull + 8 * hs, (uint32_t)(npl * HP * 16));
+            for (int q = 0; q < npl; ++q) {
+              int cq = q, sq = 0;
+              while (sq < p.nsrc - 1 && cq >= p.src[sq].chunks) {
+                cq -= p.src[sq].chunks;
+                ++sq;
+              }
+              const int nm = p.src[sq].n_mod;
+              tma_load_4d(h_base + hs * halo_stage_bytes + q * pb16, &maps.m[sq], bar_hfull + 8 * hs, cq * 8, tx * 8 + hox, ty * 16 * MT + hoy,
+                          nm ? (n % nm) : n);
+            }
+          } else {
+            mbar_expect_tx(bar_hfull + 8 * hs, (uint32_t)(HP * 128));
+            tma_load_4d(h_base + hs * halo_stage_bytes, &maps.m[si], bar_hfull + 8 * hs, c * 8, tx * 8 + hox, ty * 16 * MT + hoy,
+                        nmod ? (n % nmod) : n);
+          }
           if (++hs == NHS) {
             hs = 0;
             hph ^= 1u;
@@ -965,13 +1041,17 @@
   } else if (warp == 13) {
     if (lane == 0) {
       const uint8_t* wt = reinterpret_cast<const uint8_t*>(p.wpack);
-      const int per_tile = nchunks * p.ntaps;
+      const int nst = s_sbase[1];
       if (ws) {
         if ((int)blockIdx.x < total) {
-          mbar_expect_tx(bar_bfull, (uint32_t)(per_tile * kBStage));
-          for (int it = 0; it < per_tile; it += 8) {
-            const int nt = min(8, per_tile - it);
-            bulk_g2s(b_base + it * kBStage, wt + (size_t)it * kBStage, (uint32_t)(nt * kBStage), bar_bfull);
+          mbar_expect_tx(bar_bfull, (uint32_t)(nchunks * s_sbase[nsb] * wstep));
+          for (int z = 0; z < nsb; ++z) {
+            const uint8_t* wz = grouped ? reinterpret_cast<const uint8_t*>(p.sub[z].wpack) : wt;
+            const int per = nchunks * (s_sbase[z + 1] - s_sbase[z]);
+            for (int it = 0; it < per; it += 8) {
+              const int nt = min(8, per - it);
+              bulk_g2s(b_base + (s_sbase[z] + it) * wstep, wz + (size_t)it * wstep, (uint32_t)(nt * wstep), bar_bfull);
+            }
           }
         }
       } else {
@@ -979,11 +1059,11 @@
         uint32_t bph = 1;
         for (int w = blockIdx.x; w < total; w += gridDim.x) {
           for (int cc = 0; cc < nchunks; ++cc) {
-            for (int t0 = 0; t0 < p.ntaps; t0 += G) {
-              const uint32_t bytes = (uint32_t)min(G, p.ntaps - t0) * kBStage;
+            for (int t0 = 0; t0 < nst; t0 += G) {
+              const uint32_t bytes = (uint32_t)min(G, nst - t0) * wstep;
               mbar_wait(bar_bempty + 8 * bs, bph);
               mbar_expect_tx(bar_bfull + 8 * bs, bytes);
-              bulk_g2s(b_base + bs * stage_bytes, wt + (size_t)(cc * p.ntaps + t0) * kBStage, bytes, bar_bfull + 8 * bs);
+              bulk_g2s(b_base + bs * stage_bytes, wt + (size_t)(cc * nst + t0) * wstep, bytes, bar_bfull + 8 * bs);
               if (++bs == BS) {
                 bs = 0;
                 bph ^= 1u;
@@ -997,30 +1077,35 @@
     const int wtid = tid;
     constexpr int MTM = (kPMaxAccCols / BN) < 4 ? kPMaxAccCols / BN : 4;
     float acc[MTM][BN];
-    const uint32_t ahi = desc_hi((uint32_t)(Wh * 128)), bhi = desc_hi(1024);
-    const uint32_t a_mstep = (uint32_t)(16 * Wh * 128) >> 4;
-    const uint32_t a_half = (uint32_t)(8 * Wh * 128) >> 4;
+    const uint32_t pix = thin ? 16u : 128u;
+    const uint32_t ahi = thin ? desc_hi_ns((uint32_t)Wh * pix) : desc_hi((uint32_t)Wh * pix), bhi = thin ? desc_hi_ns(256) : desc_hi(1024);
+    const uint32_t a_mstep = (16u * Wh * pix) >> 4;
+    const uint32_t a_half = (8u * Wh * pix) >> 4;
     int hs = 0, bs = 0, as = 0;
     uint32_t hph = 0, bph = 0, tph = 1;
     if (ws && (int)blockIdx.x < total) mbar_wait(bar_bfull, 0u);
     int wi = 0;
     for (int w = blockIdx.x; w < total; w += gridDim.x, ++wi) {
       if (wtid == 0) CIS_TRACE_AT(8 + 5 * wi);
+      int z, tx, ty, n;
+      decode(w, z, tx, ty, n);
+      const int nst = s_sbase[z + 1] - s_sbase[z];
+      const uint32_t* so = s_aoff + s_sbase[z];
       for (int cc = 0; cc < nchunks; ++cc) {
         const int rem = m_chunks - cc * 8;
         const int nk16 = rem >= 8 ? 4 : (rem + 1) / 2;
         mbar_wait(bar_hfull + 8 * hs, hph);
         if (cc == 0 && wtid == 0) CIS_TRACE_AT(10 + 5 * wi);
-        const uint32_t hlo = desc_lo(h_base + hs * halo_stage_bytes, 16);
-        const int gstep = ws ? p.ntaps : G;
-        for (int t0 = 0; t0 < p.ntaps; t0 += gstep) {
-          const int gt = min(gstep, p.ntaps - t0);
+        const uint32_t hlo = desc_lo(h_base + hs * halo_stage_bytes, thin ? 0 : 16);
+        const int gstep = ws ? nst : G;
+        for (int t0 = 0; t0 < nst; t0 += gstep) {
+          const int gt = min(gstep, nst - t0);
           if (!ws) mbar_wait(bar_bfull + 8 * bs, bph);
-          const uint32_t blo = desc_lo(ws ? b_base + (uint32_t)(cc * p.ntaps) * kBStage : b_base + bs * stage_bytes, 16);
-          halo_issue_any<BN, MTM>(nk16, acc, hlo, blo, s_aoff + t0, gt, MT, ahi, bhi, a_mstep, a_half, (cc | t0) == 0);
+          const uint32_t blo = desc_lo(ws ? b_base + (uint32_t)(s_sbase[z] + cc * nst) * wstep : b_base + bs * stage_bytes, thin ? 128 : 16);
+          halo_issue_any<BN, MTM>(nk16, acc, hlo, blo, so + t0, gt, MT, ahi, bhi, a_mstep, a_half, wstep >> 4, (cc | t0) == 0);
           if (wtid == 0) {
             if (!ws) mbar_arrive(bar_bempty + 8 * bs);
-            if (t0 + gstep >= p.ntaps) mbar_arrive(bar_hempty + 8 * hs);
+            if (t0 + gstep >= nst) mbar_arrive(bar_hempty + 8 * hs);
           }
           if (!ws && ++bs == BS) {
             bs = 0;
@@ -1052,13 +1137,16 @@
       int wi = 0;
       for (int w = blockIdx.x; w < total; w += gridDim.x, ++wi) {
         if (wi % AS != grp) continue;
-        const int tx = w % tiles_x, r1 = w / tiles_x, ty = r1 % tiles_y, n = r1 / tiles_y;
+        int z, tx, ty, n;
+        decode(w, z, tx, ty, n);
+        const int OHs = grouped ? p.sub[z].OH : p.OH, OWs = grouped ? p.sub[z].OW : p.OW;
+        const int oa = grouped ? p.sub[z].oa : p.oa, ob = grouped ? p.sub[z].ob : p.ob;
         mbar_wait(bar_tfull + 8 * grp, tph);
         tph ^= 1u;
         for (int m = 0; m < MT; ++m) {
           const int oy = ty * 16 * MT + 16 * m + (r >> 3), ox = tx * 8 + (r & 7);
-          const bool valid = oy < p.OH && ox < p.OW;
-          const size_t dpix = valid ? ((size_t)(n * p.DH + oy * p.osh + p.oa) * p.DW + ox * p.osw + p.ob) : 0;
+          const bool valid = oy < OHs && ox < OWs;
+          const size_t dpix = valid ? ((size_t)(n * p.DH + oy * p.osh + oa) * p.DW + ox * p.osw + ob) : 0;
           epi_row<BN>(p, acc_base + grp * acc_bytes + (uint32_t)r * 16 + (uint32_t)(m * BN) * kAccColBytes, 0, dpix, valid, s_bias);
         }
         __syncwarp();
@@ -1574,9 +1662,12 @@
 static int launch_halo(const CisConv* d, cudaStream_t st) {
   const int MTC = d->MT * NWG;
   const int Wh = 8 + d->ex, Hh = 16 * MTC + d->ey, HP = Wh * Hh;
-  const int halo_stage = (HP * 128 + 1023) & ~1023;
+  const int thin = d->thin;
+  const int halo_stage = ((thin ? thin / 8 * thin_plane_bytes(HP) : HP * 128) + 1023) & ~1023;
   int chunks = 0;
   for (int i = 0; i < d->nsrc; ++i) chunks += d->src[i].chunks;
+  if (thin && ((thin != 8 && thin != 16) || chunks * 8 != thin || d->dil != 1 || d->nph > 1))
+    return cis_set_error(CIS_ERR_BAD_ARG, "cis_conv_igemm(halo): the compact format needs 8 or 16 undilated input channels");
   const int nchunks = (chunks + 7) / 8;
   const int nsub = d->nsub > 1 ? d->nsub : 1;
   const int nsp = (nsub == 1 && d->splits > 1) ? d->splits : 1;
@@ -1600,13 +1691,22 @@
     const int Hp0 = (d->OH + dd - 1) / dd, Wp0 = (d->OW + dd - 1) / dd;
     tiles = ((Wp0 + 7) / 8) * ((Hp0 + 16 * MTC - 1) / (16 * MTC));
   }
+  if (thin == 8) {
+    for (int i = 0; i < nsub; ++i) {
+      const int t0 = nsub > 1 ? d->sub[i].tap0 : 0, nt = nsub > 1 ? d->sub[i].ntaps : d->ntaps;
+      for (int t = t0 + 1; t < t0 + nt; ++t)
+        if (d->dh[t] * (8 + d->ex) + d->dw[t] < d->dh[t - 1] * (8 + d->ex) + d->dw[t - 1])
+          return cis_set_error(CIS_ERR_BAD_ARG, "cis_conv_igemm(halo): compact 8-channel taps must be listed in increasing halo offset");
+    }
+  }
+  const int nst_max = halo_nsteps(thin, ntaps_max);
   const long ncta_all = (long)tiles * dd * dd * d->N * d->n_tiles * nsp * nsub;
   static const int g_env = getenv("CIS_HALO_G") ? atoi(getenv("CIS_HALO_G")) : 0;
   static const int stage_kb = getenv("CIS_HALO_STAGE_KB") ? atoi(getenv("CIS_HALO_STAGE_KB")) : 48;
-  const int kB = BN * 128;
+  const int kB = thin ? BN * 32 : BN * 128;
   int G = g_env > 0 ? g_env : (stage_kb * 1024) / kB;
   if (G < 1) G = 1;
-  if (G > ntaps_max) G = ntaps_max;
+  if (G > nst_max) G = nst_max;
   const int fixed = nhs * halo_stage + HP * 4 + 1024;
   static const int lim_small_kb = getenv("CIS_HALO_SMALL_KB") ? atoi(getenv("CIS_HALO_SMALL_KB")) : 226;
   static const int lim_kb_wide = getenv("CIS_HALO_LIMIT_KB") ? atoi(getenv("CIS_HALO_LIMIT_KB")) : 113;
@@ -1616,7 +1716,7 @@
   int limit = (ncta_all > nsm && fixed + 2 * kB <= lim_kb * 1024) ? lim_kb * 1024 : 226 * 1024;
   if (ncta_all <= nsm && fixed + 2 * kB <= lim_small_kb * 1024) limit = lim_small_kb * 1024;
   while (G > 1 && fixed + 2 * G * kB > limit) --G;
-  const int groups = cper * ((nsub > 1 ? 1 : (ntaps_max + G - 1) / G));
+  const int groups = cper * ((nsub > 1 ? 1 : (nst_max + G - 1) / G));
   int BS = (limit - fixed) / (G * kB);
   if (BS > (ncta_all > nsm ? 4 : kHaloMaxBStages)) BS = ncta_all > nsm ? 4 : kHaloMaxBStages;
   if (BS > groups) BS = groups;
@@ -1642,22 +1742,32 @@
   const int nph = d->nph > 1 ? d->nph : 1;
   static const int dil_tma = getenv("CIS_DIL_TMA") ? atoi(getenv("CIS_DIL_TMA")) : 1;
   int use_tma = ((d->dil == 1 || dil_tma) && Wh * d->dil <= 256 && Hh * d->dil <= 256) ? 1 : 0;
-  for (int i = 0; use_tma && i < d->nsrc - 1; ++i)
+  for (int i = 0; use_tma && !thin && i < d->nsrc - 1; ++i)
     if (d->src[i].chunks % 8) use_tma = 0;
   for (int i = 0; use_tma && i < d->nsrc; ++i) {
     if (((uintptr_t)d->src[i].ptr + (size_t)d->src[i].c_off * 2) % 16) use_tma = 0;
     for (int ph = 0; use_tma && ph < nph; ++ph)
-      if (!encode_src_map(&maps.m[i * nph + ph], d->src[i], d->N, d->H, d->W, Wh, Hh, nph > 1 ? 2 : 1, ph >> 1, ph & 1, d->dil)) use_tma = 0;
+      if (!(thin ? encode_src_map(&maps.m[i], d->src[i], d->N, d->H, d->W, Wh, Hh, 1, 0, 0, 1, 8, CU_TENSOR_MAP_SWIZZLE_NONE)
+                 : encode_src_map(&maps.m[i * nph + ph], d->src[i], d->N, d->H, d->W, Wh, Hh, nph > 1 ? 2 : 1, ph >> 1, ph & 1, d->dil)))
+        use_tma = 0;
   }
   if (!use_tma) memset(&maps, 0, sizeof(maps));
+  if (thin && !use_tma) return cis_set_error(CIS_ERR_UNSUPPORTED, "cis_conv_igemm(halo): the compact format needs the TMA halo path");
   if (nph > 1 && !use_tma) return cis_set_error(CIS_ERR_UNSUPPORTED, "cis_conv_igemm(halo): stride-2 phases need the TMA halo path");
   const int persist_mode = g_persist_mode >= 0 ? g_persist_mode : (getenv("CIS_PERSIST_MODE") ? atoi(getenv("CIS_PERSIST_MODE")) : 1);
   static const int p_min_tiles = getenv("CIS_PERSIST_MIN_TILES") ? atoi(getenv("CIS_PERSIST_MIN_TILES")) : 296;
   static const int p_ws_kb = getenv("CIS_PERSIST_WS_KB") ? atoi(getenv("CIS_PERSIST_WS_KB")) : 112;
   if constexpr (BN <= kPMaxAccCols && NWG == 1) {
-   if (persist_mode > 0 && use_tma && d->n_tiles == 1 && splits == 1 && nph == 1 && nsub == 1 && dd == 1 && d->MT * BN <= kPMaxAccCols) {
-    const int total = tiles * d->N;
-    const int per_tile = nchunks * d->ntaps;
+   if (persist_mode > 0 && use_tma && d->n_tiles == 1 && splits == 1 && nph == 1 && (nsub == 1 || nchunks == 1) && dd == 1 &&
+       d->MT * BN <= kPMaxAccCols) {
+    int total = tiles * d->N, per_tile = nchunks * nst_max;
+    if (nsub > 1) {
+      total = per_tile = 0;
+      for (int i = 0; i < nsub; ++i) {
+        total += ((d->sub[i].OW + 7) / 8) * ((d->sub[i].OH + 16 * d->MT - 1) / (16 * d->MT)) * d->N;
+        per_tile += halo_nsteps(thin, d->sub[i].ntaps);
+      }
+    }
     const int acc_stage = d->MT * BN * (int)kAccColBytes;
     const int AS = 2;
     const int fixed_p = AS * acc_stage + 1024;
@@ -1675,7 +1785,7 @@
       if (p_bs > 4) p_bs = 4;
       p_smem = p_nhs * halo_stage + fixed_p + p_bs * G * kB;
     }
-    if (take && p_bs >= (ws_fits ? 1 : 2)) {
+    if (take && (ws_fits || nsub == 1) && p_bs >= (ws_fits ? 1 : 2)) {
       static int attr_p = 0;
       if (p_smem > attr_p) {
         cudaError_t e = cudaFuncSetAttribute(conv_halo_persist_kernel<BN>, cudaFuncAttributeMaxDynamicSharedMemorySize, p_smem);
diff --git a/unsupervised_detection_b200/csrc/misc_kernels.cu b/unsupervised_detection_b200/csrc/misc_kernels.cu
--- a/unsupervised_detection_b200/csrc/misc_kernels.cu
+++ b/unsupervised_detection_b200/csrc/misc_kernels.cu
@@ -84,6 +84,28 @@
     const int kk = (((pos >> 3) ^ (n & 7)) << 3) | (pos & 7);
     o[idx] = __float2bfloat16(tile[kk * ld + n]);
   }
+}
+__device__ __forceinline__ void pack_weights_thin_body(size_t i, const float* __restrict__ w, const int* __restrict__ kmap, int cin8, int ntaps,
+                                                       int n_tiles, int BN, int cout, int sn, const int* __restrict__ nmap, int thin,
+                                                       bf16* __restrict__ out) {
+  const int nst = thin == 8 ? (ntaps + 1) / 2 : ntaps;
+  if (i >= (size_t)n_tiles * nst * BN * 16) return;
+  const int e = (int)(i % 8);
+  const int n8 = (int)((i / 8) % 8);
+  const int j = (int)((i / 64) % 2);
+  size_t r = i / 128;
+  const int ng8 = (int)(r % (BN / 8));
+  r /= BN / 8;
+  const int s = (int)(r % nst), ny = (int)(r / nst);
+  const int t = thin == 8 ? 2 * s + j : s, c = thin == 8 ? e : 8 * j + e;
+  float v = 0.f;
+  if (t < ntaps && c < cin8) {
+    const int km = kmap[t * cin8 + c];
+    const int ng = ny * BN + ng8 * 8 + n8;
+    const int ne = nmap ? nmap[ng] : (ng < cout ? ng : -1);
+    if (km >= 0 && ne >= 0) v = w[(size_t)km + (size_t)ne * sn];
+  }
+  out[i] = __float2bfloat16(v);
 }
 __device__ __forceinline__ void unpack_wgrad_body(size_t i, const float* __restrict__ dwp, const int* __restrict__ kmap, int K_pad, int cout,
                                                   int nsplit, float* __restrict__ dw, const float* __restrict__ colpart, int nblocks, int nch,
@@ -162,11 +184,12 @@
   pack_weights_body((size_t)blockIdx.x * blockDim.x + threadIdx.x, w, kmap, K_pad, rows, cout, sn, nmap, wp);
 }
 __global__ void pack_weights_tiled_kernel(const float* __restrict__ w, const int* __restrict__ kmap, int cin8, int ntaps, int n_tiles, int BN,
-                                          int cout, int sn, const int* __restrict__ nmap, bf16* __restrict__ out) {
+                                          int cout, int sn, const int* __restrict__ nmap, bf16* __restrict__ out, int thin) {
   pdl_launch_dependents();
   pdl_wait();
   __shared__ float tile[64 * 129];
-  if (sn == 1) pack_weights_tiled_tile(blockIdx.x, w, kmap, cin8, ntaps, n_tiles, BN, cout, nmap, out, tile);
+  if (thin) pack_weights_thin_body((size_t)blockIdx.x * blockDim.x + threadIdx.x, w, kmap, cin8, ntaps, n_tiles, BN, cout, sn, nmap, thin, out);
+  else if (sn == 1) pack_weights_tiled_tile(blockIdx.x, w, kmap, cin8, ntaps, n_tiles, BN, cout, nmap, out, tile);
   else pack_weights_tiled_body((size_t)blockIdx.x * blockDim.x + threadIdx.x, w, kmap, cin8, ntaps, n_tiles, BN, cout, sn, nmap, out);
 }
 __global__ void unpack_wgrad_kernel(const float* __restrict__ dwp, const int* __restrict__ kmap, int K_pad, int cout, int nsplit,
@@ -208,7 +231,12 @@
       pack_weights_body(i, (const float*)j.p[0], (const int*)j.p[1], j.i[0], j.i[1], j.i[2], j.i[3], (const int*)j.p[2], (bf16*)j.p[3]);
       break;
     case CIS_JOB_PACK_TILED:
-      if (j.i[5] == 1)
+      if (j.i[6]) {
+        const size_t per = j.i[5] == 1 ? (size_t)j.i[3] * 64 : blockDim.x;
+        for (size_t q = threadIdx.x; q < per; q += blockDim.x)
+          pack_weights_thin_body((size_t)blk * per + q, (const float*)j.p[0], (const int*)j.p[1], j.i[0], j.i[1], j.i[2], j.i[3], j.i[4], j.i[5],
+                                 (const int*)j.p[2], j.i[6], (bf16*)j.p[3]);
+      } else if (j.i[5] == 1)
         pack_weights_tiled_tile(blk, (const float*)j.p[0], (const int*)j.p[1], j.i[0], j.i[1], j.i[2], j.i[3], j.i[4], (const int*)j.p[2],
                                 (bf16*)j.p[3], tile);
       else
@@ -1709,11 +1737,13 @@
   return cis_check_launch("pack_weights");
 }
 int cis_pack_weights_tiled(const float* w, const int32_t* kmap, int32_t cin8, int32_t ntaps, int32_t n_tiles, int32_t BN, int32_t cout, int32_t sn,
-                           const int32_t* nmap, void* out, cis_stream_t stream) {
-  const size_t total = (size_t)n_tiles * ((cin8 + 63) / 64) * ntaps * BN * 64;
-  const unsigned blocks = sn == 1 ? (unsigned)(n_tiles * ((cin8 + 63) / 64) * ntaps) : nblk(total);
+                           const int32_t* nmap, void* out, int32_t thin, cis_stream_t stream) {
+  const size_t total = thin ? (size_t)n_tiles * (thin == 8 ? (ntaps + 1) / 2 : ntaps) * BN * 16
+                            : (size_t)n_tiles * ((cin8 + 63) / 64) * ntaps * BN * 64;
+  const unsigned blocks = (sn == 1 && !thin) ? (unsigned)(n_tiles * ((cin8 + 63) / 64) * ntaps) : nblk(total);
   if (BN > 128) return cis_set_error(CIS_ERR_UNSUPPORTED, "cis_pack_weights_tiled: BN > 128");
-  CIS_LAUNCH(pack_weights_tiled_kernel, blocks, 256, 0, ST, w, kmap, cin8, ntaps, n_tiles, BN, cout, sn, nmap, (mbf)out);
+  if (thin && (cin8 != thin || (thin != 8 && thin != 16))) return cis_set_error(CIS_ERR_BAD_ARG, "cis_pack_weights_tiled: thin must be 8 or 16 = cin8");
+  CIS_LAUNCH(pack_weights_tiled_kernel, blocks, 256, 0, ST, w, kmap, cin8, ntaps, n_tiles, BN, cout, sn, nmap, (mbf)out, thin);
   return cis_check_launch("pack_weights_tiled");
 }
 int cis_unpack_wgrad(const float* dwp, const int32_t* kmap, int32_t K_pad, int32_t cout, int32_t nsplit, float* dw, const float* colpart,
diff --git a/unsupervised_detection_b200/csrc/ptx.cuh b/unsupervised_detection_b200/csrc/ptx.cuh
--- a/unsupervised_detection_b200/csrc/ptx.cuh
+++ b/unsupervised_detection_b200/csrc/ptx.cuh
@@ -139,6 +139,7 @@
 };
 
 __device__ __forceinline__ uint32_t desc_hi(uint32_t sbo_bytes) { return ((sbo_bytes >> 4) & 0x3FFF) | (1u << 30); }
+__device__ __forceinline__ uint32_t desc_hi_ns(uint32_t sbo_bytes) { return (sbo_bytes >> 4) & 0x3FFF; }
 __device__ __forceinline__ uint32_t desc_lo(uint32_t saddr, uint32_t lbo_bytes) {
   return ((saddr & 0x3FFFF) >> 4) | (((lbo_bytes >> 4) & 0x3FFF) << 16);
 }
diff --git a/unsupervised_detection_b200/engine.py b/unsupervised_detection_b200/engine.py
--- a/unsupervised_detection_b200/engine.py
+++ b/unsupervised_detection_b200/engine.py
@@ -113,11 +113,11 @@
                 j.kind, blocks = JOB_PACK, -(-(rows * K_pad) // 256)
                 ptrs, ints = [w, kmap, nmap, wp], [K_pad, rows, cout, sn]
             elif name == 'cis_pack_weights_tiled':
-                w, kmap, cin8, ntaps, n_tiles, BN, cout, sn, nmap, out = a
+                w, kmap, cin8, ntaps, n_tiles, BN, cout, sn, nmap, out, thin = a
                 j.kind, blocks = JOB_PACK_TILED, -(-(n_tiles * (-(-cin8 // 64)) * ntaps * BN * 64) // 256)
                 if sn == 1:
                     blocks = n_tiles * (-(-cin8 // 64)) * ntaps
-                ptrs, ints = [w, kmap, nmap, out], [cin8, ntaps, n_tiles, BN, cout, sn]
+                ptrs, ints = [w, kmap, nmap, out], [cin8, ntaps, n_tiles, BN, cout, sn, thin]
             elif name == 'cis_unpack_wgrad':
                 dwp, kmap, K_pad, cout, nsplit, dw, colpart, nblocks, nch, db, layout = a
                 j.kind, blocks = JOB_UNPACK, -(-(cout * K_pad + nch) // 256)
@@ -450,8 +450,17 @@
         return False
     d.halo, d.dil, d.MT, d.hoy, d.hox, d.ey, d.ex = 1, dil, best[1], hoy, hox, ey, ex
     d.nwg = halo_nwg(d, best[1], Hp0, Wp0, dil, n_tiles, ntaps, nchunks, ey, ex)
-    _fill_taps(d, rel)
+    d.thin = thin_format(m_chunks, dil)
+    _fill_taps(d, [rel[i] for i in thin_tap_order(d.thin, rel)])
     return True
+
+
+def thin_format(m_chunks, dil):
+    return m_chunks * 8 if dil == 1 and m_chunks in (1, 2) else 0
+
+
+def thin_tap_order(thin, taps):
+    return sorted(range(len(taps)), key=lambda i: tuple(taps[i])) if thin == 8 else list(range(len(taps)))
 
 
 S2_HALO = os.environ.get('CIS_S2_HALO', '0') == '1'
@@ -514,7 +523,7 @@
         return None
     d0 = descs[0]
     same = ('N', 'H', 'W', 'BN', 'n_tiles', 'nsrc', 'act', 'DH', 'DW', 'osh', 'osw', 'out', 'out_pitch', 'out_coff', 'out_ch', 'outf', 'outf_pitch',
-            'outf_coff', 'outf_ch', 'add_pre', 'add_pre_pitch', 'add_pre_coff', 'add_post', 'addf_pre', 'mode', 'bias')
+            'outf_coff', 'outf_ch', 'add_pre', 'add_pre_pitch', 'add_pre_coff', 'add_post', 'addf_pre', 'mode', 'bias', 'thin')
     for d in descs:
         if not d.halo or d.dil != 1 or d.splits > 1 or d.nph > 1 or any(getattr(d, f) != getattr(d0, f) for f in same):
             return None
@@ -607,6 +616,7 @@
     w: torch.Tensor = None
     wt: torch.Tensor = None
     wt_kmap: torch.Tensor = None
+    thin: int = 0
     rows_used: bool = None
     wg_splits: dict = dataclasses.field(default_factory=dict)
     dwp: torch.Tensor = None
@@ -701,10 +711,17 @@
             return
         if pk.wt is None:
             pk.wt = self._alloc_tiles(len(taps), kch, pk.BN, pk.n_tiles)
+            pk.thin = d.thin
             if order is not None:
                 pk.taps = list(order)
                 pk.wt_kmap, _ = self._kmap(pk.taps, self.in_chanmap, self.cin * self.cout, self.cout)
+            perm = thin_tap_order(d.thin, taps)
+            if perm != sorted(perm):
+                n = len(taps)
+                pk.wt_kmap = pk.kmap.clone()
+                pk.wt_kmap[:n * kch] = pk.kmap[:n * kch].view(n, kch)[perm].reshape(-1)
         assert order is None or pk.taps == list(order), self.name
+        assert pk.thin == d.thin, self.name
         d.wpack = pk.wt.data_ptr()
         if pk.rows_used is None:
             pk.rows_used = False
@@ -729,7 +746,7 @@
         for pk, kch, nch, sn in packs:
             if pk.wt is not None:
                 plan.add('cis_pack_weights_tiled', self.w_src_ptr(), (pk.kmap if pk.wt_kmap is None else pk.wt_kmap).data_ptr(), kch,
-                         len(pk.taps), pk.n_tiles, pk.BN, nch, sn, _ptr(pk.nmap), pk.wt.data_ptr())
+                         len(pk.taps), pk.n_tiles, pk.BN, nch, sn, _ptr(pk.nmap), pk.wt.data_ptr(), pk.thin)
             if pk.rows_used is not False:
                 plan.add('cis_pack_weights', self.w_src_ptr(), pk.kmap.data_ptr(), pk.K_pad, pk.rows, nch, sn, _ptr(pk.nmap), pk.w.data_ptr())
 
```

After: 642.5 (median of 6 runs). 1.04x the previous value.
